# Ekumen-OS/beluga

Measured on AMD Instinct MI355X. Metric: MCL update cycles/sec (motion+sensor+resample), N particles x 1080 beams, higher is better.
Workload: dtype f64; 1 GPU; BASELINE configs[1]: 1M particles/GPU, 1080-beam LikelihoodFieldModel, 4000x4000@5cm grid (seed 42), DifferentialDriveModel, multinomial resample every cycle; particles_per_gpu=1000000, particles_total=1000000, beams=1080, grid=4000x4000@0.05, parallelism=1 GPU

## Files before the change

### beluga_amd/csrc/context.hip

```cpp
#include <hip/hip_runtime.h>
#include <dlfcn.h>

#include <algorithm>
#include <cctype>
#include <atomic>
#include <chrono>
#include <thread>
#include <cmath>
#include <cstdio>
#include <cstring>
#include <limits>
#include <new>
#include <numeric>
#include <optional>
#include <string>
#include <unordered_set>
#include <map>
#include <vector>

#include "beluga_mcl.h"
#include "cluster_host.h"
#include "cycle_host.h"
#include "kernels.h"
#include "landmark_host.h"
// ... 27 lines not shown
  mcl_config cfg;
  std::string error;
  int device{0};
  hipStream_t stream{nullptr};
  bool own_stream{false};
  mcl_batch* batch{nullptr};

  uint64_t capacity{0};
  uint64_t n{0};
  ParticleSet sets[2];
  int live{0};

  bool have_map{false};
  MapHold<MapStore> map{std::make_shared<MapStore>()};
  DeviceBuffer<uint32_t> d_field_scratch;
  uint64_t comm_bytes_out{0};
  uint64_t comm_collectives{0};
  uint64_t comm_host_syncs{0};
  uint64_t comm_overflows{0};
  uint64_t comm_ranks_seen{0};
  int comm_backend{0};
  uint64_t cluster_cells{0};

  DeviceBuffer<double> d_points;
  DeviceBuffer<double> d_beam_points;
  DeviceBuffer<double> d_beam_table;
  uint32_t beam_table_count{0};
  bool beam_table_ready{false};
  HostBuffer<double> h_points;
  double scan_extent{0.0};
  uint64_t scan_no_cell{0};
  hipEvent_t points_event{nullptr};
  bool points_in_flight{false}, points_event_valid{false};

  DeviceBuffer<double> d_chunk;
  uint32_t chunk_stride{0};
  DeviceBuffer<double> d_scalars;
  HostBuffer<double> h_scalars;
  DeviceBuffer<double> d_cdf;
  DeviceBuffer<double4> d_cloud;
  DeviceBuffer<double> d_est_partials;
  uint64_t done_seq{0};
  bool done_armed{false};
  uint64_t host_ns[4]{0, 0, 0, 0};
  uint64_t host_cycles{0};
  uint64_t noise_ahead_used{0};
  DeviceBuffer<double> d_cloud_w;
  DeviceBuffer<double> d_cdf_tree;
  DeviceBuffer<unsigned long long> d_scan_state;
  uint32_t scan_epoch{0};
  SetFacts facts;
  DeviceBuffer<double> d_lf_wsum;
  DeviceBuffer<double> d_noise;
  DiffDriveSampler order_sampler{};
  uint64_t order_ahead_used{0}, order_ahead_missed{0};
  DiffDriveSampler last_sampler{};
  bool have_last_sampler{false};
  CdfTree cdf_tree() const { return make_cdf_tree(d_cdf.ptr, d_cdf_tree.ptr, n); }
  struct PendingMap {
    std::vector<int8_t> cells;
    uint32_t W{0}, H{0};
    double resolution{0.0}, origin[4]{1.0, 0.0, 0.0, 0.0};
    int8_t traits[3]{0, -1, 100};
    std::vector<float> field;
    std::thread worker;
    std::atomic<int> state{0};
  };
  PendingMap* pending_map{nullptr};

  DeviceBuffer<unsigned long long> d_hashes;
  DeviceBuffer<unsigned long long> d_table_keys;
  DeviceBuffer<unsigned int> d_table_first;
  uint64_t table_capacity{0};
  DeviceBuffer<uint32_t> d_flags, d_uchunk;
  uint64_t kld_capacity{0};
  uint32_t kld_chunks{0};
  uint64_t kld_pos{0}, kld_table_slots{0};
  int kld_flip{0};
  DeviceBuffer<unsigned long long> d_kld_scalars;
  HostBuffer<unsigned long long> h_kld_scalars;

  DeviceBuffer<double> d_cell_f64;
  DeviceBuffer<unsigned int> d_cell_u32;
  DeviceBuffer<unsigned long long> d_cell_u64;
  DeviceBuffer<double> d_cell_exchange;
  DeviceBuffer<double> d_cluster_sums;
  DeviceBuffer<unsigned int> d_cluster_labels;
  int estimate_kind{0};
  mcl_cluster_params cluster_params{0.20, 0.524, 0.90};

  ExponentialFilter slow, fast;
  bool have_latest{false};
  Pose2 latest{};
  uint64_t every_n_current{0};
  bool force_update{true};
  bool have_window{false};
  Pose2 window0{}, window1{};
  uint32_t step{0};
  Tuning tuning{};
  CloudEstimate cloud;
  uint64_t lf_fast_launches{0};
  LfPlanner lf_planner;
  uint64_t lf_patch_launches{0};
  uint64_t lf_queue_launches{0};
  uint64_t lf_beams_launches{0};
  uint64_t estimate_repivots{0};
// ... 127 lines not shown
}
void stage_end(mcl_ctx* ctx, int stage) {
  if (!stage_timed(ctx, stage)) return;
  (void)hipEventRecord(ctx->ev[stage][1], ctx->stream);
  ctx->ev_pending[stage] = true;
}
void stage_collect(mcl_ctx* ctx) {
  ctx->points_in_flight = false;
  if (!ctx->profile) return;
  for (int s = 0; s < MCL_NUM_STAGES; ++s) {
    if (!ctx->ev_pending[s]) continue;
    float ms = 0.f;
    if (hipEventElapsedTime(&ms, ctx->ev[s][0], ctx->ev[s][1]) == hipSuccess) {
      ctx->prof_ms[s] += ms;
      ctx->prof_count[s] += 1;
    }
    ctx->ev_pending[s] = false;
  }
}

mcl_status wait_for_cycle(mcl_ctx* ctx) {
  if (ctx->done_armed) {
    ctx->done_armed = false;
    const volatile uint64_t* word = reinterpret_cast<const volatile uint64_t*>(ctx->h_scalars.host + kSlotDoneWord);
    const auto t0 = std::chrono::steady_clock::now();
    for (uint32_t spins = 1;; ++spins) {
      if (*word == ctx->done_seq) {
        std::atomic_thread_fence(std::memory_order_acquire);
        if ((ctx->done_seq & 0xFFu) == 0) break;
        return MCL_OK;
      }
#if defined(__x86_64__) || defined(__i386__)
      __builtin_ia32_pause();
#elif defined(__aarch64__)
      asm volatile("yield" ::: "memory");
#else
      std::this_thread::yield();
#endif
      if ((spins & 0xFFFu) == 0 && std::chrono::steady_clock::now() - t0 > std::chrono::milliseconds(20)) break;
    }
  }
  MCL_HIP(ctx, hipStreamSynchronize(ctx->stream));
  return MCL_OK;
}

mcl_status ensure_capacity(mcl_ctx* ctx, uint64_t cap) {
  for (auto& set : ctx->sets) MCL_HIP(ctx, set.ensure(cap));
  const uint32_t chunks = num_chunks(cap) + 1;
  ctx->chunk_stride = chunks;
  MCL_HIP(ctx, ctx->d_chunk.ensure(static_cast<size_t>(12) * chunks));
  MCL_HIP(ctx, ctx->d_cdf.ensure(cap));
  MCL_HIP(ctx, ctx->d_cdf_tree.ensure(cdf_tree_doubles(cap)));
  MCL_HIP(ctx, ctx->d_lf_wsum.ensure(cap / 448 + 2));
  if (!ctx->d_scan_state.ptr) {
    MCL_HIP(ctx, ctx->d_scan_state.ensure(kScanStateWords));
    MCL_HIP(ctx, hipMemset(ctx->d_scan_state.ptr, 0, kScanStateWords * sizeof(unsigned long long)));
  }
  ctx->capacity = cap;
  {
    static_assert(sizeof(KeyFrame) <= 8 * sizeof(double), "the key frame sits in the first 8 doubles of d_sort_f64");
    const size_t table = static_cast<size_t>(kSortDigits) * num_chunks(cap);
    MCL_HIP(ctx, ctx->d_sort_u32.ensure(2 * cap + table + 2 * kSortDigits + 16));
    MCL_HIP(ctx, ctx->d_sort_u64.ensure(cap));
    MCL_HIP(ctx, ctx->d_sort_f64.ensure(8 + 8 + 6 * static_cast<size_t>(chunks) + kLfMaxSegments * std::min<uint64_t>(cap, kLfSegmentedBelow)));
  }
  return MCL_OK;
}

mcl_status ensure_kld(mcl_ctx* ctx) {
  const uint64_t cap = std::max<uint64_t>(ctx->capacity, ctx->cfg.shard_capacity ? ctx->cfg.amcl.max_particles : 0);
  MCL_HIP(ctx, ctx->d_hashes.ensure(cap));
  MCL_HIP(ctx, ctx->d_flags.ensure(cap));
  ctx->kld_chunks = num_chunks(cap) + 1;
  MCL_HIP(ctx, ctx->d_uchunk.ensure(static_cast<size_t>(2) * ctx->kld_chunks));
  uint64_t tc = 1024;
  while (tc < 2 * cap) tc <<= 1;
  MCL_HIP(ctx, ctx->d_table_keys.ensure(tc));
  MCL_HIP(ctx, ctx->d_table_first.ensure(tc));
  ctx->table_capacity = tc;
  ctx->kld_capacity = cap;
  return MCL_OK;
}

enum KldWord : int { kKldFirstFail = 0, kKldBeamSteps = 1, kKldCounts = 4 };
mcl_status kld_begin(mcl_ctx* ctx) {
  if (ctx->table_capacity == 0) {
    if (const mcl_status s = ensure_kld(ctx)) return s;
  }
  MCL_HIP(ctx, hipMemsetAsync(ctx->d_kld_scalars.ptr + kKldFirstFail, 0xFF, sizeof(unsigned long long), ctx->stream));
  uint32_t* kwords = reinterpret_cast<uint32_t*>(ctx->d_kld_scalars.ptr + kKldCounts);
  MCL_HIP(ctx, hipMemsetAsync(kwords, 0, 2 * sizeof(uint32_t), ctx->stream));
  ctx->kld_pos = 0;
  ctx->kld_table_slots = 0;
  ctx->kld_flip = 0;
  return MCL_OK;
}

mcl_status kld_grow_table(mcl_ctx* ctx, uint64_t candidates) {
  uint64_t want = 1024;
  while (want < 2 * candidates) want <<= 1;
  want = std::min<uint64_t>(want, ctx->table_capacity);
  if (want <= ctx->kld_table_slots) return MCL_OK;
  ctx->kld_table_slots = want;
  MCL_HIP(ctx, hipMemsetAsync(ctx->d_table_keys.ptr, 0xFF, want * sizeof(unsigned long long), ctx->stream));
  MCL_HIP(ctx, hipMemsetAsync(ctx->d_table_first.ptr, 0xFF, want * sizeof(unsigned int), ctx->stream));
  launch_kld_insert(ctx->stream, ctx->d_hashes.ptr, 0, ctx->kld_pos, KldTable{ctx->d_table_keys.ptr, ctx->d_table_first.ptr, want});
// ... 310 lines not shown
    staged->doubles = kept;
  }
  ctx->scan_extent = poisoned ? std::numeric_limits<double>::quiet_NaN() : extent;
  return MCL_OK;
}
void points_pulled(mcl_ctx* ctx, bool with_event) {
  if (with_event) (void)hipEventRecord(ctx->points_event, ctx->stream);
  ctx->points_event_valid = with_event;
  ctx->points_in_flight = true;
}

void advance_window(mcl_ctx* ctx, const Pose2& pose) {
  ctx->window1 = ctx->have_window ? ctx->window0 : pose;
  ctx->window0 = pose;
  ctx->have_window = true;
  ctx->step += 1;
  const Pose2 action = pose_mul(pose_inverse(ctx->window1), ctx->window0);
  ctx->facts.pivot_carried(action.r.c, action.r.s, action.x, action.y);
}
void finish_cycle(mcl_ctx* ctx, const mcl_estimate& est, const mcl_update_info& report, mcl_estimate* estimate, mcl_update_info* info) {
  ctx->facts.estimate_reported(est.pose[0], est.pose[1], est.pose[2], est.pose[3]);
  ctx->cloud.remember(est);
  if (estimate) *estimate = est;
  if (info) *info = report;
}

void patch_totals(const mcl_ctx* ctx, uint64_t* planned, uint64_t* through, bool synchronised = false) {
  const volatile uint64_t* mirror = reinterpret_cast<const volatile uint64_t*>(ctx->h_scalars.host + kSlotPatchMirror);
  if (synchronised) {
    *planned = mirror[0];
    *through = mirror[1];
    return;
  }
  const uint64_t packed = mirror[2];
  *planned = packed & 0xFFFFFFFFull;
  *through = packed >> 32;
}
LfPlanner::Mode plan_lf(mcl_ctx* ctx) {
  uint64_t planned = 0, through = 0;
  if (!ctx->lf_planner.decided()) patch_totals(ctx, &planned, &through);
  return ctx->lf_planner.decide(ctx->lf_site(), ctx->cloud, planned, through);
}
struct HeldCycle {
  bool propagate_held{false};
  bool fused{false};
  bool pending{false};
  bool beam{false};
  BatchItem item{};
  uint64_t every_n{0};
};
void launch_held_propagate(mcl_ctx* ctx, HeldCycle* hold) {
  const BatchItem& it = hold->item;
  launch_propagate(ctx->stream, it.p, it.n, it.smp, it.seed, it.step, it.index_offset, it.scan_src, it.scan_dst, it.scan_doubles, nullptr, nullptr,
                   nullptr, 0);
  hold->propagate_held = false;
}
mcl_status do_propagate(mcl_ctx* ctx, const Pose2& pose, const Pose2& prev, uint32_t step, uint64_t scan_doubles = 0,
                        bool* keys_emitted = nullptr, HeldCycle* hold = nullptr) {
  stage_begin(ctx, MCL_STAGE_PROPAGATE);
  const DiffDriveSampler sampler = make_sampler(pose, prev, ctx->cfg.motion, ctx->cfg.motion_kind, ctx->cfg.strafe_noise_from_translation);
  KeyFrame frame{};
  const SortScratch sort = ctx->sort_scratch();
  if (keys_emitted) plan_lf(ctx);
  ctx->facts.order_accepted(false);
  bool use_ahead = false;
  if (keys_emitted) {
    const SetFacts::OrderTaken ahead = ctx->facts.take_order_ahead(step, ctx->n, ctx->key_layout());
    use_ahead = ahead.matched && ctx->tuning.order_ahead != 0 && ctx->wants_ordering() && samplers_close(sampler, ctx->order_sampler);
    if (use_ahead) ctx->order_ahead_used += 1;
    else if (ahead.recorded) ctx->order_ahead_missed += 1;
  }
  ctx->last_sampler = sampler;
  ctx->have_last_sampler = true;
  const bool keys = !use_ahead && keys_emitted && ctx->wants_ordering() && ctx->predict_key_frame(&sampler, &frame);
  const bool ahead = ctx->d_noise.ptr && ctx->n > 65536 && ctx->facts.noise_ahead_serves(step, ctx->n, ctx->cfg.seed, ctx->cfg.shard_offset);
  if (hold && !keys && !ahead && ctx->n >= 1 && ctx->n <= kBatchMaxParticles && !ctx->profile) {
    BatchItem& it = hold->item;
    it.p = ctx->cur();
    it.n = ctx->n;
    it.smp = sampler;
    it.seed = ctx->cfg.seed;
    it.step = step;
    it.index_offset = ctx->cfg.shard_offset;
    it.scan_src = scan_doubles ? ctx->h_points.device : nullptr;
    it.scan_dst = scan_doubles ? ctx->d_points.ptr : nullptr;
    it.scan_doubles = static_cast<uint32_t>(scan_doubles);
    hold->propagate_held = true;
  } else {
    launch_propagate(ctx->stream, ctx->cur(), ctx->n, sampler, ctx->cfg.seed, step, ctx->cfg.shard_offset,
                     scan_doubles ? ctx->h_points.device : nullptr, scan_doubles ? ctx->d_points.ptr : nullptr, static_cast<uint32_t>(scan_doubles),
                     keys ? &sort : nullptr, keys ? &frame : nullptr, ahead ? ctx->d_noise.ptr : nullptr, ctx->facts.noise_ahead_count());
  }
  if (ahead) ctx->noise_ahead_used += 1;
  if (scan_doubles) points_pulled(ctx, false);
  if (keys_emitted) *keys_emitted = keys;
  ctx->facts.order_accepted(use_ahead);
  stage_end(ctx, MCL_STAGE_PROPAGATE);
  MCL_HIP(ctx, hipGetLastError());
  return MCL_OK;
}

mcl_status reweight_preconditions(mcl_ctx* ctx, uint64_t B) {
  if (ctx->is_ndt()) {
    if (!ctx->have_ndt_map) return fail(ctx, MCL_ERR_NOT_READY, "mcl_reweight: no NDT map set (mcl_set_ndt_map)");
    MCL_REQUIRE(ctx, B <= 0x7FFFFFFFull, "too many points");
    return MCL_OK;
  }
  if (ctx->is_landmark()) {
    if (!ctx->have_landmark_map) return fail(ctx, MCL_ERR_NOT_READY, "no landmark map set (mcl_set_landmark_map)");
    return MCL_OK;
  }
  if (!ctx->have_map) return fail(ctx, MCL_ERR_NOT_READY, "mcl_reweight: no map set");
  MCL_REQUIRE(ctx, B <= 0x7FFFFFFFull, "too many points");
  if (ctx->cfg.sensor_kind == MCL_SENSOR_BEAM && !(ctx->n < (1ull << 32) && ctx->n >= static_cast<uint64_t>(ctx->tuning.beam_sort_min_particles)))
    MCL_REQUIRE(ctx, B * sizeof(double2) <= 64 * 1024, "scan too large for the beam model's small-set kernel (4096 points)");
  return MCL_OK;
}

mcl_status do_reweight(mcl_ctx* ctx, Measurement m, bool points_staged = false, bool keys_ready = false,
                       bool want_weight_sums = false, HeldCycle* hold = nullptr) {
  ctx->facts.lf_sums_dropped();
  if (const mcl_status s = reweight_preconditions(ctx, ctx->off_grid() ? 0 : m.doubles / 2)) return s;
  const bool unit_weights = ctx->facts.take_unit_weights() && ctx->tuning.lf_unit_weights != 0;
  if (!points_staged) {
    if (const mcl_status s = stage_points(ctx, &m)) return s;
    if (m.doubles) {
      launch_pull_scan(ctx->stream, ctx->h_points.device, ctx->d_points.ptr, static_cast<uint32_t>(m.doubles));
      points_pulled(ctx, true);
    }
  }
  const uint64_t B = ctx->off_grid() ? 0 : m.doubles / 2;
  stage_begin(ctx, MCL_STAGE_REWEIGHT);
  const LfPlanner::Mode mode = plan_lf(ctx);
  const bool ordered = ctx->wants_ordering();
  const bool dispersed = ctx->lf_planner.gathers_dispersed(ctx->tuning);
  ctx->lf_planner.mode_consumed();
  const SortScratch sort = ctx->sort_scratch();
  const bool have_order = ctx->facts.take_order_accepted();
  const bool lf_kind = !ctx->off_grid() && ctx->cfg.sensor_kind != MCL_SENSOR_BEAM;
  LfReweightArgs lf_args{};
  if (lf_kind)
    lf_args = LfReweightArgs{.p = ctx->cur(), .n = ctx->n, .f = ctx->field_view(), .d_points = ctx->d_points.ptr, .B = static_cast<uint32_t>(B),
                             .sort = ordered ? &sort : nullptr, .patches = mode.patches, .beams = mode.beams,
                             .dispersed = dispersed,
                             .scan_cells = ctx->scan_extent / ctx->map->resolution, .unit_weights = unit_weights,
                             .stats = PatchStats{reinterpret_cast<unsigned long long*>(ctx->d_scalars.ptr + kSlotPatchTotals),
                                                 reinterpret_cast<unsigned long long*>(ctx->h_scalars.device + kSlotPatchMirror),
                                                 static_cast<uint32_t>(ctx->tuning.lf_loose_below), ctx->tuning.lf_margin ? 0u : 1u,
                                                 static_cast<uint32_t>(ctx->tuning.lf_split), want_weight_sums ? ctx->d_lf_wsum.ptr : nullptr,
                                                 reinterpret_cast<unsigned int*>(ctx->d_scalars.ptr + kSlotPatchQueue)}};
  if (hold && hold->propagate_held) {
    hold->fused = lf_kind && batch_member_fused(BatchMemberFacts{
                                 ctx->cfg.sensor_kind, ctx->have_comm && ctx->comm_world > 1, ctx->tuning.small_fused != 0, ctx->n,
                                 std::min<uint64_t>(ctx->cfg.amcl.max_particles, ctx->capacity), lf_takes_beams(lf_args, ctx->tuning), ctx->profile != 0});
    hold->beam = !lf_kind && !ordered && batch_beam_member_fused(BatchBeamFacts{
                                 ctx->cfg.sensor_kind, ctx->have_comm && ctx->comm_world > 1, ctx->tuning.small_fused != 0,
                                 ctx->tuning.batch_beam_fused != 0, ctx->n, std::min<uint64_t>(ctx->cfg.amcl.max_particles, ctx->capacity),
                                 static_cast<uint64_t>(ctx->tuning.beam_sort_min_particles), ctx->profile != 0});
    hold->fused = hold->fused || hold->beam;
    if (!hold->fused) launch_held_propagate(ctx, hold);
  }
  if (ordered && !have_order) {
    KeyFrame frame{};
    const bool have_frame = !keys_ready && ctx->predict_key_frame(nullptr, &frame);
    launch_order_particles(ctx->stream, ctx->cur(), ctx->n, &sort, have_frame ? &frame : nullptr, keys_ready, frame.layout);
  }
  if (ctx->is_ndt()) {
    stage_begin(ctx, MCL_STAGE_SENSOR_KERNEL);
    launch_reweight_ndt(ctx->stream, ctx->cur(), ctx->n, ctx->ndt_view, ctx->d_points.ptr, static_cast<uint32_t>(m.doubles / kNdtRecord));
    stage_end(ctx, MCL_STAGE_SENSOR_KERNEL);
  } else if (ctx->is_landmark()) {
    const uint32_t k = static_cast<uint32_t>(m.doubles / kLandmarkRecord);
    stage_begin(ctx, MCL_STAGE_SENSOR_KERNEL);
    if (ctx->cfg.sensor_kind == MCL_SENSOR_LANDMARK) launch_reweight_landmarks(ctx->stream, ctx->cur(), ctx->n, ctx->landmark_view, ctx->d_points.ptr, k);
    else launch_reweight_bearings(ctx->stream, ctx->cur(), ctx->n, ctx->landmark_view, ctx->d_points.ptr, k);
    stage_end(ctx, MCL_STAGE_SENSOR_KERNEL);
  } else if (ctx->cfg.sensor_kind != MCL_SENSOR_BEAM) {
    stage_begin(ctx, MCL_STAGE_SENSOR_KERNEL);
    LfLaunch launched{LfKernel::kBeams, 0};
    if (hold && hold->fused) {
      hold->item.f = lf_args.f;
      hold->item.B = lf_args.B;
    } else {
      launched = launch_reweight_lf(ctx->stream, lf_args, ctx->tuning);
    }
    ctx->facts.lf_sums_left(launched.weight_sums);
    switch (launched.kernel) {
      case LfKernel::kPatchQueue: ctx->lf_queue_launches += 1; [[fallthrough]];
      case LfKernel::kPatch: ctx->lf_patch_launches += 1; ctx->lf_fast_launches += 1; break;
      case LfKernel::kFarBeams: ctx->lf_far_beams_launches += 1; [[fallthrough]];
      case LfKernel::kPaletteFar: ctx->lf_far_launches += 1; [[fallthrough]];
      case LfKernel::kPaletteFast: ctx->lf_fast_launches += 1; break;
      case LfKernel::kBeams: ctx->lf_beams_launches += 1; break;
      default: break;
    }
    stage_end(ctx, MCL_STAGE_SENSOR_KERNEL);
  } else {
    const mcl_beam_params& b = ctx->cfg.beam;
    const BeamModel model{b.z_hit, b.z_short, b.z_max, b.z_rand, b.sigma_hit, b.lambda_short, b.beam_max_range};
    const bool use_table = ordered && ctx->tuning.beam_table != 0 && ctx->beam_table_count != 0;
    if (use_table && !ctx->beam_table_ready) {
      hipError_t e = ctx->d_beam_table.ensure(4 * static_cast<size_t>(ctx->beam_table_count));
      if (e == hipSuccess) {
        launch_beam_table(ctx->stream, model, ctx->map->resolution, ctx->beam_table_count, ctx->d_beam_table.ptr);
        e = hipGetLastError();
      }
      if (e != hipSuccess) {
        stage_end(ctx, MCL_STAGE_REWEIGHT);
        return fail(ctx, MCL_ERR_HIP, std::string("reweight (beam table): ") + hipGetErrorString(e));
      }
      ctx->beam_table_ready = true;
    }
    stage_begin(ctx, MCL_STAGE_SENSOR_KERNEL);
    if (hold && hold->fused) {
      hold->item.B = static_cast<uint32_t>(B);
      hold->item.beam = batch_beam_record(ctx->grid_view(), model, ctx->map->d_nonfree_bits.ptr, ctx->d_kld_scalars.ptr + kKldBeamSteps);
    } else {
      launch_reweight_beam(ctx->stream, ctx->cur(), ctx->n, ctx->grid_view(), model,
                           ctx->d_points.ptr, static_cast<uint32_t>(B), ctx->d_kld_scalars.ptr + kKldBeamSteps, ordered ? &sort : nullptr,
                           ctx->map->d_nonfree_bits.ptr, ctx->d_beam_points.ptr, use_table ? ctx->d_beam_table.ptr : nullptr,
                           use_table ? ctx->beam_table_count : 0u, ctx->tuning.beam_free_ahead != 0, ctx->tuning.beam_sectors != 0);
    }
    stage_end(ctx, MCL_STAGE_SENSOR_KERNEL);
  }
  stage_end(ctx, MCL_STAGE_REWEIGHT);
  ctx->profile_tick += 1;
  if (const hipError_t e = hipGetLastError(); e != hipSuccess) {
    ctx->facts.lf_sums_dropped();
    return fail(ctx, MCL_ERR_HIP, std::string("reweight: ") + hipGetErrorString(e));
  }
  return MCL_OK;
}

mcl_weight_stats mirrored_weight_stats(const mcl_ctx* ctx) {
  return mcl_weight_stats{ctx->h_scalars.host[kSlotWeightSum], ctx->h_scalars.host[kSlotNormSum], ctx->h_scalars.host[kSlotNormSumSq]};
// ... 1231 lines not shown
    p->cells.assign(cells, cells + static_cast<size_t>(width) * height);
  } catch (const std::bad_alloc&) {
    delete p;
    return fail(ctx, MCL_ERR_OUT_OF_MEMORY, "mcl_set_map_async: out of memory");
  }
  p->W = width;
  p->H = height;
  p->resolution = resolution;
  std::memcpy(p->origin, origin, sizeof p->origin);
  std::memcpy(p->traits, value_traits, sizeof p->traits);
  ctx->pending_map = p;
  if (ctx->cfg.sensor_kind != MCL_SENSOR_BEAM && ctx->tuning.field_build == 0) {
    p->state.store(1, std::memory_order_release);
    const mcl_lf_params lf = ctx->cfg.lf;
    p->worker = std::thread([p, lf] {
      build_likelihood_field(p->cells.data(), p->W, p->H, p->resolution, OccupancyTraits{p->traits[0], p->traits[1], p->traits[2]}, lf, p->field);
      p->state.store(2, std::memory_order_release);
    });
  } else {
    p->state.store(2, std::memory_order_release);
  }
  return MCL_OK;
}

mcl_status mcl_map_pending(mcl_ctx* ctx, int32_t* state) {
  if (!ctx || !state) return MCL_ERR_INVALID_ARGUMENT;
  *state = ctx->pending_map ? ctx->pending_map->state.load(std::memory_order_acquire) : 0;
  return MCL_OK;
}

mcl_status mcl_map_commit(mcl_ctx* ctx, int32_t wait) {
  if (!ctx) return MCL_ERR_INVALID_ARGUMENT;
  return apply_pending_map(ctx, wait != 0);
}

}
namespace {
void map_installed(mcl_ctx* ctx) {
  if (ctx->cfg.sensor_kind == MCL_SENSOR_BEAM) {
    ctx->beam_table_count = beam_table_entries(ctx->cfg.beam.beam_max_range, ctx->map->resolution);
    ctx->beam_table_ready = false;
  }
  ctx->have_map = true;
}

mcl_status set_map_impl(mcl_ctx* ctx, const int8_t* cells, uint32_t width, uint32_t height, double resolution, const double origin[4],
                        const int8_t value_traits[3], std::vector<float>* prebuilt_field) {
  if (const mcl_status s = bind_device(ctx)) return s;
  MCL_HIP(ctx, hipStreamSynchronize(ctx->stream));
  auto store = std::make_shared<MapStore>();
  if (const std::shared_ptr<MapStore> old = ctx->map.take_private()) store->take_buffers(*old);
  ctx->map.drop();
  ctx->have_map = false;
  store->key = MapStoreKey{ctx->device, ctx->cfg.sensor_kind, ctx->cfg.lf};
  const MapSource in{cells, width, height, resolution, origin, value_traits, ctx->tuning.field_build, prebuilt_field};
  std::string err;
  if (const mcl_status s = build_map_store(*store, in, ctx->stream, &ctx->d_field_scratch, ctx->ev[MCL_STAGE_REWEIGHT], &err)) return fail(ctx, s, err);
  ctx->map.own(std::move(store));
  map_installed(ctx);
  return MCL_OK;
}

struct InstallSet {
  uint64_t n;
  bool unit_weights;
  enum { kGlobalKept, kGlobalShares, kGlobalAsked } global;
  bool force_update;
  enum { kCloudKept, kCloudUnknown, kCloudGiven } cloud;
  double cloud_mean[3], cloud_sigma[3];
  LfPlanner::Installed patches;
  bool pivot_known = false;
  double pivot[2] = {0.0, 0.0};
  bool pivot_kept = false;
};
void install_set(mcl_ctx* ctx, const InstallSet& s) {
  ctx->facts.set_replaced(s.unit_weights, s.pivot_kept);
  ctx->n = s.n;
  if (s.global == InstallSet::kGlobalShares) ctx->global_n = 0;
  if (s.global != InstallSet::kGlobalKept) ctx->global_n_unknown = s.global == InstallSet::kGlobalAsked && ctx->have_comm && ctx->comm_world > 1;
  if (s.force_update) ctx->force_update = true;
  if (s.cloud == InstallSet::kCloudGiven) ctx->cloud.set(s.cloud_mean, s.cloud_sigma);
  else if (s.cloud == InstallSet::kCloudUnknown) ctx->cloud.forget();
  if (s.cloud == InstallSet::kCloudGiven)
    ctx->facts.estimate_reported(std::cos(s.cloud_mean[2]), std::sin(s.cloud_mean[2]), s.cloud_mean[0], s.cloud_mean[1]);
  else if (s.pivot_known) ctx->facts.pivot_given(s.pivot[0], s.pivot[1]);
  uint64_t planned = 0, through = 0;
  if (s.patches != LfPlanner::Installed::kKept) patch_totals(ctx, &planned, &through);
  ctx->lf_planner.set_installed(s.patches, planned, through);
}
}
extern "C" {

mcl_status mcl_get_likelihood_field(mcl_ctx* ctx, float* out) {
  if (!ctx) return MCL_ERR_INVALID_ARGUMENT;
  MCL_REQUIRE(ctx, out, "null output");
  if (ctx->off_grid()) return fail(ctx, MCL_ERR_UNSUPPORTED, "The current sensor model does not support likelihood field");
  if (!ctx->have_map || !ctx->map->d_field.ptr) return fail(ctx, MCL_ERR_NOT_READY, "no likelihood field");
  if (const mcl_status s = bind_device(ctx)) return s;
  MCL_HIP(ctx, hipStreamSynchronize(ctx->stream));
  MCL_HIP(ctx, hipMemcpy(out, ctx->map->d_field.ptr, static_cast<size_t>(ctx->map->W) * ctx->map->H * sizeof(float), hipMemcpyDeviceToHost));
  return MCL_OK;
}

mcl_status mcl_set_likelihood_field(mcl_ctx* ctx, const float* field) {
  if (!ctx) return MCL_ERR_INVALID_ARGUMENT;
  MCL_REQUIRE(ctx, field, "null field");
  if (ctx->off_grid()) return fail(ctx, MCL_ERR_UNSUPPORTED, "mcl_set_likelihood_field: not on a context whose sensor model has a map of its own (mcl_set_ndt_map, mcl_set_landmark_map)");
  if (!ctx->have_map) return fail(ctx, MCL_ERR_NOT_READY, "set the map first");
  if (ctx->map.shared())
    return fail(ctx, MCL_ERR_UNSUPPORTED, "mcl_set_likelihood_field: the context reads a shared map, which does not change (mcl_set_map gives it a map of its own)");
  if (const mcl_status s = bind_device(ctx)) return s;
  MCL_HIP(ctx, hipStreamSynchronize(ctx->stream));
  const std::shared_ptr<MapStore> old = ctx->map.take_private();
  if (!old) return fail(ctx, MCL_ERR_NOT_READY, "set the map first");
  ctx->have_map = false;
  auto store = std::make_shared<MapStore>();
  store->take_buffers(*old);
  store->key = old->key;
  store->W = old->W;
  store->H = old->H;
  store->resolution = old->resolution;
  store->origin = old->origin;
  store->origin_inverse = old->origin_inverse;
  store->traits = old->traits;
  store->n_free = old->n_free;
  store->field_built_on_device = old->field_built_on_device;
  store->field_build_ms = old->field_build_ms;
  const size_t n = static_cast<size_t>(store->W) * store->H;
  MCL_HIP(ctx, store->d_field.ensure(n));
  MCL_HIP(ctx, hipMemcpy(store->d_field.ptr, field, n * sizeof(float), hipMemcpyHostToDevice));
  store->h_field.assign(field, field + n);
  std::string err;
  if (const mcl_status s = build_field_tables(*store, field, ctx->stream, &err)) return fail(ctx, s, err);
  ctx->map.own(std::move(store));
  ctx->have_map = true;
  return MCL_OK;
}

}
struct mcl_shared_map {
  std::shared_ptr<const MapStore> store;
  std::string error;
};
namespace {
thread_local std::string g_shared_map_error;
mcl_status fail_shared_map(mcl_status code, const std::string& msg) {
  g_shared_map_error = msg;
  return code;
}
}
extern "C" {

mcl_status mcl_shared_map_create(const mcl_config* cfg, const int8_t* cells, uint32_t width, uint32_t height, double resolution,
                                 const double origin[4], const int8_t value_traits[3], int32_t field_build, mcl_shared_map** out) {
  if (!cfg || !out) return fail_shared_map(MCL_ERR_INVALID_ARGUMENT, "mcl_shared_map_create: null argument");
  *out = nullptr;
  if (const char* why = map_store_check_kind(cfg->sensor_kind)) return fail_shared_map(MCL_ERR_UNSUPPORTED, why);
  if (!(cells && origin && value_traits && width > 0 && height > 0 && resolution > 0) || (field_build != 0 && field_build != 1))
    return fail_shared_map(MCL_ERR_INVALID_ARGUMENT, "mcl_shared_map_create: bad argument");
  if (!(static_cast<uint64_t>(width) * height < 0xFFFFFFFFull)) return fail_shared_map(MCL_ERR_INVALID_ARGUMENT, "mcl_shared_map_create: grid too large");
  int count = 0;
  if (hipGetDeviceCount(&count) != hipSuccess || count == 0)
    return fail_shared_map(MCL_ERR_NO_DEVICE, "mcl_shared_map_create: no HIP device (this library has no CPU fallback)");
  if (cfg->device_id < 0 || cfg->device_id >= count) return fail_shared_map(MCL_ERR_INVALID_ARGUMENT, "mcl_shared_map_create: bad device_id");
  mcl_shared_map* map = new (std::nothrow) mcl_shared_map();
  if (!map) return fail_shared_map(MCL_ERR_OUT_OF_MEMORY, "mcl_shared_map_create: host allocation failed");
  hipStream_t stream = nullptr;
  DeviceBuffer<uint32_t> scratch;
  auto store = std::make_shared<MapStore>();
  store->key = MapStoreKey{cfg->device_id, cfg->sensor_kind, cfg->lf};
  std::string err;
  auto build = [&]() -> mcl_status {
    MAP_HIP(&err, hipSetDevice(cfg->device_id));
    MAP_HIP(&err, configure_device_kernels());
    MAP_HIP(&err, hipStreamCreateWithFlags(&stream, hipStreamNonBlocking));
    const MapSource in{cells, width, height, resolution, origin, value_traits, field_build, nullptr};
    if (const mcl_status s = build_map_store(*store, in, stream, &scratch, nullptr, &err)) return s;
    MAP_HIP(&err, hipStreamSynchronize(stream));
    return MCL_OK;
  };
  const mcl_status st = build();
  if (stream) {
    (void)hipStreamSynchronize(stream);
    (void)hipStreamDestroy(stream);
  }
  scratch.release();
  if (st != MCL_OK) {
    delete map;
    return fail_shared_map(st, "mcl_shared_map_create: " + err);
  }
  map->store = std::move(store);
  *out = map;
  return MCL_OK;
}

void mcl_shared_map_release(mcl_shared_map* map) { delete map; }

mcl_status mcl_shared_map_get_info(const mcl_shared_map* map, mcl_shared_map_info* info) {
  if (!map || !info) return MCL_ERR_INVALID_ARGUMENT;
  const MapStore& s = *map->store;
  *info = mcl_shared_map_info{s.W, s.H, s.resolution, s.key.sensor_kind, s.key.device, s.device_bytes(), s.host_bytes(),
                              s.users.load(std::memory_order_relaxed)};
  return MCL_OK;
}

const char* mcl_shared_map_last_error(const mcl_shared_map* map) { return map ? map->error.c_str() : g_shared_map_error.c_str(); }

mcl_status mcl_use_shared_map(mcl_ctx* ctx, mcl_shared_map* map) {
  if (!ctx) return MCL_ERR_INVALID_ARGUMENT;
  MCL_REQUIRE(ctx, map, "mcl_use_shared_map: null map");
  if (ctx->off_grid()) return fail(ctx, MCL_ERR_UNSUPPORTED, "mcl_use_shared_map: not on a context whose sensor model has a map of its own (mcl_set_ndt_map, mcl_set_landmark_map)");
  if (const char* why = map_store_mismatch(map->store->key, ctx->device, ctx->cfg.sensor_kind, ctx->cfg.lf))
    return fail(ctx, MCL_ERR_INVALID_ARGUMENT, why);
  drop_pending_map(ctx);
  if (const mcl_status s = bind_device(ctx)) return s;
  MCL_HIP(ctx, hipStreamSynchronize(ctx->stream));
  ctx->map.attach(map->store);
  map_installed(ctx);
  return MCL_OK;
}

mcl_status mcl_initialize_normal(mcl_ctx* ctx, const double mean_xytheta[3], const double cov[9]) {
  if (!ctx) return MCL_ERR_INVALID_ARGUMENT;
  ctx->facts.set_changes();
  MCL_REQUIRE(ctx, mean_xytheta && cov, "null argument");
  double T[9];
  if (!covariance_to_transform(cov, T)) return fail(ctx, MCL_ERR_BAD_COVARIANCE, "Invalid covariance matrix");
  if (const mcl_status s = bind_device(ctx)) return s;
  const uint64_t n = std::min<uint64_t>(ctx->cfg.amcl.max_particles, ctx->capacity);
  ctx->facts.weights_rewrite_begins();
  launch_init_normal(ctx->stream, ctx->cur(), n, mean_xytheta, T, ctx->cfg.seed, ctx->cfg.shard_offset);
  MCL_HIP(ctx, hipGetLastError());
  install_set(ctx, {.n = n, .unit_weights = true, .global = InstallSet::kGlobalShares, .force_update = true ,
                    .cloud = InstallSet::kCloudGiven, .cloud_mean = {mean_xytheta[0], mean_xytheta[1], mean_xytheta[2]},
                    .cloud_sigma = {std::sqrt(std::max(cov[0], 0.0)), std::sqrt(std::max(cov[4], 0.0)), std::sqrt(std::max(cov[8], 0.0))},
                    .patches = LfPlanner::Installed::kFresh});
  return MCL_OK;
}

mcl_status mcl_set_particles(mcl_ctx* ctx, const double* states, const double* weights, uint64_t n) {
  if (!ctx) return MCL_ERR_INVALID_ARGUMENT;
  ctx->facts.set_changes();
  MCL_REQUIRE(ctx, n == 0 || (states && weights), "null argument");
  MCL_REQUIRE(ctx, n <= ctx->capacity, "mcl_set_particles: n exceeds capacity");
  if (const mcl_status s = bind_device(ctx)) return s;
  if (n) {
    MCL_HIP(ctx, hipStreamSynchronize(ctx->stream));
    MCL_HIP(ctx, hipMemcpy(ctx->cur().pose, states, n * 4 * sizeof(double), hipMemcpyHostToDevice));
    MCL_HIP(ctx, hipMemcpy(ctx->cur().w, weights, n * sizeof(double), hipMemcpyHostToDevice));
  }
  uint64_t first = 0;
  while (first < n && !(weights[first] > 0.0)) ++first;
  const bool sharded = ctx->have_comm && ctx->comm_world > 1;
  const bool pivot_known = first < n && !sharded;
  install_set(ctx, {.n = n, .unit_weights = false, .global = InstallSet::kGlobalAsked, .force_update = true, .cloud = InstallSet::kCloudUnknown,
                    .patches = LfPlanner::Installed::kFresh, .pivot_known = pivot_known,
                    .pivot = {pivot_known ? states[4 * first + 2] : 0.0, pivot_known ? states[4 * first + 3] : 0.0}, .pivot_kept = sharded});
  return MCL_OK;
}

mcl_status mcl_num_particles(mcl_ctx* ctx, uint64_t* n) {
  if (!ctx || !n) return MCL_ERR_INVALID_ARGUMENT;
  *n = ctx->n;
  return MCL_OK;
}

mcl_status mcl_get_particles(mcl_ctx* ctx, double* states, double* weights, uint64_t capacity, uint64_t* n) {
  if (!ctx) return MCL_ERR_INVALID_ARGUMENT;
  MCL_REQUIRE(ctx, capacity >= ctx->n, "mcl_get_particles: output too small");
  if (const mcl_status s = bind_device(ctx)) return s;
// ... 973 lines not shown
  origin[1] = o.r.s;
  origin[2] = o.x;
  origin[3] = o.y;
  return MCL_OK;
}

mcl_status mcl_update_point_cloud(mcl_ctx* ctx, const double control_pose[4], const float* points_xyz, uint64_t num_points,
                                  const double origin_se3[7], mcl_estimate* estimate, mcl_update_info* info) {
  if (!ctx) return MCL_ERR_INVALID_ARGUMENT;
  if (ctx->is_landmark()) return fail(ctx, MCL_ERR_UNSUPPORTED, "mcl_update_point_cloud: not on a landmark or bearing context");
  MCL_REQUIRE(ctx, origin_se3 && (num_points == 0 || points_xyz), "null argument");
  std::vector<double> pts(2 * num_points + 2);
  if (mcl_project_point_cloud(points_xyz, num_points, origin_se3, pts.data()) != MCL_OK) return fail(ctx, MCL_ERR_INVALID_ARGUMENT, "bad point cloud");
  return mcl_update(ctx, control_pose, pts.data(), num_points, estimate, info);
}

mcl_status mcl_set_option(mcl_ctx* ctx, const char* name, int64_t value) {
  if (!ctx || !name) return MCL_ERR_INVALID_ARGUMENT;
  const std::string key(name);
  const Tuning before = ctx->tuning;
  if (!set_tuning(ctx->tuning, name, value)) return fail(ctx, MCL_ERR_INVALID_ARGUMENT, "mcl_set_option: unknown option " + key);
  if (key == "device_policy" || key == "shard_pad_permille") {
    if (const mcl_status s = comm_agree(ctx, ("mcl_set_option(" + key + ")").c_str())) {
      ctx->tuning = before;
      return s;
    }
  } else if (key == "beam_table" && !ctx->tuning.beam_table && ctx->beam_table_ready) {
    if (bind_device(ctx) == MCL_OK && hipStreamSynchronize(ctx->stream) == hipSuccess) {
      ctx->d_beam_table.release();
      ctx->beam_table_ready = false;
    }
  }
  return MCL_OK;
}

}
namespace {
struct Counter {
  const char* name;
  uint64_t mcl_ctx::*member;
};
constexpr Counter kCounters[] = {
    {"lf_fast_launches", &mcl_ctx::lf_fast_launches},
    {"lf_patch_launches", &mcl_ctx::lf_patch_launches},
    {"lf_queue_launches", &mcl_ctx::lf_queue_launches},
    {"lf_beams_launches", &mcl_ctx::lf_beams_launches},
    {"lf_far_launches", &mcl_ctx::lf_far_launches},
    {"lf_far_beams_launches", &mcl_ctx::lf_far_beams_launches},
    {"small_tail_launches", &mcl_ctx::small_tail_launches},
    {"estimate_repivots", &mcl_ctx::estimate_repivots},
    {"noise_ahead_used", &mcl_ctx::noise_ahead_used},
    {"order_ahead_used", &mcl_ctx::order_ahead_used},
    {"order_ahead_missed", &mcl_ctx::order_ahead_missed},
    {"host_cycles", &mcl_ctx::host_cycles},
    {"cluster_cells", &mcl_ctx::cluster_cells},
    {"comm_bytes_out", &mcl_ctx::comm_bytes_out},
    {"comm_collectives", &mcl_ctx::comm_collectives},
    {"comm_host_syncs", &mcl_ctx::comm_host_syncs},
    {"comm_overflows", &mcl_ctx::comm_overflows},
    {"comm_ranks_seen", &mcl_ctx::comm_ranks_seen},
};
}
extern "C" {

mcl_status mcl_get_counter(mcl_ctx* ctx, const char* name, uint64_t* value) {
  if (!ctx || !name || !value) return MCL_ERR_INVALID_ARGUMENT;
  const std::string key(name);
  for (const Counter& c : kCounters) {
    if (key != c.name) continue;
    *value = ctx->*c.member;
    return MCL_OK;
  }
  if (key == "lf_far_tiles") *value = ctx->map->far_tiles;
  else if (key == "lf_patch_groups_planned" || key == "lf_patch_groups_through") {
    if (const mcl_status s = bind_device(ctx)) return s;
    MCL_HIP(ctx, hipStreamSynchronize(ctx->stream));
    uint64_t planned, through;
    patch_totals(ctx, &planned, &through, true);
    *value = key == "lf_patch_groups_planned" ? planned : through;
  }
  else if (key == "host_ns_to_first_launch") *value = ctx->host_ns[0];
  else if (key == "host_ns_other_launches") *value = ctx->host_ns[1];
  else if (key == "host_ns_wait") *value = ctx->host_ns[2];
  else if (key == "host_ns_after_wait") *value = ctx->host_ns[3];
  else if (key == "field_build_us") *value = static_cast<uint64_t>(ctx->map->field_build_ms * 1e3);
  else if (key == "field_built_on_device") *value = ctx->map->field_built_on_device ? 1 : 0;
  else if (key == "map_device_bytes") *value = ctx->map.shared() ? 0 : ctx->map->device_bytes();
  else if (key == "map_shared") *value = ctx->map.shared() ? 1 : 0;
  else if (key == "comm_backend") *value = static_cast<uint64_t>(ctx->comm_backend);
  else return fail(ctx, MCL_ERR_INVALID_ARGUMENT, "mcl_get_counter: unknown counter " + key);
  return MCL_OK;
}

mcl_status mcl_debug_order(mcl_ctx* ctx, uint32_t* perm, uint32_t* keys) {
  if (!ctx) return MCL_ERR_INVALID_ARGUMENT;
  MCL_REQUIRE(ctx, perm && keys, "null output");
  MCL_REQUIRE(ctx, ctx->n > 0 && ctx->n < (1ull << 32), "no particles");
  if (const mcl_status s = bind_device(ctx)) return s;
  const SortScratch sort = ctx->sort_scratch();
  KeyFrame frame{};
  const bool have_frame = ctx->predict_key_frame(nullptr, &frame);
  launch_order_particles(ctx->stream, ctx->cur(), ctx->n, &sort, have_frame ? &frame : nullptr, false, frame.layout);
  MCL_HIP(ctx, hipGetLastError());
  MCL_HIP(ctx, hipMemcpyAsync(perm, sort.perm, ctx->n * sizeof(uint32_t), hipMemcpyDeviceToHost, ctx->stream));
  MCL_HIP(ctx, hipMemcpyAsync(keys, sort.keys, ctx->n * sizeof(uint32_t), hipMemcpyDeviceToHost, ctx->stream));
  MCL_HIP(ctx, hipStreamSynchronize(ctx->stream));
// ... 303 lines not shown
```

### beluga_amd/csrc/cycle_host.cpp

```cpp
#include "cycle_host.h"

#include <algorithm>
#include <cmath>
#include <limits>

namespace mcl {

namespace {

double rotation_variance(const Rot2& r) {
  const Rot2 flipped = rot_mul(r, rot_exp(kPi));
  const double delta = std::min(std::abs(rot_log(r)), std::abs(rot_log(flipped)));
  return delta * delta;
}

bool off_grid(int sensor_kind) {
  return sensor_kind == MCL_SENSOR_NDT || sensor_kind == MCL_SENSOR_LANDMARK || sensor_kind == MCL_SENSOR_BEARING;
}

}


DiffDriveSampler make_sampler(const Pose2& pose, const Pose2& prev, const mcl_diffdrive_params& a, int kind, double alpha5) {
  const double tx = pose.x - prev.x, ty = pose.y - prev.y;
// ... 258 lines not shown
  const double average = norm_sum / static_cast<double>(n);
  const double fast_average = fast(average), slow_average = slow(average);
  if (std::abs(slow_average) >= std::numeric_limits<double>::epsilon())
    r.random_state_probability = std::clamp(1.0 - fast_average / slow_average, 0.0, 1.0);
  r.resample = fires;
  if (fires && selective_resampling) {
    r.ess = norm_sum == 0.0 ? 0.0 : (norm_sum * norm_sum) / norm_sumsq;
    r.resample = r.ess < static_cast<double>(n) * 0.5;
  }
  return r;
}


void shard_bounds(uint64_t n_total, uint32_t world, uint32_t rank, uint64_t* first, uint64_t* count) {
  const uint64_t base = n_total / world, rem = n_total % world;
  *first = rank * base + std::min<uint64_t>(rank, rem);
  *count = base + (rank < rem ? 1 : 0);
}

uint64_t padded_capacity(uint64_t n_total, uint32_t world, uint32_t permille) {
  const uint64_t m_max = (n_total + world - 1) / world;
  const double mean = static_cast<double>(m_max) / world;
  const double cap = mean * (permille / 1000.0) + 8.0 * std::sqrt(mean) + 64.0;
  return (static_cast<uint64_t>(cap) + 63u) & ~63ull;
}

uint64_t rebalance_block(uint64_t pos, uint64_t cnt, uint64_t n_out, uint32_t world, uint32_t rank, uint64_t* send, uint64_t* recv) {
  auto overlap = [](uint64_t a0, uint64_t a1, uint64_t b0, uint64_t b1) {
    const uint64_t lo = std::max(a0, b0), hi = std::min(a1, b1);
    return hi > lo ? hi - lo : 0;
  };
  uint64_t new_first, new_n, my_lo, my_m;
  shard_bounds(n_out, world, rank, &new_first, &new_n);
  shard_bounds(cnt, world, rank, &my_lo, &my_m);
  for (uint32_t q = 0; q < world; ++q) {
    uint64_t q_lo, q_m, span_first, span_n;
    shard_bounds(cnt, world, q, &q_lo, &q_m);
    shard_bounds(n_out, world, q, &span_first, &span_n);
    send[q] = overlap(pos + my_lo, std::min(pos + my_lo + my_m, n_out), span_first, span_first + span_n) * 4 * sizeof(double);
    recv[q] = overlap(pos + q_lo, std::min(pos + q_lo + q_m, n_out), new_first, new_first + new_n) * 4 * sizeof(double);
  }
  return std::min(std::max(pos, new_first) - new_first, new_n);
}

bool estimate_needs_repivot(const double sums[12]) {
  const double w = sums[0];
  if (!(w > 0.0)) return false;
  const double mx = sums[4] / w, my = sums[5] / w;
  const double m2 = mx * mx + my * my, second = (sums[6] + sums[8]) / w;
  if (!(m2 - m2 == 0.0 && second - second == 0.0)) return false;
  return (1.0 + kRepivotMultiple) * m2 > kRepivotMultiple * second;
}

}
```

### beluga_amd/csrc/cycle_host.h

```cpp
#pragma once

#include <cstdint>

#include "beluga_mcl.h"
#include "cycle_types.h"
#include "se2.h"

namespace mcl {

DiffDriveSampler make_sampler(const Pose2& pose, const Pose2& prev, const mcl_diffdrive_params& a, int kind, double alpha5);
bool samplers_close(const DiffDriveSampler& now, const DiffDriveSampler& predicted);
bool covariance_to_transform(const double cov[9], double T[9]);

class CloudEstimate {
 public:
  bool valid() const { return valid_; }
  const double* mean() const { return mean_; }
  const double* sigma() const { return sigma_; }
  void remember(const mcl_estimate& est);
  void set(const double mean[3], const double sigma[3]);
  void forget() { valid_ = false; }

 private:
  bool valid_{false};
  double mean_[3]{0, 0, 0}, sigma_[3]{0, 0, 0};
};

struct KeyFrameInputs {
  bool patch_useful;
  double resolution;
  double scan_extent;
  int key_warp, key_bits_xy;
};
bool predict_key_frame(const CloudEstimate& cloud, const DiffDriveSampler* motion, int moves, uint32_t layout, const KeyFrameInputs& in,
                       KeyFrame* out);

constexpr double kRepivotMultiple = 3.0;
bool estimate_needs_repivot(const double sums[12]);

struct LfSite {
  int sensor_kind;
  uint64_t n;
  bool palette;
  bool far_tiles;
  double resolution;
  const Tuning& tuning;
};

class LfPlanner {
 public:
  struct Mode { bool patches, beams; };
  enum class Installed { kKept, kFresh, kDispersed };

  bool patch_useful() const { return patch_useful_; }
  bool decided() const { return decided_; }

  void cycle_begins() { decided_ = false; }
  Mode decide(const LfSite& site, const CloudEstimate& cloud, uint64_t planned, uint64_t through);
  void mode_consumed() { decided_ = false; }
  void set_installed(Installed how, uint64_t planned, uint64_t through);

  bool wants_ordering(const LfSite& site) const;
  uint32_t key_layout(const LfSite& site) const;
  bool gathers_dispersed(const Tuning& tuning) const;
  static bool hopelessly_sparse(const LfSite& site, const CloudEstimate& cloud);

 private:
  bool wants_patches(const LfSite& site, const CloudEstimate& cloud, uint64_t planned, uint64_t through);

  uint64_t seen_planned_{0}, seen_through_{0};
  bool patch_useful_{true};
  int probe_in_{0};
  bool decided_{false};
  Mode mode_{false, false};
};

struct ExponentialFilter {
  double alpha{0.}, output{0.};
  void reset() { output = 0.; }
  double operator()(double input) {
    output += (output == 0.) ? input : alpha * (input - output);
    return output;
  }
};
bool moved_enough(const Pose2& latest, const Pose2& pose, double min_d, double min_a);
inline uint64_t next_every_n(uint64_t current, uint64_t interval) { return (current + 1) % interval; }

inline double lf_acc0(bool prob, float unknown_value, uint64_t no_cell) {
  const double pz = static_cast<double>(unknown_value);
  if (no_cell == 0) return prob ? 0.0 : 1.0;
  return prob ? static_cast<double>(no_cell) * std::log(pz) : 1.0 + static_cast<double>(no_cell) * (pz * pz * pz);
}
struct HostPolicy {
  double random_state_probability{0.0}, ess{-1.0};
  bool resample{false};
};
HostPolicy host_policy(ExponentialFilter& slow, ExponentialFilter& fast, bool selective_resampling, bool fires, double norm_sum,
                       double norm_sumsq, uint64_t n);

void shard_bounds(uint64_t n_total, uint32_t world, uint32_t rank, uint64_t* first, uint64_t* count);
uint64_t padded_capacity(uint64_t n_total, uint32_t world, uint32_t permille);
uint64_t rebalance_block(uint64_t pos, uint64_t cnt, uint64_t n_out, uint32_t world, uint32_t rank, uint64_t* send, uint64_t* recv);

}
```

### beluga_amd/csrc/cycle_types.h

```cpp
#pragma once

#include <algorithm>
#include <cstdint>

namespace mcl {

struct DiffDriveSampler {
  int kind;
  double m1, s1, mt, st, m2, s2;
  double first_c, first_s;
};

enum LfVariant : int {
  kLfWavePerParticle = 0,
  kLfLanePerParticle = 1,
  kLfSortedLanes = 2,
  kLfBeamLanes = 3
};

struct Tuning {
  int lf_variant = kLfSortedLanes;
  int lf_fast = -1;
  int lf_table = 0;
  int lf_patch = 1;
  int lf_loose_below = 224;
  int lf_dispersed = 2;
  int lf_far_beams_per_wave = 0;
  int device_policy = 1;
  int sort_min_particles = 16384;
  int beam_sort_min_particles = 16384;
  int lf_far_tiles = 1;
  int key_layout = -1;
  int lf_small_particles = 65536;
  int field_build = 0;
  int key_curve = 1;
  int key_warp = 1;
  int key_bits_xy = 0;
  int cycle_spin = -1;
  int beam_table = 1;
  int lf_weight_sums = 1;
  int lf_split = 3;
  int lf_margin = 1;
  int beam_free_ahead = 1;
  int lf_queue_grid = 0;
  int device_cus = 0;
  int shard_pad_permille = 1063;
  int lf_ends_first = 1;
  int beam_sectors = 1;
  int lf_queue = 1;
  int scan_fused = 1;
  int draw_fold = 1;
  int noise_ahead = 1;
  int order_ahead = 1;
  int draw_key_hist = 1;
  int rows_merged = 1;
  int norm_store = 0;
  int batch_cluster_fused = 1;
  int batch_beam_fused = 0;
  int small_fused = 1;
  int lf_unit_weights = 1;
};

struct KeyFrame {
  double cx, cy;
  double c0, s0;
  float inv_x, inv_y;
  float inv_t, t_off;
  uint32_t layout;
  uint32_t bits_xy;
};

inline bool lf_set_is_small(uint64_t n, const Tuning& t) {
  return n < static_cast<uint64_t>(std::max(t.sort_min_particles, t.lf_small_particles));
}

}
```

### beluga_amd/csrc/kernels.h

```cpp
#pragma once
#include <hip/hip_runtime.h>

#include <algorithm>
#include <cstdint>

#include "batch_host.h"
#include "cycle_types.h"
#include "se2.h"
#include "sensor_records.h"

namespace mcl {

struct Particles {
  double4* pose;
  double* w;
};

struct FieldView {
  const float* data;
  uint32_t W, H;
  double inv_resolution;
  Pose2 world_to_field;
  float unknown_value;
  const double* cube;
  int prob;
  const uint16_t* pal_idx;
  const double* pal_val;
  uint32_t pal_count;
  uint32_t pal_pitch;
  uint32_t pal_base;
  uint32_t pal_bytes;
  const uint8_t* far_bits;
  uint32_t far_row_bytes;
  uint32_t far_bytes;
  uint32_t far_entry;
  const uint8_t* far_linear;
  uint32_t far_linear_bytes;
  double acc0;
};

constexpr uint32_t kMaxPalette = 2048;
__host__ __device__ inline uint32_t palette_row_offset(int32_t y, uint32_t pitch) {
  const uint32_t py = static_cast<uint32_t>(y + 8);
  return (py >> 3) * pitch + ((py & 7u) << 1) + 128u;
}
__host__ __device__ inline uint32_t palette_offset(int32_t x, int32_t y, uint32_t pitch) {
  return palette_row_offset(y, pitch) + (static_cast<uint32_t>(x) << 4);
}

struct GridView {
  const int8_t* cells;
  uint32_t W, H;
  double resolution;
  Pose2 origin;
  Pose2 origin_inverse;
  int8_t free_value;
};

struct BeamModel {
  double z_hit, z_short, z_max, z_rand, sigma_hit, lambda_short, beam_max_range;
};

struct FreeCells {
  const uint32_t* index;
  uint64_t count;
  int normal{0};
  double mean[3]{0.0, 0.0, 0.0};
  double T[9]{0.0, 0.0, 0.0, 0.0, 0.0, 0.0, 0.0, 0.0, 0.0};
// ... 89 lines not shown
      const bool inv = (x1 & q) != 0;
      x0 ^= inv ? p : t;
      x1 ^= inv ? 0u : t;
    }
    {
      const uint32_t t = (x0 ^ x2) & p;
      const bool inv = (x2 & q) != 0;
      x0 ^= inv ? p : t;
      x2 ^= inv ? 0u : t;
    }
  }
  x1 ^= x0;
  x2 ^= x1;
  uint32_t t = 0;
#pragma unroll
  for (uint32_t q = 1u << (bits - 1); q > 1; q >>= 1) t ^= (x2 & q) ? q - 1 : 0u;
  x0 ^= t;
  x1 ^= t;
  x2 ^= t;
  auto spread = [](uint32_t v) {
    v = (v | (v << 8)) & 0x0300F00Fu;
    v = (v | (v << 4)) & 0x030C30C3u;
    v = (v | (v << 2)) & 0x09249249u;
    return v;
  };
  return (spread(x0) << 2) | (spread(x1) << 1) | spread(x2);
}
__host__ __device__ inline uint32_t hilbert_index_3(uint32_t a0, uint32_t a1, uint32_t a2, uint32_t bits) {
  switch (bits) {
    case 1: return hilbert_index_3_fixed<1>(a0, a1, a2);
    case 2: return hilbert_index_3_fixed<2>(a0, a1, a2);
    case 3: return hilbert_index_3_fixed<3>(a0, a1, a2);
    case 4: return hilbert_index_3_fixed<4>(a0, a1, a2);
    case 5: return hilbert_index_3_fixed<5>(a0, a1, a2);
    default: return hilbert_index_3_fixed<6>(a0, a1, a2);
  }
}
struct SortScratch {
  uint32_t* keys;
  uint32_t* perm;
  uint32_t* table;
  uint32_t* totals;
  unsigned long long* keyidx;
  double* bbox;
  KeyFrame* frame;
  double* partial;
};
constexpr uint32_t kLfMaxSegments = 16;
constexpr uint64_t kLfSegmentedBelow = 262144;

void launch_propagate(hipStream_t st, Particles p, uint64_t n, DiffDriveSampler smp, uint64_t seed, uint32_t step,
                      uint64_t index_offset, const double* scan_src = nullptr, double* scan_dst = nullptr, uint32_t scan_doubles = 0,
                      const SortScratch* sort = nullptr, const KeyFrame* frame = nullptr, const double* normals_ahead = nullptr,
                      uint64_t normals_stride = 0);
void launch_noise_ahead(hipStream_t st, uint64_t seed, uint32_t step, uint64_t index_offset, uint64_t n, double* d_normals);
void launch_pull_scan(hipStream_t st, const double* scan_src, double* scan_dst, uint32_t scan_doubles);
void launch_order_particles(hipStream_t st, Particles p, uint64_t n, const SortScratch* sort, const KeyFrame* frame, bool keys_ready,
                            uint32_t layout = 0);
enum OrderAheadDone : int {
  kOrderAheadKeys = 0,
  kOrderAheadHalfColumns = 1,
  kOrderAheadTable = 2
};
void launch_order_ahead(hipStream_t st, uint64_t n, const SortScratch* sort, OrderAheadDone done = kOrderAheadKeys);
struct PatchStats {
  unsigned long long* device;
  unsigned long long* mirror;
  uint32_t loose_below;
  uint32_t isotropic_margin;
  uint32_t split_patches;
  double* weight_sums;
  unsigned int* arrivals;
};
struct LfReweightArgs {
  Particles p;
  uint64_t n;
  FieldView f;
  const double* d_points;
  uint32_t B;
  const SortScratch* sort;
  bool patches, beams;
  bool dispersed;
  double scan_cells;
  bool unit_weights;
  PatchStats stats;
};
enum class LfKernel { kNone, kPatch, kPatchQueue, kFarBeams, kPaletteFar, kPaletteFast, kPaletteExact, kSortedCube, kSortedField, kBeams, kIndexOrder };
struct LfLaunch { LfKernel kernel; uint32_t weight_sums; };
LfLaunch launch_reweight_lf(hipStream_t st, const LfReweightArgs& a, const Tuning& tuning);
bool lf_takes_beams(const LfReweightArgs& a, const Tuning& tuning);
inline size_t lf_palette_lds(const FieldView& f) { return static_cast<size_t>(f.pal_base) + static_cast<size_t>(f.pal_count) * sizeof(double); }
constexpr uint32_t kBeamPointDoubles = 5;
void launch_lf_combine(hipStream_t st, double* w, uint64_t n, const uint32_t* perm, const double* partial, uint32_t segments, int mode);
void launch_reweight_beam(hipStream_t st, Particles p, uint64_t n, GridView g, BeamModel m, const double* d_points, uint32_t B,
                          unsigned long long* d_steps, const SortScratch* sorted, const uint32_t* nonfree_bits, double* d_beam_points,
                          const double* d_beam_table = nullptr, uint32_t beam_table_count = 0, bool free_ahead = true, bool sectors = true);
constexpr double kBeamTableMaxCells = 2046.0;
uint32_t beam_table_entries(double beam_max_range, double resolution);
void launch_beam_table(hipStream_t st, BeamModel m, double resolution, uint32_t entries, double* table);
struct NonFreeBits {
  const uint32_t* fine;
  const uint32_t* rows;
  const uint32_t* columns;
  const uint8_t* dist;
  uint32_t words_per_row, row_words, column_words, dist_stride;
};
NonFreeBits nonfree_layout(uint32_t W, uint32_t H, uint32_t* base);
size_t nonfree_words(uint32_t W, uint32_t H);
void launch_pack_nonfree(hipStream_t st, const int8_t* cells, uint32_t W, uint32_t H, int8_t free_value, uint32_t* bits);
hipError_t configure_device_kernels();
hipError_t configure_beam_kernels();

constexpr uint32_t kChunk = 2048;
inline uint32_t num_chunks(uint64_t n) { return static_cast<uint32_t>((n + kChunk - 1) / kChunk); }

void launch_weight_sum(hipStream_t st, const double* w, uint64_t n, double* d_partials, double* d_out, double* host_mirror = nullptr);
void launch_normalize(hipStream_t st, double* w, uint64_t n, const double* d_factor, double* d_chunk_sum, double* d_chunk_sumsq,
                      double* d_out, double* host_mirror = nullptr);
void launch_sum_and_normalize(hipStream_t st, double* w, uint64_t n, double* d_partials, double* d_chunk_sum, double* d_chunk_sumsq,
                              double* d_sums, double* host_mirror, bool finalize = true, const double* known_partials = nullptr,
                              uint32_t known_count = 0, bool store_weights = true);
struct RecoveryPolicy {
  double alpha_slow, alpha_fast;
  int resampling;
  double* d_policy;
  double* host_mirror;
};
void launch_norm_finalize(hipStream_t st, const double* d_chunk_sum, const double* d_chunk_sumsq, uint64_t n, double* d_sums,
                          double* sums_mirror, const RecoveryPolicy* policy);
struct Completion {
  unsigned long long* d_ticket{nullptr};
  unsigned long long* host_flag{nullptr};
  unsigned long long seq{0};
};
constexpr int kCdfTreeMaxDepth = 8;
struct CdfTree {
  const double* cdf;
  const double* levels;
// ... 59 lines not shown
  uint32_t step;
  bool fires, selective;
  double alpha_slow, alpha_fast, slow, fast, kld_epsilon, kld_z;
  HashParams hp;
  GridView g;
  FreeCells fc;
  double pivot_x, pivot_y;
  double* mirror;
  double* d_scalars;
  unsigned long long* done_flag{nullptr};
  unsigned long long done_seq{0};
};
bool launch_small_tail(hipStream_t st, const SmallTail& t);
struct SmallTailArgs {
  Particles src, dst;
  uint32_t n;
  uint32_t min_particles, max_particles;
  uint64_t seed;
  uint32_t step;
  int fires;
  int selective;
  int adaptive;
  double alpha_slow, alpha_fast, slow, fast;
  double two_epsilon, z;
  HashParams hp;
  GridView g;
  FreeCells fc;
  double pivot_x, pivot_y;
  double* out;
  double* d_out;
  unsigned long long* done_flag;
  unsigned long long done_seq;
};
SmallTailArgs small_tail_args(const SmallTail& t);
bool small_tail_fits(uint64_t n, uint64_t max_particles);

struct BatchBeam {
  GridView g;
  BeamModel m;
  NonFreeBits bits;
  unsigned long long* d_steps;
};
BatchBeam batch_beam_record(GridView g, BeamModel m, const uint32_t* nonfree_bits, unsigned long long* d_steps);
struct BatchItem {
  Particles p;
  uint64_t n;
  DiffDriveSampler smp;
  uint64_t seed;
  uint32_t step;
  uint64_t index_offset;
  const double* scan_src;
  double* scan_dst;
  uint32_t scan_doubles;
  FieldView f;
  uint32_t B;
  SmallTailArgs tail;
  uint32_t first_propagate_block, first_reweight_block;
  BatchBeam beam;
  uint32_t first_beam_block;
};
uint32_t launch_batch_cycle(hipStream_t st, const BatchItem* d_items, const BatchGrid& grid, const BatchBeamGrid& beam);
void launch_batch_reweight_beam(hipStream_t st, const BatchItem* d_items, uint32_t members, const BatchBeamGrid& grid);
void launch_resample_draw(hipStream_t st, Particles src, CdfTree cdf, const double* d_total, Particles dst,
                          ResampleArgs a, GridView g, FreeCells fc, HashParams hp, unsigned long long* d_hashes);
OrderAheadDone launch_resample_draw_and_estimate(hipStream_t st, Particles src, CdfTree cdf, const double* d_total, Particles dst, ResampleArgs a,
                                                 GridView g, FreeCells fc, HashParams hp, double pivot_x, double pivot_y, double* d_partials,
                                                 double* d_sums, double* host_mirror, const Completion* done = nullptr,
                                                 unsigned int* fold_ticket = nullptr, double* normals_ahead = nullptr,
                                                 uint64_t normals_stride = 0, uint64_t normals_index_offset = 0, uint32_t normals_step = 0,
                                                 uint32_t* keys_ahead = nullptr, const DiffDriveSampler* predicted = nullptr,
                                                 const KeyFrame* frame_ahead = nullptr, const SortScratch* hist_sort = nullptr,
                                                 bool rows_merged = false);
void launch_resample_targets(hipStream_t st, uint64_t seed, uint32_t step, double p, double total, uint64_t first_slot,
                             uint64_t count, uint64_t n_free, double* d_targets, const double* d_plan = nullptr);
struct RecoveryPolicy;
void launch_shard_plan(hipStream_t st, const double* d_stats, uint32_t world, uint64_t n_total, double* d_sums, double* sums_mirror,
                       const RecoveryPolicy& policy, double* d_intervals, double* d_plan);
void launch_route_targets(hipStream_t st, const double* d_targets, uint64_t count, const double* d_ends, const double* d_offsets,
                          uint32_t world, uint32_t self_rank, uint8_t* d_dest, uint32_t* d_block_hist, uint32_t* d_chunk_sum,
                          uint32_t* d_chunk_off, double* d_send_targets, uint32_t* d_order, long long* d_counts, uint32_t pad_capacity = 0,
                          double* d_overflow = nullptr);
void launch_gather_by_cdf_aos(hipStream_t st, Particles src, CdfTree cdf, const double* d_targets, uint64_t m,
                              double* d_out);
void launch_commit_routed(hipStream_t st, Particles dst, uint64_t seed, uint32_t step, uint64_t first_slot, uint64_t count,
                          const double* d_replies, const uint32_t* d_order, const double* d_targets, GridView g, FreeCells fc);
void launch_commit_injected(hipStream_t st, Particles dst, uint64_t seed, uint32_t step, uint64_t first_slot, uint64_t count,
                            const double* d_targets, GridView g, FreeCells fc);
void launch_finish_candidates(hipStream_t st, uint64_t seed, uint32_t step, uint64_t first_slot, uint64_t count, const double* d_replies,
                              const uint32_t* d_order, const double* d_targets, GridView g, FreeCells fc, HashParams hp,
                              double* d_states, unsigned long long* d_hashes);
struct KldTable {
  unsigned long long* keys;
  unsigned int* first;
  uint64_t capacity;
};
void launch_kld_insert(hipStream_t st, const unsigned long long* d_hashes, uint64_t first, uint64_t count, KldTable t);
void launch_kld_scan(hipStream_t st, const unsigned long long* d_hashes, uint64_t first, uint64_t count, KldTable t,
                     uint32_t* d_flags_scan, uint32_t* d_chunk_sum, uint32_t* d_chunk_offset, const uint32_t* d_k_base,
                     uint32_t* d_k_total, uint64_t min_particles, double epsilon, double z, unsigned long long* d_first_fail);
void launch_estimate_sums(hipStream_t st, Particles p, uint64_t n, double pivot_x, double pivot_y, double* d_partials,
                          double* d_out, double* host_mirror = nullptr);
struct CellTable {
  unsigned long long* keys;
  unsigned int* first;
  double* wsum;
  unsigned int* count;
// ... 71 lines not shown
```

### beluga_amd/csrc/kernels.hip

```cpp
#include "device_common.hpp"


namespace mcl {
namespace {

constexpr uint32_t kKeyBitsXY = 6, kKeyBitsTheta = 8, kKeyBits = 2 * kKeyBitsXY + kKeyBitsTheta;
constexpr uint32_t kDigitBits = 10;
static_assert((1u << kDigitBits) == kSortDigits && kKeyBits == 2 * kDigitBits, "two passes of one digit each");
__device__ __forceinline__ uint32_t spread3(uint32_t v) {
  v &= 0x3FF;
  v = (v | (v << 16)) & 0x030000FF;
  v = (v | (v << 8)) & 0x0300F00F;
  v = (v | (v << 4)) & 0x030C30C3;
  v = (v | (v << 2)) & 0x09249249;
  return v;
}
__device__ __forceinline__ uint32_t spread2(uint32_t v) {
  v &= 0x3F;
  v = (v | (v << 4)) & 0x30F;
  v = (v | (v << 2)) & 0x333;
  v = (v | (v << 1)) & 0x555;
  return v;
}
__device__ __forceinline__ int unit_bin(float u, int bins) {
// ... 119 lines not shown
  rot_apply(a.r, b.x, b.y, tx, ty);
  o.x = a.x + tx;
  o.y = a.y + ty;
  return o;
}
__device__ __forceinline__ void box_muller_fast(double u1, double u2, double& z0, double& z1) {
  const double r = sqrt(-2.0 * log(1.0 - u1));
  double sn, cs;
  sincos_fast(2.0 * kPi * u2, sn, cs);
  z0 = r * cs;
  z1 = r * sn;
}
__device__ __forceinline__ double4 propagation_normals(uint64_t seed, uint32_t step, uint64_t index) {
  const RngWords a = rng_draw(seed, step, kRngPropagateA, index);
  const RngWords b = rng_draw(seed, step, kRngPropagateB, index);
  double z0, z1, z2, z3;
  box_muller_fast(rng_uniform53(a.w[0], a.w[1]), rng_uniform53(a.w[2], a.w[3]), z0, z1);
  box_muller_fast(rng_uniform53(b.w[0], b.w[1]), rng_uniform53(b.w[2], b.w[3]), z2, z3);
  return double4{z0, z1, z2, z3};
}
__device__ __forceinline__ Pose2 propagate_with_normals(const Pose2& state, const DiffDriveSampler& smp, double z0, double z1, double z2) {
  if (smp.kind == 1) {
    const Rot2 first{smp.first_c, smp.first_s};
    const Rot2 second = rot_mul_fast(rot_exp_fast(z0 * smp.s1 + smp.m1), rot_inverse(first));
    const double t = z1 * smp.st + smp.mt;
    const double strafe = z2 * smp.s2 + 0.0;
    return pose_mul_fast(pose_mul_fast(state, Pose2{first, 0.0, 0.0}), Pose2{second, t, -strafe});
  }
  if (smp.kind == 2) {
    return pose_mul_fast(state, Pose2{rot_exp_fast(z0 * 0.02 + 0.0), z1 * 0.02 + 0.0, z2 * 0.02 + 0.0});
  }
  const double r1 = z0 * smp.s1 + smp.m1;
  const double t = z1 * smp.st + smp.mt;
  const double r2 = z2 * smp.s2 + smp.m2;
  return pose_mul_fast(pose_mul_fast(state, Pose2{rot_exp_fast(r1), 0.0, 0.0}), Pose2{rot_exp_fast(r2), t, 0.0});
}

__device__ __forceinline__ Pose2 propagate_one(const Pose2& state, const DiffDriveSampler& smp, uint64_t seed, uint32_t step, uint64_t index,
                                               const double* __restrict__ normals_ahead = nullptr, uint64_t local = 0, uint64_t stride = 0) {
  double z0, z1, z2;
  if (normals_ahead) {
    z0 = normals_ahead[local];
    z1 = normals_ahead[stride + local];
    z2 = normals_ahead[2 * stride + local];
  } else {
    const double4 z = propagation_normals(seed, step, index);
    z0 = z.x;
    z1 = z.y;
    z2 = z.z;
  }
  return propagate_with_normals(state, smp, z0, z1, z2);
}

__device__ __forceinline__ void propagate_small_block(uint32_t block, uint32_t blocks, const Particles& p, uint64_t n, const DiffDriveSampler& smp,
                                                      uint64_t seed, uint32_t step, uint64_t index_offset, const double* __restrict__ scan_src,
                                                      double* __restrict__ scan_dst, uint32_t scan_doubles) {
  if (scan_dst && block == blocks - 1) pull_scan(scan_src, scan_dst, scan_doubles);
  const uint64_t i = static_cast<uint64_t>(block) * kBlock + threadIdx.x;
  if (i < n) store_pose(p, i, propagate_one(load_pose(p, i), smp, seed, step, index_offset + i));
}
__global__ __launch_bounds__(kBlock) void k_propagate_small(Particles p, uint64_t n, DiffDriveSampler smp, uint64_t seed, uint32_t step,
                                                           uint64_t index_offset, const double* __restrict__ scan_src,
                                                           double* __restrict__ scan_dst, uint32_t scan_doubles) {
  propagate_small_block(blockIdx.x, gridDim.x, p, n, smp, seed, step, index_offset, scan_src, scan_dst, scan_doubles);
}

constexpr int kPropBlock = 512;
template <bool kKeys>
__global__ __launch_bounds__(kPropBlock) void k_propagate(Particles p, uint64_t n, DiffDriveSampler smp, uint64_t seed, uint32_t step,
                                                      uint64_t index_offset, const double* __restrict__ scan_src,
                                                      double* __restrict__ scan_dst, uint32_t scan_doubles, KeyFrame kf,
                                                      uint32_t* __restrict__ keys, uint32_t* __restrict__ table, uint32_t nblocks,
                                                      const double* __restrict__ normals_ahead, uint64_t normals_stride) {
  __shared__ uint32_t hist[kKeys ? kSortDigits : 1];
  if (kKeys) {
    for (uint32_t d = threadIdx.x; d < kSortDigits; d += kPropBlock) hist[d] = 0;
    __syncthreads();
  }
  if (scan_dst && blockIdx.x == gridDim.x - 1) pull_scan(scan_src, scan_dst, scan_doubles);
  const uint64_t base = static_cast<uint64_t>(blockIdx.x) * kChunk;
#pragma unroll 1
  for (int k = 0; k < kChunk / kPropBlock; ++k) {
    const uint64_t i = base + static_cast<uint64_t>(k) * kPropBlock + threadIdx.x;
    if (i >= n) break;
    const Pose2 out = propagate_one(load_pose(p, i), smp, seed, step, index_offset + i, normals_ahead, i, normals_stride);
    store_pose(p, i, out);
    if (kKeys) {
      const uint32_t key = order_key(double4{out.r.c, out.r.s, out.x, out.y}, kf);
      keys[i] = key;
      atomicAdd(&hist[key >> kDigitBits], 1u);
    }
  }
  if (kKeys) {
    __syncthreads();
    for (uint32_t d = threadIdx.x; d < kSortDigits; d += kPropBlock) table[static_cast<size_t>(d) * nblocks + blockIdx.x] = hist[d];
  }
}

__global__ __launch_bounds__(kBlock) void k_noise_ahead(uint64_t seed, uint32_t step, uint64_t index_offset, uint64_t n, double* __restrict__ out) {
  const uint64_t i = static_cast<uint64_t>(blockIdx.x) * kBlock + threadIdx.x;
  if (i >= n) return;
  const double4 z = propagation_normals(seed, step, index_offset + i);
  out[i] = z.x;
  out[n + i] = z.y;
  out[2 * n + i] = z.z;
}

__device__ __forceinline__ double lf_beam(const FieldView& f, double px, double py, double ct, double st, double xt, double yt) {
  const double x = px * ct - py * st + xt;
  const double y = px * st + py * ct + yt;
  const int xi = static_cast<int>(floor(x * f.inv_resolution));
  const int yi = static_cast<int>(floor(y * f.inv_resolution));
  const bool inside = static_cast<unsigned>(xi) < f.W && static_cast<unsigned>(yi) < f.H;
  const size_t idx = inside ? static_cast<size_t>(yi) * f.W + static_cast<size_t>(xi) : size_t{0};
  float v = f.data[idx];
  v = inside ? v : f.unknown_value;
  const double pz = static_cast<double>(v);
  return f.prob ? log(pz) : pz * pz * pz;
}

constexpr double kFloorMagic = 6755399441055744.0;
#define MCL_RD_BEGIN "s_nop 1\n\ts_setreg_imm32_b32 hwreg(HW_REG_MODE, 2, 2), 2\n\t"
#define MCL_RD_END "s_setreg_imm32_b32 hwreg(HW_REG_MODE, 2, 2), 0"
__device__ __forceinline__ void floor_rd_16(double (&v)[16]) {
  asm volatile(MCL_RD_BEGIN
               "v_add_f64 %0, %0, %16\n\tv_add_f64 %1, %1, %16\n\tv_add_f64 %2, %2, %16\n\tv_add_f64 %3, %3, %16\n\t"
               "v_add_f64 %4, %4, %16\n\tv_add_f64 %5, %5, %16\n\tv_add_f64 %6, %6, %16\n\tv_add_f64 %7, %7, %16\n\t"
               "v_add_f64 %8, %8, %16\n\tv_add_f64 %9, %9, %16\n\tv_add_f64 %10, %10, %16\n\tv_add_f64 %11, %11, %16\n\t"
               "v_add_f64 %12, %12, %16\n\tv_add_f64 %13, %13, %16\n\tv_add_f64 %14, %14, %16\n\tv_add_f64 %15, %15, %16\n\t"
               MCL_RD_END
               : "+v"(v[0]), "+v"(v[1]), "+v"(v[2]), "+v"(v[3]), "+v"(v[4]), "+v"(v[5]), "+v"(v[6]), "+v"(v[7]), "+v"(v[8]),
                 "+v"(v[9]), "+v"(v[10]), "+v"(v[11]), "+v"(v[12]), "+v"(v[13]), "+v"(v[14]), "+v"(v[15])
               : "s"(kFloorMagic));
}
__device__ __forceinline__ void floor_rd_8(double (&v)[8]) {
  asm volatile(MCL_RD_BEGIN
               "v_add_f64 %0, %0, %8\n\tv_add_f64 %1, %1, %8\n\tv_add_f64 %2, %2, %8\n\tv_add_f64 %3, %3, %8\n\t"
               "v_add_f64 %4, %4, %8\n\tv_add_f64 %5, %5, %8\n\tv_add_f64 %6, %6, %8\n\tv_add_f64 %7, %7, %8\n\t"
               MCL_RD_END
               : "+v"(v[0]), "+v"(v[1]), "+v"(v[2]), "+v"(v[3]), "+v"(v[4]), "+v"(v[5]), "+v"(v[6]), "+v"(v[7])
               : "s"(kFloorMagic));
}
__device__ __forceinline__ void floor_rd_2(double& a, double& b) {
  asm volatile(MCL_RD_BEGIN "v_add_f64 %0, %0, %2\n\tv_add_f64 %1, %1, %2\n\t" MCL_RD_END : "+v"(a), "+v"(b) : "s"(kFloorMagic));
}
__device__ __forceinline__ int floor_rd_result(double v) { return static_cast<int>(static_cast<uint32_t>(__builtin_bit_cast(uint64_t, v))); }

__device__ __forceinline__ double lf_cube_fetch(__amdgpu_buffer_rsrc_t rsrc, const FieldView& f, uint32_t row_bytes,
                                                uint32_t unknown_offset, int xi, int yi) {
  const bool inside = static_cast<unsigned>(xi) < f.W && static_cast<unsigned>(yi) < f.H;
  const uint32_t offset = inside ? __umul24(static_cast<unsigned>(yi), row_bytes) + (static_cast<unsigned>(xi) << 3) : unknown_offset;
  return __builtin_bit_cast(double, __builtin_amdgcn_raw_buffer_load_b64(rsrc, offset, 0, 0));
}

__device__ __forceinline__ Pose2 ordered_pose(const Pose2& to_frame, const double4* __restrict__ pose, uint64_t i) {
  const double4 q = pose[i];
  return pose_mul_ieee(to_frame, Pose2{Rot2{q.x, q.y}, q.z, q.w});
}

template <bool kCube>
__global__ __launch_bounds__(kBlock) void k_reweight_lf_sorted(double* __restrict__ w, uint64_t n, FieldView f,
                                                               const double* __restrict__ pts, uint32_t B,
                                                               const uint32_t* __restrict__ perm, const double4* __restrict__ pose,
                                                               double* __restrict__ partial, uint32_t beams_per_segment) {
  const uint64_t t = static_cast<uint64_t>(blockIdx.x) * kBlock + threadIdx.x;
  const uint64_t tt = t < n ? t : n - 1;
  const uint64_t i = perm ? perm[tt] : tt;
  const Pose2 T = ordered_pose(f.world_to_field, pose, i);
  const double ct = T.r.c, st = T.r.s, xt = T.x, yt = T.y;
  const uint32_t b_begin = partial ? blockIdx.y * beams_per_segment : 0u;
  const uint32_t b_end = partial ? (b_begin + beams_per_segment < B ? b_begin + beams_per_segment : B) : B;
  double acc = partial ? 0.0 : f.acc0;
  if (kCube) {
    const uint32_t cells = f.W * f.H;
    const __amdgpu_buffer_rsrc_t rsrc =
        __builtin_amdgcn_make_buffer_rsrc(const_cast<double*>(f.cube), 0, static_cast<int>((cells + 1) * 8u), 0x00020000);
    const uint32_t row_bytes = f.W * 8u, unknown_offset = cells * 8u;
    uint32_t b = b_begin;
    for (; b + 8 <= b_end; b += 8) {
      double v[16];
#pragma unroll
      for (int k = 0; k < 8; ++k) {
        const double px = pts[2 * (b + k)], py = pts[2 * (b + k) + 1];
        v[2 * k] = (px * ct - py * st + xt) * f.inv_resolution;
        v[2 * k + 1] = (px * st + py * ct + yt) * f.inv_resolution;
      }
      floor_rd_16(v);
      double t[8];
#pragma unroll
      for (int k = 0; k < 8; ++k)
        t[k] = lf_cube_fetch(rsrc, f, row_bytes, unknown_offset, floor_rd_result(v[2 * k]), floor_rd_result(v[2 * k + 1]));
      acc += sum4(t[0], t[1], t[2], t[3]);
      acc += sum4(t[4], t[5], t[6], t[7]);
    }
    auto term = [&](uint32_t at) {
      const double px = pts[2 * at], py = pts[2 * at + 1];
      double vx = (px * ct - py * st + xt) * f.inv_resolution, vy = (px * st + py * ct + yt) * f.inv_resolution;
      floor_rd_2(vx, vy);
      return lf_cube_fetch(rsrc, f, row_bytes, unknown_offset, floor_rd_result(vx), floor_rd_result(vy));
    };
    if (b + 4 <= b_end) {
      const double t0 = term(b), t1 = term(b + 1), t2 = term(b + 2), t3 = term(b + 3);
      acc += sum4(t0, t1, t2, t3);
      b += 4;
    }
    for (; b < b_end; ++b) acc += term(b);
  } else {
    uint32_t b = b_begin;
#pragma unroll 2
    for (; b + 4 <= b_end; b += 4) {
      double t[4];
#pragma unroll
      for (int k = 0; k < 4; ++k) t[k] = lf_beam(f, pts[2 * (b + k)], pts[2 * (b + k) + 1], ct, st, xt, yt);
      acc += sum4(t[0], t[1], t[2], t[3]);
    }
    for (; b < b_end; ++b) acc += lf_beam(f, pts[2 * b], pts[2 * b + 1], ct, st, xt, yt);
  }
  if (t < n) {
    if (partial) {
      partial[static_cast<size_t>(blockIdx.y) * n + t] = acc;
    } else {
// ... 3 lines not shown
}

constexpr int kPalBlock = 512;
typedef __attribute__((address_space(3))) const double lds_f64_t;
typedef __attribute__((address_space(3))) const uint32_t lds_u32_t;
typedef __attribute__((address_space(3))) const uint8_t lds_u8_t;
__device__ __forceinline__ int clamp_cell(int v, uint32_t hi) {
  int r;
  asm("v_med3_i32 %0, %1, -1, %2" : "=v"(r) : "v"(v), "s"(hi));
  return r;
}
constexpr uint32_t kFastBias = 0x41380000u;
constexpr uint32_t kFastBiasX = kFastBias << 4;
constexpr double kFastMagic = 1572864.0;
__device__ __forceinline__ uint32_t lf_palette_offset(const FieldView& f, int xi, int yi, uint32_t row_fix) {
  const int xc = clamp_cell(xi, f.W), yc = clamp_cell(yi, f.H);
  const uint32_t row = *reinterpret_cast<lds_u32_t*>(static_cast<uintptr_t>(static_cast<uint32_t>(yc + 1) << 2));
  return (static_cast<uint32_t>(xc) << 4) + row_fix + row;
}
__device__ __forceinline__ int med3_i32(int v, int lo , int hi) {
  int r;
  asm("v_med3_i32 %0, %1, %2, %3" : "=v"(r) : "v"(v), "v"(lo), "s"(hi));
  return r;
}
__device__ __forceinline__ uint32_t mad_u24(uint32_t a, uint32_t b , uint32_t c) {
  uint32_t r;
  asm("v_mad_u32_u24 %0, %1, %2, %3" : "=v"(r) : "v"(a), "s"(b), "v"(c));
  return r;
}
__device__ __forceinline__ uint32_t patch_address(uint32_t cx, uint32_t cy, uint32_t K ) {
  uint32_t r;
  asm("v_lshl_add_u32 %0, %1, 1, %3\n\tv_mad_u32_u24 %0, %2, %4, %0" : "=&v"(r) : "v"(cy), "v"(cx), "s"(K), "s"(144u));
  return r;
}
__device__ __forceinline__ uint32_t min3_u32(uint32_t a, uint32_t b, uint32_t c) {
  uint32_t r;
  asm("v_min3_u32 %0, %1, %2, %3" : "=v"(r) : "v"(a), "v"(b), "v"(c));
  return r;
}
__device__ __forceinline__ uint32_t lf_palette_fetch(__amdgpu_buffer_rsrc_t rsrc, const FieldView& f, int xi, int yi, uint32_t row_fix) {
  return static_cast<uint32_t>(
      static_cast<uint16_t>(__builtin_amdgcn_raw_buffer_load_b16(rsrc, lf_palette_offset(f, xi, yi, row_fix), 0, 0)));
}
__device__ __forceinline__ double lf_palette_value(uint32_t lds_address) {
  return *reinterpret_cast<lds_f64_t*>(static_cast<uintptr_t>(lds_address));
}

__device__ __forceinline__ uint32_t far_block(uint32_t b, uint32_t blocks ) { return (b & 7u) * (blocks >> 3) + (b >> 3); }
template <bool kFast, bool kFar = false>
__global__ __launch_bounds__(kPalBlock) void k_reweight_lf_palette(double* __restrict__ w, uint64_t n, FieldView f,
                                                                   const double* __restrict__ pts, uint32_t B,
                                                                   const uint32_t* __restrict__ perm, const double4* __restrict__ pose,
                                                                   double* __restrict__ partial, uint32_t beams_per_segment,
                                                                   uint32_t far_base) {
  static_assert(kFast || !kFar, "far tiles ride on the biased coordinates of the FMA variant");
  extern __shared__ __attribute__((aligned(16))) unsigned char smem[];
  if constexpr (kFar) {
    if (static_cast<uint64_t>(far_block(blockIdx.x, gridDim.x)) * kPalBlock >= n) return;
    const uint4* src = reinterpret_cast<const uint4*>(f.far_bits);
    uint4* dst = reinterpret_cast<uint4*>(smem + far_base);
    for (uint32_t j = threadIdx.x; j < f.far_bytes / 16; j += kPalBlock) dst[j] = src[j];
  }
  {
    uint32_t* s_row = reinterpret_cast<uint32_t*>(smem);
    constexpr uint32_t row_fix_stored = kFast ? kFastBiasX : 0u;
    for (uint32_t j = threadIdx.x; j < f.H + 2; j += kPalBlock)
      s_row[j] = palette_row_offset(static_cast<int32_t>(j) - 1, f.pal_pitch) - row_fix_stored;
    double* s_pal = reinterpret_cast<double*>(smem + f.pal_base);
    for (uint32_t k = threadIdx.x; k < f.pal_count; k += kPalBlock) s_pal[k] = f.pal_val[k];
  }
  __syncthreads();
  const uint32_t block = kFar ? far_block(blockIdx.x, gridDim.x) : blockIdx.x;
  const uint64_t t = static_cast<uint64_t>(block) * kPalBlock + threadIdx.x;
  const uint64_t tt = t < n ? t : n - 1;
  const uint32_t i = perm[tt];
  const Pose2 T = ordered_pose(f.world_to_field, pose, i);
  const double ct = T.r.c, st = T.r.s, xt = T.x, yt = T.y;
  const uint32_t b_begin = partial ? blockIdx.y * beams_per_segment : 0u;
  const uint32_t b_end = partial ? (b_begin + beams_per_segment < B ? b_begin + beams_per_segment : B) : B;
  double acc = partial ? 0.0 : f.acc0;
  const __amdgpu_buffer_rsrc_t rsrc =
      __builtin_amdgcn_make_buffer_rsrc(const_cast<uint16_t*>(f.pal_idx), 0, static_cast<int>(f.pal_bytes), 0x00020000);
  constexpr uint32_t row_fix = kFast ? kFastBiasX : 0u;
  auto issue = [&](uint32_t (&e)[8], uint32_t b0) {
    double v[16];
#pragma unroll
    for (int k = 0; k < 8; ++k) {
      const double px = pts[2 * (b0 + k)], py = pts[2 * (b0 + k) + 1];
      v[2 * k] = (px * ct - py * st + xt) * f.inv_resolution;
      v[2 * k + 1] = (px * st + py * ct + yt) * f.inv_resolution;
    }
    floor_rd_16(v);
#pragma unroll
    for (int k = 0; k < 8; ++k) e[k] = lf_palette_fetch(rsrc, f, floor_rd_result(v[2 * k]), floor_rd_result(v[2 * k + 1]), row_fix);
  };
  auto consume = [&](uint32_t (&e)[8], bool) {
    double t[8];
#pragma unroll
    for (int k = 0; k < 8; ++k) t[k] = lf_palette_value(e[k]);
    acc += sum4(t[0], t[1], t[2], t[3]);
    acc += sum4(t[4], t[5], t[6], t[7]);
  };
  uint32_t b = b_begin;
  uint32_t groups = (b_end - b_begin) / 8;
  bool fast = false;
  if constexpr (kFast) {
    const double ict = ct * f.inv_resolution, ist = st * f.inv_resolution, ixt = xt * f.inv_resolution, iyt = yt * f.inv_resolution;
    const bool lane_small = fabs(ixt) < 16384.0 && fabs(iyt) < 16384.0;
    fast = __builtin_amdgcn_ballot_w64(!lane_small) == 0;
    if (groups && fast) {
      const int c_lo = static_cast<int>(kFastBias) - 1, x_hi = static_cast<int>(kFastBias + f.W), y_hi = static_cast<int>(kFastBias + f.H);
      const uint32_t row_bias = 4u - (kFastBias << 2);
      auto issue_fast = [&](uint32_t (&e)[8], uint32_t b0) {
        uint32_t near_integer = 0xFFFFFFFFu;
#pragma unroll
        for (int k = 0; k < 8; ++k) {
          const double px = pts[2 * (b0 + k)], py = pts[2 * (b0 + k) + 1];
          const double sx = __builtin_fma(px, ict, __builtin_fma(-py, ist, ixt)) + kFastMagic;
          const double sy = __builtin_fma(px, ist, __builtin_fma(py, ict, iyt)) + kFastMagic;
          const uint64_t bx = __builtin_bit_cast(uint64_t, sx), by = __builtin_bit_cast(uint64_t, sy);
          near_integer = min3_u32(near_integer, static_cast<uint32_t>(bx), static_cast<uint32_t>(by));
          const int xc = med3_i32(static_cast<int>(bx >> 32), c_lo, x_hi), yc = med3_i32(static_cast<int>(by >> 32), c_lo, y_hi);
          const uint32_t row = *reinterpret_cast<lds_u32_t*>(static_cast<uintptr_t>((static_cast<uint32_t>(yc) << 2) + row_bias));
          uint32_t offset = (static_cast<uint32_t>(xc) << 4) + row;
          uint32_t common = 0u;
          if constexpr (kFar) {
            const uint32_t tx8 = static_cast<uint32_t>(xc) + 8u, ty8 = static_cast<uint32_t>(yc) + 8u;
            const uint32_t at = mad_u24(__builtin_amdgcn_ubfe(ty8, 3, 16), f.far_row_bytes, __builtin_amdgcn_ubfe(tx8, 6, 13)) + far_base;
            const uint32_t byte = *reinterpret_cast<lds_u8_t*>(static_cast<uintptr_t>(at));
// ... 24 lines not shown
        b += 8;
      } else {
        consume(ea, false);
      }
      groups = 0;
    }
  }
  if (groups) {
    uint32_t ea[8], eb[8];
    issue(ea, b);
    b += 8;
    --groups;
    while (groups >= 2) {
      issue(eb, b);
      consume(ea, true);
      issue(ea, b + 8);
      consume(eb, true);
      b += 16;
      groups -= 2;
    }
    if (groups) {
      issue(eb, b);
      consume(ea, true);
      consume(eb, false);
      b += 8;
    } else {
      consume(ea, false);
    }
  }
  auto term = [&](uint32_t at) {
    const double px = pts[2 * at], py = pts[2 * at + 1];
    double vx = (px * ct - py * st + xt) * f.inv_resolution, vy = (px * st + py * ct + yt) * f.inv_resolution;
    floor_rd_2(vx, vy);
    return lf_palette_value(lf_palette_fetch(rsrc, f, floor_rd_result(vx), floor_rd_result(vy), row_fix));
  };
  if (b + 4 <= b_end) {
    const double t0 = term(b), t1 = term(b + 1), t2 = term(b + 2), t3 = term(b + 3);
    acc += sum4(t0, t1, t2, t3);
    b += 4;
  }
  for (; b < b_end; ++b) acc += term(b);
  if (t < n) {
    if (partial) {
      partial[static_cast<size_t>(blockIdx.y) * n + t] = acc;
    } else {
      w[i] = w[i] * (f.prob ? exp(acc) : acc);
    }
  }
}

constexpr int kBeamsBlock = 256;
__device__ __forceinline__ void reweight_lf_beams_block(uint32_t block, const Particles& p, uint64_t n, const FieldView& f,
                                                        const double2* __restrict__ pts, uint32_t B,
                                                        uint32_t per_wave ) {
  extern __shared__ __attribute__((aligned(16))) unsigned char smem[];
  {
    uint32_t* s_row = reinterpret_cast<uint32_t*>(smem);
    for (uint32_t j = threadIdx.x; j < f.H + 2; j += kBeamsBlock) s_row[j] = palette_row_offset(static_cast<int32_t>(j) - 1, f.pal_pitch);
    double* s_pal = reinterpret_cast<double*>(smem + f.pal_base);
    for (uint32_t k = threadIdx.x; k < f.pal_count; k += kBeamsBlock) s_pal[k] = f.pal_val[k];
  }
  __syncthreads();
  const uint32_t lane = threadIdx.x & 63;
  const uint64_t tile = static_cast<uint64_t>(block) * (kBeamsBlock / kWave) + (threadIdx.x >> 6);
  const uint64_t base = tile * per_wave;
  if (base >= n) return;
  const uint32_t cnt = static_cast<uint32_t>(n - base < per_wave ? n - base : per_wave);
  const uint64_t i = base + lane;
  Pose2 state = pose_identity();
  if (lane < cnt) state = load_pose(p, i);
  const Pose2 T = pose_mul_ieee(f.world_to_field, state);
  const __amdgpu_buffer_rsrc_t rsrc =
      __builtin_amdgcn_make_buffer_rsrc(const_cast<uint16_t*>(f.pal_idx), 0, static_cast<int>(f.pal_bytes), 0x00020000);
  const uint32_t full = B & ~255u;
  double mine = 0.0;
#pragma unroll 1
  for (uint32_t q = 0; q < cnt; ++q) {
    const double ct = readlane_f64(T.r.c, q), st = readlane_f64(T.r.s, q);
    const double xt = readlane_f64(T.x, q), yt = readlane_f64(T.y, q);
    double acc = 0.0;
#pragma unroll 1
    for (uint32_t b0 = 0; b0 < full; b0 += 256) {
      double v[8];
#pragma unroll
      for (int k = 0; k < 4; ++k) {
        const double2 pt = pts[b0 + 64 * k + lane];
        v[2 * k] = (pt.x * ct - pt.y * st + xt) * f.inv_resolution;
        v[2 * k + 1] = (pt.x * st + pt.y * ct + yt) * f.inv_resolution;
      }
      floor_rd_8(v);
      uint32_t e[4];
#pragma unroll
      for (int k = 0; k < 4; ++k) e[k] = lf_palette_fetch(rsrc, f, floor_rd_result(v[2 * k]), floor_rd_result(v[2 * k + 1]), 0u);
#pragma unroll
      for (int k = 0; k < 4; ++k) acc += lf_palette_value(e[k]);
    }
    for (uint32_t b = full + lane; b < B; b += kWave) {
      const double2 pt = pts[b];
      double vx = (pt.x * ct - pt.y * st + xt) * f.inv_resolution, vy = (pt.x * st + pt.y * ct + yt) * f.inv_resolution;
      floor_rd_2(vx, vy);
      acc += lf_palette_value(lf_palette_fetch(rsrc, f, floor_rd_result(vx), floor_rd_result(vy), 0u));
    }
    const double total = wave_sum_f64(acc);
    if (lane == q) mine = total;
  }
  if (lane < cnt) p.w[i] = p.w[i] * (f.prob ? exp(f.acc0 + mine) : f.acc0 + mine);
}
__global__ __launch_bounds__(kBeamsBlock) void k_reweight_lf_beams(Particles p, uint64_t n, FieldView f, const double2* __restrict__ pts,
                                                                   uint32_t B, uint32_t per_wave ) {
  reweight_lf_beams_block(blockIdx.x, p, n, f, pts, B, per_wave);
}

constexpr int kFarBeamsBlock = 768;
constexpr int kFarBeamsWaves = 6;
constexpr int kFarBeamsPoses = 2;
typedef double f64x2_t __attribute__((ext_vector_type(2)));
typedef __attribute__((address_space(3))) const f64x2_t lds_f64x2_t;
constexpr uint32_t kFarBeamsPalShift = 32768;
constexpr uint32_t kFarBeamsChunk = 16;
template <bool kProb>
__global__ __launch_bounds__(kFarBeamsBlock) __attribute__((amdgpu_waves_per_eu(kFarBeamsWaves, kFarBeamsWaves))) void k_reweight_lf_far_beams(double* __restrict__ w, uint64_t n, FieldView f,
                                                                          const double2* __restrict__ pts, uint32_t B,
                                                                          const uint32_t* __restrict__ perm, const double4* __restrict__ pose,
                                                                          uint32_t pts_at, uint32_t per_wave, uint32_t unit_weights) {
  extern __shared__ __attribute__((aligned(16))) unsigned char smem[];
  constexpr int J = kFarBeamsPoses;
  const uint32_t rows_at = f.far_linear_bytes;
  const uint32_t rounds = (B + 63u) >> 6;
  {
    const uint4* src = reinterpret_cast<const uint4*>(f.far_linear);
    uint4* dst = reinterpret_cast<uint4*>(smem);
    for (uint32_t j = threadIdx.x; j < f.far_linear_bytes / 16; j += kFarBeamsBlock) dst[j] = src[j];
    uint32_t* s_row = reinterpret_cast<uint32_t*>(smem + rows_at);
    for (uint32_t j = threadIdx.x; j < f.H + 2; j += kFarBeamsBlock)
      s_row[j] = palette_row_offset(static_cast<int32_t>(j) - 1, f.pal_pitch) - kFastBiasX;
    double* s_pal = reinterpret_cast<double*>(smem + kFarBeamsPalShift + f.pal_base);
    for (uint32_t k = threadIdx.x; k < f.pal_count; k += kFarBeamsBlock) s_pal[k] = f.pal_val[k];
    double2* s_pts = reinterpret_cast<double2*>(smem + pts_at);
    for (uint32_t b = threadIdx.x; b < rounds * 64u; b += kFarBeamsBlock) s_pts[b] = b < B ? pts[b] : double2{0.0, 0.0};
  }
  __syncthreads();
  const uint32_t lane = threadIdx.x & 63, wave = threadIdx.x >> 6;
  const uint64_t first = (static_cast<uint64_t>(far_block(blockIdx.x, gridDim.x)) * (kFarBeamsBlock / kWave) + wave) * per_wave;
  if (first >= n) return;
  const uint32_t cnt = static_cast<uint32_t>(n - first < per_wave ? n - first : per_wave);
  const bool dead_last = ((rounds - 1u) << 6) + lane >= B;
  const __amdgpu_buffer_rsrc_t rsrc =
      __builtin_amdgcn_make_buffer_rsrc(const_cast<uint16_t*>(f.pal_idx), 0, static_cast<int>(f.pal_bytes), 0x00020000);
  const int c_lo = static_cast<int>(kFastBias) - 1, x_hi = static_cast<int>(kFastBias + f.W), y_hi = static_cast<int>(kFastBias + f.H);
  const uint32_t row_bias = rows_at + 4u - (kFastBias << 2);
  const uint32_t my_point = pts_at + (lane << 4);
  const uint32_t slots_at = pts_at + (rounds << 10) + wave * (kFarBeamsChunk * 32u);
#pragma unroll 1
  for (uint32_t c0 = 0; c0 < cnt; c0 += kFarBeamsChunk) {
    const uint32_t m = cnt - c0 < kFarBeamsChunk ? cnt - c0 : kFarBeamsChunk;
    uint32_t i = 0;
    Pose2 T = pose_identity();
    if (lane < m) {
      i = perm[first + c0 + lane];
      T = ordered_pose(f.world_to_field, pose, i);
    }
    unsigned long long large;
    {
      const double l_ict = T.r.c * f.inv_resolution, l_ist = T.r.s * f.inv_resolution, l_ixt = T.x * f.inv_resolution,
                   l_iyt = T.y * f.inv_resolution;
      large = __builtin_amdgcn_ballot_w64(!(fabs(l_ixt) < 16384.0 && fabs(l_iyt) < 16384.0));
      if (lane < kFarBeamsChunk) {
        f64x2_t* slot = reinterpret_cast<f64x2_t*>(smem + slots_at + (lane << 5));
        slot[0] = f64x2_t{l_ict, l_ist};
        slot[1] = f64x2_t{l_ixt, l_iyt};
      }
    }
    double mine = 0.0;
#pragma unroll 1
    for (uint32_t q0 = 0; q0 < m; q0 += J) {
      double ict[J], ist[J], ixt[J], iyt[J], acc[J];
#pragma unroll
      for (int j = 0; j < J; ++j) {
        const uint32_t at = slots_at + ((q0 + j) << 5);
        const f64x2_t rot = *reinterpret_cast<lds_f64x2_t*>(static_cast<uintptr_t>(at));
        const f64x2_t tr = *reinterpret_cast<lds_f64x2_t*>(static_cast<uintptr_t>(at + 16u));
        ict[j] = rot.x;
        ist[j] = rot.y;
        ixt[j] = tr.x;
        iyt[j] = tr.y;
        acc[j] = 0.0;
      }
      bool exact = ((large >> q0) & ((1ull << J) - 1ull)) != 0;
      if (!exact) {
        uint32_t near_integer = 0xFFFFFFFFu;
        auto issue = [&](uint32_t (&e)[J], uint32_t k) {
          const f64x2_t pt = *reinterpret_cast<lds_f64x2_t*>(static_cast<uintptr_t>(my_point + (k << 10)));
#pragma unroll
          for (int j = 0; j < J; ++j) {
            const double sx = __builtin_fma(pt.x, ict[j], __builtin_fma(-pt.y, ist[j], ixt[j])) + kFastMagic;
            const double sy = __builtin_fma(pt.x, ist[j], __builtin_fma(pt.y, ict[j], iyt[j])) + kFastMagic;
            const uint64_t bx = __builtin_bit_cast(uint64_t, sx), by = __builtin_bit_cast(uint64_t, sy);
            near_integer = min3_u32(near_integer, static_cast<uint32_t>(bx), static_cast<uint32_t>(by));
            const int xc = med3_i32(static_cast<int>(bx >> 32), c_lo, x_hi), yc = med3_i32(static_cast<int>(by >> 32), c_lo, y_hi);
            const uint32_t row = *reinterpret_cast<lds_u32_t*>(static_cast<uintptr_t>((static_cast<uint32_t>(yc) << 2) + row_bias));
            const uint32_t offset = (static_cast<uint32_t>(xc) << 4) + row;
            const uint32_t byte = *reinterpret_cast<lds_u8_t*>(static_cast<uintptr_t>(offset >> 10));
            const uint32_t far = __builtin_amdgcn_ubfe(byte, __builtin_amdgcn_ubfe(offset, 7, 3), 1);
            const uint32_t loaded = static_cast<uint32_t>(
                static_cast<uint16_t>(__builtin_amdgcn_raw_buffer_load_b16(rsrc, offset | (far << 31), 0, 0)));
            e[j] = mad_u24(far, f.far_entry, loaded);
          }
        };
        auto consume = [&](const uint32_t (&e)[J], bool last) {
#pragma unroll
          for (int j = 0; j < J; ++j) {
            double v = lf_palette_value(e[j] + kFarBeamsPalShift);
            if (last) v = dead_last ? 0.0 : v;
            acc[j] += v;
          }
        };
        uint32_t ea[J], eb[J];
        if (rounds > 1) {
          issue(ea, 0);
          uint32_t k = 1;
          while (k + 2 < rounds) {
            issue(eb, k);
            consume(ea, false);
            issue(ea, k + 1);
            consume(eb, false);
            k += 2;
          }
          if (k + 1 < rounds) {
            issue(eb, k);
            consume(ea, false);
            issue(ea, k + 1);
            consume(eb, false);
            consume(ea, true);
          } else {
            issue(eb, k);
            consume(ea, false);
            consume(eb, true);
          }
        } else {
          issue(ea, 0);
          consume(ea, true);
        }
        exact = __builtin_amdgcn_ballot_w64(near_integer == 0) != 0;
      }
      if (exact) {
#pragma unroll 1
        for (int j = 0; j < J; ++j) {
          const uint32_t iq = static_cast<uint32_t>(__builtin_amdgcn_readlane(static_cast<int>(i), static_cast<int>(q0) + j));
          const Pose2 Tq = ordered_pose(f.world_to_field, pose, iq);
          double sum = 0.0;
#pragma unroll 1
          for (uint32_t k = 0; k < rounds; ++k) {
            if (64u * k + lane < B) {
              const double2 pt = pts[64u * k + lane];
              double vx = (pt.x * Tq.r.c - pt.y * Tq.r.s + Tq.x) * f.inv_resolution, vy = (pt.x * Tq.r.s + pt.y * Tq.r.c + Tq.y) * f.inv_resolution;
              floor_rd_2(vx, vy);
              const int xc = clamp_cell(floor_rd_result(vx), f.W), yc = clamp_cell(floor_rd_result(vy), f.H);
              const uint32_t row = *reinterpret_cast<lds_u32_t*>(static_cast<uintptr_t>(rows_at + (static_cast<uint32_t>(yc + 1) << 2)));
              const uint32_t at = (static_cast<uint32_t>(xc) << 4) + kFastBiasX + row;
              sum += lf_palette_value(static_cast<uint32_t>(static_cast<uint16_t>(__builtin_amdgcn_raw_buffer_load_b16(rsrc, at, 0, 0))) +
                                      kFarBeamsPalShift);
            }
          }
#pragma unroll
          for (int jj = 0; jj < J; ++jj)
            if (j == jj) acc[jj] = sum;
        }
      }
#pragma unroll
      for (int j = 0; j < J; ++j) {
        const double total = wave_sum_f64(acc[j]);
        if (lane == q0 + j) mine = total;
      }
    }
    if (lane < m) w[i] = (unit_weights != 0u ? 1.0 : w[i]) * (kProb ? exp(f.acc0 + mine) : f.acc0 + mine);
  }
}

constexpr int kPatchW = 64, kPatchH = 64;
constexpr uint32_t kPatchPitch = kPatchH * 2 + 16;
static_assert(kPatchPitch == 144, "patch_address() carries the pitch as a literal");
constexpr uint32_t kPatchBytes = kPatchW * kPatchPitch;
constexpr int kPatchBlock = 512;
constexpr uint32_t kPatchParticles = kPatchBlock - 64;
constexpr uint32_t kPatchPlanned = 192;
constexpr uint32_t kPatchBuffers = 3;
constexpr uint32_t kPatchLdsBytes = kPatchBuffers * kPatchBytes + kPatchPlanned * 32 + 16 + 48 * 4;
static_assert(kPatchPlanned * 8 * 16 <= kPatchBuffers * kPatchBytes, "the per-beam records of the plan live in the patch buffers");
constexpr double kPatchMagic = 1572864.0 + 4.656612873077392578125e-10;
__device__ __attribute__((noinline)) double exp_out_of_line(double x) { return exp(x); }
struct PatchArgs {
  double* w;
  uint64_t n;
  FieldView f;
  const double* pts;
  uint32_t B;
  const uint32_t* perm;
  const double4* pose;
  double* partial;
  uint32_t beams_per_segment;
  uint32_t patch_base;
  PatchStats stats;
  uint32_t nblocks;
  uint32_t ends_first;
  uint32_t unit_weights;
};
template <bool kQueue>
__global__ __launch_bounds__(kPatchBlock) __attribute__((amdgpu_waves_per_eu(6, 6))) void k_reweight_lf_patch(PatchArgs args) {
  typedef const __attribute__((address_space(4))) unsigned char* kernarg_bytes_t;
  const kernarg_bytes_t kernarg = (kernarg_bytes_t)(__builtin_amdgcn_kernarg_segment_ptr());
  const PatchArgs* ka = (const PatchArgs*)(kernarg);
  const uint32_t patch_base = ka->patch_base;
  extern __shared__ __attribute__((aligned(16))) unsigned char smem[];
  {
    const FieldView& f = ka->f;
    uint32_t* s_row = reinterpret_cast<uint32_t*>(smem);
    for (uint32_t j = threadIdx.x; j < f.H + 2; j += kPatchBlock)
      s_row[j] = palette_row_offset(static_cast<int32_t>(j) - 1, f.pal_pitch) - kFastBiasX;
    double* s_pal = reinterpret_cast<double*>(smem + f.pal_base);
    for (uint32_t k = threadIdx.x; k < f.pal_count; k += kPatchBlock) s_pal[k] = f.pal_val[k];
    if (threadIdx.x == 0) *reinterpret_cast<int4*>(smem + patch_base + kPatchBuffers * kPatchBytes + kPatchPlanned * 32) = int4{0, 0, 0, 0};
  }
  auto buffer_of = [&](uint32_t g) -> uint32_t {
    const uint32_t slot = g - 3u * ((g * 0xAAABu) >> 17);
    return patch_base + slot * kPatchBytes;
  };
  int4* s_plan = reinterpret_cast<int4*>(smem + patch_base + kPatchBuffers * kPatchBytes);
  int4* s_plan_k = s_plan + kPatchPlanned;
  float* s_bound = reinterpret_cast<float*>(smem + patch_base + kPatchBuffers * kPatchBytes + kPatchPlanned * 32 + 16);
  constexpr uint32_t kConsumers = kPatchBlock / 64 - 1;
  constexpr uint32_t kParticles = kConsumers * 64;
  const uint32_t wave_id = static_cast<uint32_t>(__builtin_amdgcn_readfirstlane(threadIdx.x >> 6));
  const bool producer = wave_id == (kPatchBlock / 64 - 1);
  uint32_t* s_next = reinterpret_cast<uint32_t*>(s_bound) + 46;
#pragma unroll 1
  for (;;) {
  uint32_t tid = threadIdx.x;
  if constexpr (kQueue) asm volatile("" : "+v"(tid));
  const uint32_t lane = tid & 63;
  uint32_t kernarg_offset = 0;
  if constexpr (kQueue) asm volatile("" : "+s"(kernarg_offset));
  const PatchArgs* kb = (const PatchArgs*)(kernarg + kernarg_offset);
  double* const& w = kb->w;
  const uint64_t& n = kb->n;
  const FieldView& f = kb->f;
  const double* const pts = kb->pts;
  const uint32_t B = kb->B;
  const uint32_t* const& perm = kb->perm;
  const double4* const& pose = kb->pose;
  double* const& partial = kb->partial;
  const uint32_t beams_per_segment = kb->beams_per_segment;
  const PatchStats& stats = kb->stats;
  const uint32_t nblocks = kb->nblocks;
  const bool ends_first = kb->ends_first != 0u;
  const uint32_t& unit_weights = kb->unit_weights;
  uint32_t block = blockIdx.x;
  if constexpr (kQueue) {
    __syncthreads();
    if (tid == 0) *s_next = atomicInc(stats.arrivals, nblocks + gridDim.x - 1u);
    __syncthreads();
    block = static_cast<uint32_t>(__builtin_amdgcn_readfirstlane(*s_next));
    if (block >= nblocks) break;
  }
  if (ends_first) block = (block & 1u) ? nblocks - 1u - (block >> 1) : (block >> 1);
  const uint64_t first = static_cast<uint64_t>(block) * kParticles;
  const uint64_t t = producer ? first : first + tid;
  const uint64_t tt = t < n ? t : n - 1;
  const uint32_t i = perm[tt];
  const Pose2 T = ordered_pose(f.world_to_field, pose, i);
  const double ct = T.r.c, st = T.r.s, xt = T.x, yt = T.y;
  const uint32_t b_begin = partial ? blockIdx.y * beams_per_segment : 0u;
  const uint32_t b_end = partial ? (b_begin + beams_per_segment < B ? b_begin + beams_per_segment : B) : B;
  const uint32_t groups = (b_end - b_begin) / 8;
  const __amdgpu_buffer_rsrc_t rsrc =
      __builtin_amdgcn_make_buffer_rsrc(const_cast<uint16_t*>(f.pal_idx), 0, static_cast<int>(f.pal_bytes), 0x00020000);
  const double ict = ct * f.inv_resolution, ist = st * f.inv_resolution, ixt = xt * f.inv_resolution, iyt = yt * f.inv_resolution;
  const double ixm = ixt + kPatchMagic, iym = iyt + kPatchMagic;
  const bool lane_small = fabs(ixt) < 16384.0 && fabs(iyt) < 16384.0;

  float* s_part = s_bound;
  if (!producer) {
    float lo_x = static_cast<float>(ixt), hi_x = lo_x, lo_y = static_cast<float>(iyt), hi_y = lo_y;
    float sum_c = static_cast<float>(ct), sum_s = static_cast<float>(st);
    for (int o = 32; o > 0; o >>= 1) {
      lo_x = fminf(lo_x, __shfl_xor(lo_x, o));
      hi_x = fmaxf(hi_x, __shfl_xor(hi_x, o));
      lo_y = fminf(lo_y, __shfl_xor(lo_y, o));
      hi_y = fmaxf(hi_y, __shfl_xor(hi_y, o));
      sum_c += __shfl_xor(sum_c, o);
      sum_s += __shfl_xor(sum_s, o);
    }
    if (lane == 0) {
      float* mine = s_part + 6 * (tid >> 6);
      mine[0] = lo_x;
      mine[1] = hi_x;
      mine[2] = lo_y;
      mine[3] = hi_y;
      mine[4] = sum_c;
      mine[5] = sum_s;
    }
  }
  __syncthreads();
  double ref_c, ref_s, ref_x, ref_y;
  {
    float lo_x = s_part[0], hi_x = s_part[1], lo_y = s_part[2], hi_y = s_part[3], sum_c = s_part[4], sum_s = s_part[5];
    for (uint32_t k = 1; k < kConsumers; ++k) {
      lo_x = fminf(lo_x, s_part[6 * k]);
      hi_x = fmaxf(hi_x, s_part[6 * k + 1]);
      lo_y = fminf(lo_y, s_part[6 * k + 2]);
      hi_y = fmaxf(hi_y, s_part[6 * k + 3]);
      sum_c += s_part[6 * k + 4];
      sum_s += s_part[6 * k + 5];
    }
    const float len = sqrtf(sum_c * sum_c + sum_s * sum_s);
    ref_c = len > 0.f ? static_cast<double>(sum_c / len) : 1.0;
    ref_s = len > 0.f ? static_cast<double>(sum_s / len) : 0.0;
    ref_x = static_cast<double>(0.5f * (lo_x + hi_x));
    ref_y = static_cast<double>(0.5f * (lo_y + hi_y));
  }
  const double rc = ref_c * f.inv_resolution, rs = ref_s * f.inv_resolution;
  const double rxm = ref_x + kPatchMagic, rym = ref_y + kPatchMagic;
  __syncthreads();
// ... 213 lines not shown
        const uint32_t row_b = palette_row_offset(min(max(yu_b, -8), y_last), f.pal_pitch) - 128u;
        piece[r] = __builtin_bit_cast(uint4, __builtin_amdgcn_raw_buffer_load_b128(rsrc, (low ? column_low : column) + (half_b ? row_b : row_a), 0, 0));
      }
    };
    auto store = [&](uint32_t g, const Pieces& piece) {
      unsigned char* dst = smem + buffer_of(g) + lane * kPatchPitch;
#pragma unroll
      for (int r = 0; r < kPatchH / 8; ++r) *reinterpret_cast<uint4*>(dst + r * 16) = piece[r];
    };
    Pieces even, odd;
    fetch(0, even);
    store(0, even);
    fetch(1, odd);
    fetch(2, even);
    uint32_t g = 0;
    for (; g + 1 < groups; g += 2) {
      __syncthreads();
      store(g + 1, odd);
      fetch(g + 3, odd);
      __syncthreads();
      store(g + 2, even);
      fetch(g + 4, even);
    }
    if (g < groups) __syncthreads();
    report();
    if constexpr (kQueue) {
      if (stats.weight_sums) __syncthreads();
      continue;
    }
    return;
  }

  double acc = partial ? 0.0 : f.acc0;
  const bool fast = __builtin_amdgcn_ballot_w64(!lane_small) == 0;
  const double e_ct = fast ? ict : 0.0, e_st = fast ? ist : 0.0, e_xm = fast ? ixm : 1572864.0, e_ym = fast ? iym : 1572864.0;
  const int c_lo = static_cast<int>(kFastBias) - 1, x_hi = static_cast<int>(kFastBias + f.W), y_hi = static_cast<int>(kFastBias + f.H);
  const uint32_t row_bias = 4u - (kFastBias << 2);
  struct Lookups {
    uint32_t e[8];
    uint64_t redo;
  };
  auto particle_again = [&](uint64_t& position) -> uint32_t {
    uint32_t zero = 0;
    const uint32_t* perm_again = perm;
    asm volatile("" : "+v"(zero), "+s"(perm_again));
    position = static_cast<uint64_t>(block) * kParticles + (tid + zero);
    return perm_again[position < n ? position : n - 1];
  };
  auto add_exact = [&](uint32_t b0, uint32_t count) {
    if (count == 0) return;
    const double4* pose_again = pose;
    asm volatile("" : "+s"(pose_again));
    uint64_t position;
    const Pose2 T_again = ordered_pose(f.world_to_field, pose_again, particle_again(position));
    const double ct = T_again.r.c, st = T_again.r.s, xt = T_again.x, yt = T_again.y;
    auto term = [&](uint32_t at) {
      const double px = pts[2 * at], py = pts[2 * at + 1];
      double vx = (px * ct - py * st + xt) * f.inv_resolution, vy = (px * st + py * ct + yt) * f.inv_resolution;
      floor_rd_2(vx, vy);
      return lf_palette_value(lf_palette_fetch(rsrc, f, floor_rd_result(vx), floor_rd_result(vy), kFastBiasX));
    };
    uint32_t b = b0;
    const uint32_t end = b0 + count;
#pragma unroll 1
    for (; b + 4 <= end; b += 4) {
      const double t0 = term(b), t1 = term(b + 1), t2 = term(b + 2), t3 = term(b + 3);
      acc += sum4(t0, t1, t2, t3);
    }
#pragma unroll 1
    for (; b < end; ++b) acc += term(b);
  };
  auto consume = [&](const Lookups& e, uint32_t b0) {
    if (e.redo != 0) {
      add_exact(b0, 8);
      return;
    }
    {
      const double t0 = lf_palette_value(e.e[0]), t1 = lf_palette_value(e.e[1]), t2 = lf_palette_value(e.e[2]), t3 = lf_palette_value(e.e[3]);
      acc += sum4(t0, t1, t2, t3);
    }
    {
      const double t4 = lf_palette_value(e.e[4]), t5 = lf_palette_value(e.e[5]), t6 = lf_palette_value(e.e[6]), t7 = lf_palette_value(e.e[7]);
      acc += sum4(t4, t5, t6, t7);
    }
  };
  typedef const __attribute__((address_space(4))) double* scan_ptr_t;
  auto step_as = [&](auto is_loose, auto add_before, auto in_loop, auto whole_patch, uint32_t g, Lookups& now, const Lookups& before, uint32_t& rotor,
                     scan_ptr_t& cursor, Plan& carried) {
    const Plan plan = carried;
    const uint32_t buffer = rotor;
    rotor = buffer + kPatchBytes == patch_base + kPatchBuffers * kPatchBytes ? patch_base : buffer + kPatchBytes;
    if constexpr (!decltype(is_loose)::value) {
      asm volatile("" ::: "memory");
      __builtin_amdgcn_s_barrier();
      asm volatile("" ::: "memory");
    }
    const scan_ptr_t q = cursor;
    cursor = q + 16;
    int cx[8], cy[8];
    uint32_t lowest = 0u;
#pragma unroll
    for (int k = 0; k < 8; ++k) {
      const double px = q[2 * k], py = q[2 * k + 1];
      const double sx = __builtin_fma(px, e_ct, __builtin_fma(-py, e_st, e_xm));
      const double sy = __builtin_fma(px, e_st, __builtin_fma(py, e_ct, e_ym));
      const uint64_t bx = __builtin_bit_cast(uint64_t, sx), by = __builtin_bit_cast(uint64_t, sy);
      if (k == 0) lowest = min(static_cast<uint32_t>(bx), static_cast<uint32_t>(by));
// ... 1851 lines not shown
        const double dx = state[k].x - a.pivot_x, dy = state[k].y - a.pivot_y;
        v[0] += 1.0;
        v[1] += 1.0;
        v[2] += state[k].r.c;
        v[3] += state[k].r.s;
        v[4] += dx;
        v[5] += dy;
        v[6] += dx * dx;
        v[7] += dx * dy;
        v[8] += dy * dy;
      }
    }
  }
#pragma unroll
  for (int k = 0; k < 9; ++k) v[k] = wave_sum_f64(v[k]);
  __syncthreads();
  if (lane == 0) {
#pragma unroll
    for (int k = 0; k < 9; ++k) s_wave[wave * 9 + k] = v[k];
  }
  __syncthreads();
  if (tid < 9) {
    double acc = s_wave[tid];
    for (uint32_t q = 1; q < kSmallBlock / 64; ++q) acc += s_wave[q * 9 + tid];
    a.out[kSlotEstimate + tid] = acc;
    a.d_out[kSlotEstimate + tid] = acc;
  }
  if (tid == 0) {
    const double scalars[kSlotEss + 1] = {total, norm_sum, norm_sumsq, 0.0, 0.0, resample ? 1.0 : 0.0, static_cast<double>(n_out), ess};
    for (int k = kSlotWeightSum; k <= kSlotNormSumSq; ++k) a.out[k] = a.d_out[k] = scalars[k];
    for (int k = kSlotResampled; k <= kSlotEss; ++k) a.out[k] = a.d_out[k] = scalars[k];
    a.out[kSlotSlow] = a.d_out[kSlotSlow] = slow;
    a.out[kSlotFast] = a.d_out[kSlotFast] = fast;
    a.out[kSlotPolicy] = a.d_out[kSlotPolicy] = slow;
    a.out[kSlotPolicyFast] = a.d_out[kSlotPolicyFast] = fast;
    a.out[kSlotPolicyP] = a.d_out[kSlotPolicyP] = p;
  }
  if (a.done_flag) {
    __threadfence_system();
    __syncthreads();
    if (tid == 0) __hip_atomic_store(a.done_flag, a.done_seq, __ATOMIC_RELEASE, __HIP_MEMORY_SCOPE_SYSTEM);
  }
}
__global__ __launch_bounds__(kSmallBlock) void k_small_tail(SmallTailArgs a) { small_tail_block(a); }

static_assert(kBatchPropagateBlock == kBlock && kBatchReweightBlock == kBeamsBlock / kWave && kBatchMaxParticles == kSmallMax,
              "batch_host.h restates the small cycle's launch geometry");
__device__ __forceinline__ uint32_t batch_member_here(const BatchItem* __restrict__ items, uint32_t count, uint32_t BatchItem::*first) {
  return batch_member_of(count, blockIdx.x, [items, first](uint32_t m) { return items[m].*first; });
}
__global__ __launch_bounds__(kBlock) void k_batch_propagate(const BatchItem* __restrict__ items, uint32_t count) {
  const BatchItem& it = items[batch_member_here(items, count, &BatchItem::first_propagate_block)];
  propagate_small_block(blockIdx.x - it.first_propagate_block, batch_propagate_blocks(it.n), it.p, it.n, it.smp, it.seed, it.step, it.index_offset,
                        it.scan_src, it.scan_dst, it.scan_doubles);
}
__global__ __launch_bounds__(kBeamsBlock) void k_batch_reweight_lf_beams(const BatchItem* __restrict__ items, uint32_t count) {
  const BatchItem& it = items[batch_member_here(items, count, &BatchItem::first_reweight_block)];
  reweight_lf_beams_block(blockIdx.x - it.first_reweight_block, it.p, it.n, it.f, reinterpret_cast<const double2*>(it.scan_dst), it.B, 1u);
}
__global__ __launch_bounds__(kSmallBlock) void k_batch_small_tail(const BatchItem* __restrict__ items) {
  const SmallTailArgs a = items[blockIdx.x].tail;
  small_tail_block(a);
}

__global__ __launch_bounds__(kBlock) void k_cluster_hash(Particles p, uint64_t n, HashParams hp, unsigned long long* __restrict__ hashes) {
  const uint64_t i = static_cast<uint64_t>(blockIdx.x) * kBlock + threadIdx.x;
  if (i < n) hashes[i] = spatial_hash(load_pose(p, i), hp);
}

__global__ __launch_bounds__(kBlock) void k_cell_aggregate(const unsigned long long* __restrict__ hashes, const double* __restrict__ w,
                                                           uint64_t n, CellTable t) {
  __shared__ unsigned long long lkeys[kLocalSlots];
  __shared__ unsigned int lfirst[kLocalSlots];
  __shared__ unsigned int lcount[kLocalSlots];
  __shared__ double lsum[kLocalSlots];
  for (uint32_t s = threadIdx.x; s < kLocalSlots; s += kBlock) {
    lkeys[s] = kEmptyKey;
    lfirst[s] = 0xFFFFFFFFu;
    lcount[s] = 0;
    lsum[s] = 0.0;
  }
  __syncthreads();
  const uint64_t base = static_cast<uint64_t>(blockIdx.x) * kChunk;
#pragma unroll
  for (int k = 0; k < kChunk / kBlock; ++k) {
    const uint64_t i = base + k * kBlock + threadIdx.x;
    if (i < n) {
      const unsigned long long key = kld_key(hashes[i]);
      uint32_t slot = static_cast<uint32_t>(kld_slot(key, kLocalSlots - 1));
      while (true) {
        const unsigned long long prev = atomicCAS(&lkeys[slot], kEmptyKey, key);
        if (prev == kEmptyKey || prev == key) break;
        slot = (slot + 1) & (kLocalSlots - 1);
      }
      atomicMin(&lfirst[slot], static_cast<unsigned int>(i));
      atomicAdd(&lcount[slot], 1u);
      atomicAdd(&lsum[slot], w[i]);
    }
  }
  __syncthreads();
  const uint64_t mask = t.capacity - 1;
  for (uint32_t s = threadIdx.x; s < kLocalSlots; s += kBlock) {
    const unsigned long long key = lkeys[s];
    if (key == kEmptyKey) continue;
    uint64_t slot = kld_slot(key, mask);
    while (true) {
      const unsigned long long prev = atomicCAS(&t.keys[slot], kEmptyKey, key);
      if (prev == kEmptyKey || prev == key) break;
      slot = (slot + 1) & mask;
    }
    atomicMin(&t.first[slot], lfirst[s]);
// ... 481 lines not shown
__global__ __launch_bounds__(kBlock) void k_far_tile_votes(const uint16_t* __restrict__ idx, uint32_t tiles, uint32_t pal_base,
                                                           uint32_t count, uint32_t* __restrict__ votes) {
  const uint32_t tile = blockIdx.x * kBlock + threadIdx.x;
  uint32_t entry = 0;
  const bool uniform = tile < tiles && tile_is_uniform(idx, tile, &entry);
  const uint32_t k = (entry - pal_base) >> 3;
  const uint32_t lane = threadIdx.x & 63u;
  uint64_t pending = __builtin_amdgcn_ballot_w64(uniform && k < count);
  while (pending) {
    const uint32_t leader = static_cast<uint32_t>(__builtin_ctzll(pending));
    const uint32_t kk = static_cast<uint32_t>(__builtin_amdgcn_readlane(static_cast<int>(k), static_cast<int>(leader)));
    const uint64_t same = __builtin_amdgcn_ballot_w64(uniform && k == kk) & pending;
    if (lane == leader) atomicAdd(votes + kk, static_cast<uint32_t>(__builtin_popcountll(same)));
    pending &= ~same;
  }
}
__global__ __launch_bounds__(kBlock) void k_far_tile_bits(const uint16_t* __restrict__ idx, uint32_t tiles_x, uint32_t tiles_y,
                                                          uint32_t entry, uint32_t row_bytes, uint32_t far_bytes,
                                                          uint8_t* __restrict__ bits) {
  const uint32_t at = blockIdx.x * kBlock + threadIdx.x;
  if (at >= far_bytes) return;
  const uint32_t ty = at / row_bytes, bx = at % row_bytes;
  uint32_t byte = 0;
  if (ty < tiles_y) {
    for (uint32_t k = 0; k < 8; ++k) {
      const uint32_t tx = bx * 8 + k;
      uint32_t found;
      if (tx < tiles_x && tile_is_uniform(idx, static_cast<uint64_t>(ty) * tiles_x + tx, &found) && found == entry) byte |= 1u << k;
    }
  }
  bits[at] = static_cast<uint8_t>(byte);
}
__global__ __launch_bounds__(kBlock) void k_far_tile_bits_linear(const uint16_t* __restrict__ idx, uint32_t tiles, uint32_t entry, uint32_t bytes,
                                                                 uint8_t* __restrict__ bits) {
  const uint32_t at = blockIdx.x * kBlock + threadIdx.x;
  if (at >= bytes) return;
  uint32_t byte = 0;
  for (uint32_t k = 0; k < 8; ++k) {
    const uint64_t tile = static_cast<uint64_t>(at) * 8 + k;
    uint32_t found;
    if (tile < tiles && tile_is_uniform(idx, tile, &found) && found == entry) byte |= 1u << k;
  }
  bits[at] = static_cast<uint8_t>(byte);
}
__global__ __launch_bounds__(kBlock) void k_fill(double* p, uint64_t n, double v) {
  const uint64_t i = static_cast<uint64_t>(blockIdx.x) * kBlock + threadIdx.x;
  if (i < n) p[i] = v;
}

}

void launch_propagate(hipStream_t st, Particles p, uint64_t n, DiffDriveSampler smp, uint64_t seed, uint32_t step,
                      uint64_t index_offset, const double* scan_src, double* scan_dst, uint32_t scan_doubles, const SortScratch* sort,
                      const KeyFrame* frame, const double* normals_ahead, uint64_t normals_stride) {
  if (n == 0) {
    if (scan_dst && scan_doubles) launch_pull_scan(st, scan_src, scan_dst, scan_doubles);
    return;
  }
  const uint32_t nblocks = num_chunks(n);
  if (!(sort && frame) && n <= 65536) {
    hipLaunchKernelGGL(k_propagate_small, dim3(blocks_for(n)), dim3(kBlock), 0, st, p, n, smp, seed, step,
                       index_offset, scan_src, scan_dst, scan_doubles);
    return;
  }
  if (sort && frame && n < (1ull << 32))
    hipLaunchKernelGGL(k_propagate<true>, dim3(nblocks), dim3(kPropBlock), 0, st, p, n, smp, seed, step, index_offset, scan_src, scan_dst,
                       scan_doubles, *frame, sort->keys, sort->table, nblocks, normals_ahead, normals_stride);
  else
    hipLaunchKernelGGL(k_propagate<false>, dim3(nblocks), dim3(kPropBlock), 0, st, p, n, smp, seed, step, index_offset, scan_src, scan_dst,
                       scan_doubles, KeyFrame{}, static_cast<uint32_t*>(nullptr), static_cast<uint32_t*>(nullptr), nblocks, normals_ahead,
                       normals_stride);
}

void launch_noise_ahead(hipStream_t st, uint64_t seed, uint32_t step, uint64_t index_offset, uint64_t n, double* d_normals) {
  if (n == 0) return;
  hipLaunchKernelGGL(k_noise_ahead, dim3(blocks_for(n)), dim3(kBlock), 0, st, seed, step, index_offset, n, d_normals);
}

void launch_pull_scan(hipStream_t st, const double* scan_src, double* scan_dst, uint32_t scan_doubles) {
  if (scan_doubles == 0) return;
  hipLaunchKernelGGL(k_pull_scan, dim3(1), dim3(kBlock), 0, st, scan_src, scan_dst, scan_doubles);
}

void launch_order_particles(hipStream_t st, Particles p, uint64_t n, const SortScratch* sort, const KeyFrame* frame, bool keys_ready,
                            uint32_t layout) {
  if (n == 0 || !sort || n >= (1ull << 32)) return;
  const uint32_t nblocks = num_chunks(n);
  if (!keys_ready) {
    const KeyFrame* device_frame = nullptr;
    if (!frame) {
      double* partials = sort->bbox + 8;
      hipLaunchKernelGGL(k_bbox_partials, dim3(nblocks), dim3(kBlock), 0, st, p, n, partials, nblocks);
      hipLaunchKernelGGL(k_bbox_final, dim3(1), dim3(kBlock), 0, st, partials, nblocks, nblocks, sort->bbox, p, sort->frame, layout);
      device_frame = sort->frame;
    }
    hipLaunchKernelGGL(k_order_keys, dim3(nblocks), dim3(kWide), 0, st, p, n, frame ? *frame : KeyFrame{}, device_frame, sort->keys,
                       sort->table, nblocks);
  }
  const dim3 rows(kSortDigits / (kBlock / 64));
  hipLaunchKernelGGL(k_row_scan, rows, dim3(kBlock), 0, st, sort->table, nblocks, sort->totals, static_cast<const uint32_t*>(nullptr), 0u);
  hipLaunchKernelGGL(k_sort_scatter_high, dim3(nblocks), dim3(kStable), 0, st, sort->keys, n, sort->table, nblocks, sort->totals,
                     sort->keyidx, sort->totals + kSortDigits);
  hipLaunchKernelGGL(k_sort_buckets, dim3(kSortDigits), dim3(kStable), 0, st, sort->keyidx, sort->totals, sort->totals + kSortDigits,
                     sort->perm);
}

namespace {
uint32_t* order_half_columns(const SortScratch* sort) { return reinterpret_cast<uint32_t*>(sort->keyidx); }
uint32_t draw_workgroups(uint64_t n) { return static_cast<uint32_t>((n + kDrawBlock - 1) / kDrawBlock); }
}

void launch_order_ahead(hipStream_t st, uint64_t n, const SortScratch* sort, OrderAheadDone done) {
  if (n == 0 || !sort || n >= (1ull << 32)) return;
  const uint32_t nblocks = num_chunks(n);
  const dim3 rows(kSortDigits / (kBlock / 64));
  if (done == kOrderAheadKeys) {
    hipLaunchKernelGGL(k_key_hist, dim3(nblocks), dim3(kWide), 0, st, sort->keys, n, sort->table, nblocks);
    hipLaunchKernelGGL(k_row_scan, rows, dim3(kBlock), 0, st, sort->table, nblocks, sort->totals, static_cast<const uint32_t*>(nullptr), 0u);
  } else if (done == kOrderAheadHalfColumns) {
    hipLaunchKernelGGL(k_row_scan, rows, dim3(kBlock), 0, st, sort->table, nblocks, sort->totals,
                       static_cast<const uint32_t*>(order_half_columns(sort)), draw_workgroups(n));
  }
  hipLaunchKernelGGL(k_sort_scatter_high, dim3(nblocks), dim3(kStable), 0, st, sort->keys, n, sort->table, nblocks, sort->totals,
                     sort->keyidx, sort->totals + kSortDigits);
  hipLaunchKernelGGL(k_sort_buckets, dim3(kSortDigits), dim3(kStable), 0, st, sort->keyidx, sort->totals, sort->totals + kSortDigits,
                     sort->perm);
}

namespace {
constexpr uint32_t kFarBeamsMaxLds = 80 * 1024;
uint32_t far_beams_points_at(const FieldView& f) {
  return (kFarBeamsPalShift + f.pal_base + f.pal_count * 8u + 15u) & ~15u;
}
uint32_t far_beams_lds(const FieldView& f, uint32_t B) {
  return far_beams_points_at(f) + ((B + 63u) & ~63u) * 16u + (kFarBeamsBlock / kWave) * kFarBeamsChunk * 32u;
}
}

hipError_t configure_device_kernels() {
  const struct { const void* kernel; size_t lds; } opt_ins[] = {
      {reinterpret_cast<const void*>(k_reweight_lf_far_beams<false>), kFarBeamsMaxLds},
      {reinterpret_cast<const void*>(k_reweight_lf_far_beams<true>), kFarBeamsMaxLds},
      {reinterpret_cast<const void*>(k_small_tail), kSmallLdsBytes},
      {reinterpret_cast<const void*>(k_batch_small_tail), kSmallLdsBytes},
      {reinterpret_cast<const void*>(k_small_cluster_cells), kSmallClusterLdsBytes},
      {reinterpret_cast<const void*>(k_small_cluster_sums), kSmallClusterLdsBytes},
      {reinterpret_cast<const void*>(k_batch_small_cluster_cells), kSmallClusterLdsBytes},
      {reinterpret_cast<const void*>(k_batch_small_cluster_sums), kSmallClusterLdsBytes}};
  for (const auto& o : opt_ins)
    if (const hipError_t e = hipFuncSetAttribute(o.kernel, hipFuncAttributeMaxDynamicSharedMemorySize, static_cast<int>(o.lds)); e != hipSuccess)
      return e;
  return configure_beam_kernels();
}

namespace {
bool lf_palette_ok(const FieldView& f, const Tuning& tuning) {
  return tuning.lf_table == 0 && f.pal_idx != nullptr && f.pal_count > 0 && lf_palette_lds(f) <= 65536;
}
}
bool lf_takes_beams(const LfReweightArgs& a, const Tuning& tuning) {
  return a.n != 0 && !a.sort && lf_palette_ok(a.f, tuning) &&
         (a.beams || ((tuning.lf_variant == kLfSortedLanes || tuning.lf_variant == kLfBeamLanes) && lf_set_is_small(a.n, tuning)));
}

LfLaunch launch_reweight_lf(hipStream_t st, const LfReweightArgs& a, const Tuning& tuning) {
  const Particles p = a.p;
  const uint64_t n = a.n;
  const FieldView& f = a.f;
  const double* d_points = a.d_points;
  const uint32_t B = a.B;
  LfLaunch launched{LfKernel::kNone, 0};
  if (n == 0) return launched;
  const size_t pal_lds = lf_palette_lds(f);
  const bool palette_ok = lf_palette_ok(f, tuning);
  if (const SortScratch* sort = a.sort) {
    const uint64_t cells = static_cast<uint64_t>(f.W) * f.H;
    const bool cube_ok = f.cube != nullptr && f.W < (1u << 21) && (cells + 1) * 8 < (1ull << 31);
    uint32_t segments = 1;
    const uint64_t waves = (n + kWave - 1) / kWave;
    if (sort->partial && waves < 4096) {
      segments = static_cast<uint32_t>(std::min<uint64_t>((4096 + waves - 1) / waves, kLfMaxSegments));
      segments = std::max(1u, std::min(segments, B / 64));
    }
    const uint32_t per_segment = (B + segments - 1) / segments;
    double* partial = segments > 1 ? sort->partial : nullptr;
    const dim3 grid(blocks_for(n), segments);
    if (palette_ok) {
      const dim3 pgrid(static_cast<unsigned>((n + kPalBlock - 1) / kPalBlock), segments);
      const bool fast = tuning.lf_fast != 0 && a.scan_cells < 8192.0 && f.W < 16384 && f.H < 16384;
      const uint32_t patch_base = (static_cast<uint32_t>(pal_lds) + 15u) & ~15u;
      const size_t patch_lds = patch_base + kPatchLdsBytes;
      if (fast && a.patches && patch_lds <= 65536) {
        const uint32_t per_group = kPatchParticles;
        const unsigned groups_x = static_cast<unsigned>((n + per_group - 1) / per_group);
        PatchStats patch_stats = a.stats;
        if (segments > 1) patch_stats.weight_sums = nullptr;
        const uint32_t cus = tuning.device_cus > 0 ? static_cast<uint32_t>(tuning.device_cus) : 256u;
        const uint32_t resident = tuning.lf_queue_grid > 0 ? static_cast<uint32_t>(tuning.lf_queue_grid) : 3u * cus;
        const PatchArgs args{p.w, n, f, d_points, B, sort->perm, p.pose, partial, per_segment, patch_base, patch_stats, groups_x,
                             tuning.lf_ends_first != 0 ? 1u : 0u, (a.unit_weights && segments == 1) ? 1u : 0u};
        if (tuning.lf_queue != 0 && segments == 1 && patch_stats.arrivals != nullptr && groups_x > resident) {
          launched.kernel = LfKernel::kPatchQueue;
          hipLaunchKernelGGL(k_reweight_lf_patch<true>, dim3(resident), dim3(kPatchBlock), patch_lds, st, args);
        } else {
          launched.kernel = LfKernel::kPatch;
          hipLaunchKernelGGL(k_reweight_lf_patch<false>, dim3(groups_x, segments), dim3(kPatchBlock), patch_lds, st, args);
        }
        if (patch_stats.weight_sums) launched.weight_sums = groups_x;
      }
      else if (fast && a.dispersed && tuning.lf_far_tiles != 0 && tuning.lf_dispersed == 2 && f.far_linear != nullptr && B > 0 &&
               f.far_linear_bytes <= kFarBeamsPalShift && far_beams_lds(f, B) <= kFarBeamsMaxLds) {
        segments = 1;
        const uint64_t waves_wanted = 256ull * 4 * kFarBeamsWaves;
        const uint32_t per_wave_auto = static_cast<uint32_t>(std::min<uint64_t>(32, std::max<uint64_t>(kFarBeamsPoses, n / waves_wanted)));
        const uint32_t per_wave = tuning.lf_far_beams_per_wave > 0 ? static_cast<uint32_t>(tuning.lf_far_beams_per_wave) : per_wave_auto;
        const uint64_t per_block = static_cast<uint64_t>(per_wave) * (kFarBeamsBlock / kWave);
        const unsigned blocks = (static_cast<unsigned>((n + per_block - 1) / per_block) + 7u) & ~7u;
        if (f.prob)
          hipLaunchKernelGGL(k_reweight_lf_far_beams<true>, dim3(blocks), dim3(kFarBeamsBlock), far_beams_lds(f, B), st, p.w, n, f,
                             reinterpret_cast<const double2*>(d_points), B, sort->perm, p.pose, far_beams_points_at(f), per_wave,
                             a.unit_weights ? 1u : 0u);
        else
          hipLaunchKernelGGL(k_reweight_lf_far_beams<false>, dim3(blocks), dim3(kFarBeamsBlock), far_beams_lds(f, B), st, p.w, n, f,
                             reinterpret_cast<const double2*>(d_points), B, sort->perm, p.pose, far_beams_points_at(f), per_wave,
                             a.unit_weights ? 1u : 0u);
        launched.kernel = LfKernel::kFarBeams;
      }
      else if (fast && a.dispersed && tuning.lf_far_tiles != 0 && f.far_bits != nullptr && patch_base + f.far_bytes <= 65536) {
        const dim3 fgrid((pgrid.x + 7u) & ~7u, segments);
        hipLaunchKernelGGL((k_reweight_lf_palette<true, true>), fgrid, dim3(kPalBlock), patch_base + f.far_bytes, st, p.w, n, f, d_points, B,
                           sort->perm, p.pose, partial, per_segment, patch_base);
        launched.kernel = LfKernel::kPaletteFar;
      } else if (fast) {
        hipLaunchKernelGGL(k_reweight_lf_palette<true>, pgrid, dim3(kPalBlock), pal_lds, st, p.w, n, f, d_points, B, sort->perm, p.pose,
                           partial, per_segment, 0u);
        launched.kernel = LfKernel::kPaletteFast;
      } else {
        hipLaunchKernelGGL(k_reweight_lf_palette<false>, pgrid, dim3(kPalBlock), pal_lds, st, p.w, n, f, d_points, B, sort->perm, p.pose,
                           partial, per_segment, 0u);
        launched.kernel = LfKernel::kPaletteExact;
      }
    } else if (cube_ok) {
      hipLaunchKernelGGL(k_reweight_lf_sorted<true>, grid, dim3(kBlock), 0, st, p.w, n, f, d_points, B, sort->perm, p.pose, partial,
                         per_segment);
      launched.kernel = LfKernel::kSortedCube;
    } else {
      hipLaunchKernelGGL(k_reweight_lf_sorted<false>, grid, dim3(kBlock), 0, st, p.w, n, f, d_points, B, sort->perm, p.pose, partial,
                         per_segment);
      launched.kernel = LfKernel::kSortedField;
    }
    if (segments > 1)
      hipLaunchKernelGGL(k_lf_combine, dim3(blocks_for(n)), dim3(kBlock), 0, st, p.w, n, sort->perm, partial, segments, f.prob, f.acc0);
  } else if (lf_takes_beams(a, tuning)) {
    const uint32_t per_wave = static_cast<uint32_t>(std::min<uint64_t>(kWave, std::max<uint64_t>(1, (n + 4095) / 4096)));
    const uint64_t tiles = (n + per_wave - 1) / per_wave;
    const dim3 grid(static_cast<unsigned>((tiles + (kBeamsBlock / kWave) - 1) / (kBeamsBlock / kWave)));
    hipLaunchKernelGGL(k_reweight_lf_beams, grid, dim3(kBeamsBlock), pal_lds, st, p, n, f, reinterpret_cast<const double2*>(d_points), B,
                       per_wave);
    launched.kernel = LfKernel::kBeams;
  } else {
    hipLaunchKernelGGL(k_reweight_lf_sorted<false>, dim3(blocks_for(n)), dim3(kBlock), 0, st, p.w, n, f, d_points, B,
                       static_cast<const uint32_t*>(nullptr), p.pose, static_cast<double*>(nullptr), 0u);
    launched.kernel = LfKernel::kIndexOrder;
  }
  return launched;
}

}
extern "C" int mcl_measurement_build(void) {
#ifdef MCL_MEASUREMENT_BUILD
  return 1;
#else
  return 0;
#endif
}
namespace mcl {
void launch_lf_combine(hipStream_t st, double* w, uint64_t n, const uint32_t* perm, const double* partial, uint32_t segments, int mode) {
  hipLaunchKernelGGL(k_lf_combine, dim3(blocks_for(n)), dim3(kBlock), 0, st, w, n, perm, partial, segments, mode, mode == 0 ? 1.0 : 0.0);
}

void launch_weight_sum(hipStream_t st, const double* w, uint64_t n, double* d_partials, double* d_out, double* host_mirror) {
  const uint32_t chunks = num_chunks(n);
  if (chunks) hipLaunchKernelGGL(k_chunk_sum, dim3(chunks), dim3(kBlock), 0, st, w, n, d_partials);
  hipLaunchKernelGGL(k_final_rows, dim3(1), dim3(kBlock), 0, st, d_partials, chunks, chunks, d_out, host_mirror, Completion{});
}

void launch_normalize(hipStream_t st, double* w, uint64_t n, const double* d_factor, double* d_chunk_sum, double* d_chunk_sumsq,
                      double* d_out, double* host_mirror) {
  constexpr bool store_weights = true;
  const uint32_t chunks = num_chunks(n);
  if (chunks)
    hipLaunchKernelGGL(k_normalize, dim3(chunks), dim3(kBlock), 0, st, w, n, d_factor, d_chunk_sum, d_chunk_sumsq,
                       static_cast<const double*>(nullptr), 0u, static_cast<double*>(nullptr), static_cast<double*>(nullptr), store_weights ? 1 : 0);
  hipLaunchKernelGGL(k_final_rows, dim3(2), dim3(kBlock), 0, st, d_chunk_sum, chunks, static_cast<uint32_t>(d_chunk_sumsq - d_chunk_sum),
                     d_out, host_mirror, Completion{});
}

void launch_sum_and_normalize(hipStream_t st, double* w, uint64_t n, double* d_partials, double* d_chunk_sum, double* d_chunk_sumsq,
                              double* d_sums, double* host_mirror, bool finalize, const double* known_partials, uint32_t known_count,
                              bool store_weights) {
  const uint32_t chunks = num_chunks(n);
  if (chunks) {
    if (!known_partials) hipLaunchKernelGGL(k_chunk_sum, dim3(chunks), dim3(kBlock), 0, st, w, n, d_partials);
    const double* partials = known_partials ? known_partials : d_partials;
    const uint32_t count = known_partials ? known_count : chunks;
    if (count > 4096u) {
      hipLaunchKernelGGL(k_final_rows, dim3(1), dim3(kBlock), 0, st, partials, count, count, d_sums, host_mirror, Completion{});
      hipLaunchKernelGGL(k_normalize, dim3(chunks), dim3(kBlock), 0, st, w, n, static_cast<const double*>(d_sums), d_chunk_sum, d_chunk_sumsq,
                         static_cast<const double*>(nullptr), 0u, static_cast<double*>(nullptr), static_cast<double*>(nullptr), store_weights ? 1 : 0);
    } else {
      hipLaunchKernelGGL(k_normalize, dim3(chunks), dim3(kBlock), 0, st, w, n, static_cast<const double*>(nullptr), d_chunk_sum,
                         d_chunk_sumsq, partials, count, d_sums, host_mirror, store_weights ? 1 : 0);
    }
  } else {
    hipLaunchKernelGGL(k_final_rows, dim3(1), dim3(kBlock), 0, st, d_partials, chunks, chunks, d_sums, host_mirror, Completion{});
// ... 429 lines not shown
```

### beluga_amd/csrc/options_host.cpp

```cpp
#include "options_host.h"

#include <cctype>
#include <cstdlib>
#include <cstring>
#include <string>

namespace mcl {

namespace {

enum class Rule : int {
  kFlag,
  kTristate,
  kClamp,
  kLowBits,
  kLfVariant,
  kLfPatch,
  kKeyBits
};

struct Option {
  const char* name;
  int Tuning::*member;
  Rule rule;
  int64_t lo, hi;
};

constexpr Option kOptions[] = {
    {"lf_variant", &Tuning::lf_variant, Rule::kLfVariant, 0, 0},
    {"lf_fast", &Tuning::lf_fast, Rule::kTristate, 0, 0},
    {"lf_table", &Tuning::lf_table, Rule::kFlag, 0, 0},
    {"lf_patch", &Tuning::lf_patch, Rule::kLfPatch, 0, 0},
    {"lf_dispersed", &Tuning::lf_dispersed, Rule::kClamp, 0, 2},
    {"lf_far_tiles", &Tuning::lf_far_tiles, Rule::kClamp, 0, 2},
    {"key_layout", &Tuning::key_layout, Rule::kTristate, 0, 0},
    {"lf_loose_below", &Tuning::lf_loose_below, Rule::kClamp, 0, 257},
    {"lf_small_particles", &Tuning::lf_small_particles, Rule::kClamp, 0, INT32_MAX},
    {"device_policy", &Tuning::device_policy, Rule::kFlag, 0, 0},
    {"sort_min_particles", &Tuning::sort_min_particles, Rule::kClamp, 0, 1ll << 30},
    {"beam_sort_min_particles", &Tuning::beam_sort_min_particles, Rule::kClamp, 0, 1ll << 30},
    {"field_build", &Tuning::field_build, Rule::kFlag, 0, 0},
    {"key_curve", &Tuning::key_curve, Rule::kFlag, 0, 0},
    {"key_warp", &Tuning::key_warp, Rule::kFlag, 0, 0},
    {"key_bits_xy", &Tuning::key_bits_xy, Rule::kKeyBits, 0, 0},
    {"lf_margin", &Tuning::lf_margin, Rule::kFlag, 0, 0},
    {"lf_split", &Tuning::lf_split, Rule::kLowBits, 0, 0},
    {"lf_queue_grid", &Tuning::lf_queue_grid, Rule::kClamp, 0, 1 << 20},
    {"shard_pad_permille", &Tuning::shard_pad_permille, Rule::kClamp, 0, 8000},
    {"lf_queue", &Tuning::lf_queue, Rule::kFlag, 0, 0},
    {"lf_ends_first", &Tuning::lf_ends_first, Rule::kFlag, 0, 0},
    {"beam_free_ahead", &Tuning::beam_free_ahead, Rule::kFlag, 0, 0},
    {"beam_sectors", &Tuning::beam_sectors, Rule::kFlag, 0, 0},
    {"lf_weight_sums", &Tuning::lf_weight_sums, Rule::kFlag, 0, 0},
    {"beam_table", &Tuning::beam_table, Rule::kFlag, 0, 0},
    {"cycle_spin", &Tuning::cycle_spin, Rule::kTristate, 0, 0},
    {"scan_fused", &Tuning::scan_fused, Rule::kClamp, 0, 2},
    {"draw_fold", &Tuning::draw_fold, Rule::kClamp, 0, 2},
    {"lf_unit_weights", &Tuning::lf_unit_weights, Rule::kFlag, 0, 0},
    {"small_fused", &Tuning::small_fused, Rule::kFlag, 0, 0},
    {"norm_store", &Tuning::norm_store, Rule::kFlag, 0, 0},
    {"noise_ahead", &Tuning::noise_ahead, Rule::kClamp, 0, 2},
    {"order_ahead", &Tuning::order_ahead, Rule::kFlag, 0, 0},
    {"lf_far_beams_per_wave", &Tuning::lf_far_beams_per_wave, Rule::kClamp, 0, 4096},
    {"batch_cluster_fused", &Tuning::batch_cluster_fused, Rule::kFlag, 0, 0},
    {"batch_beam_fused", &Tuning::batch_beam_fused, Rule::kFlag, 0, 0},
    {"draw_key_hist", &Tuning::draw_key_hist, Rule::kFlag, 0, 0},
    {"rows_merged", &Tuning::rows_merged, Rule::kFlag, 0, 0},
};
constexpr size_t kOptionCount = sizeof(kOptions) / sizeof(kOptions[0]);

int normalised(const Option& o, int64_t value) {
  switch (o.rule) {
    case Rule::kFlag: return value ? 1 : 0;
    case Rule::kTristate: return value < 0 ? -1 : (value ? 1 : 0);
    case Rule::kClamp: return static_cast<int>(std::clamp<int64_t>(value, o.lo, o.hi));
    case Rule::kLowBits: return static_cast<int>(value & 3);
    case Rule::kLfVariant: return value == 0 ? kLfWavePerParticle : (value == 1 ? kLfLanePerParticle : (value == 3 ? kLfBeamLanes : kLfSortedLanes));
    case Rule::kLfPatch: return value < 0 || value > 2 ? 1 : static_cast<int>(value);
    case Rule::kKeyBits: return (value >= 4 && value <= 6) ? static_cast<int>(value) : 0;
  }
  return 0;
}

}

const char* const* tuning_names(size_t* count) {
  static const char* names[kOptionCount];
  static const bool filled = [] {
    for (size_t i = 0; i < kOptionCount; ++i) names[i] = kOptions[i].name;
    return true;
  }();
  (void)filled;
  *count = kOptionCount;
  return names;
}

bool set_tuning(Tuning& t, const char* name, int64_t value) {
  for (const Option& o : kOptions) {
    if (std::strcmp(o.name, name) != 0) continue;
    t.*o.member = normalised(o, value);
    return true;
  }
  return false;
}

void tuning_from_environment(Tuning& t, const std::function<const char*(const char*)>& lookup) {
  for (const Option& o : kOptions) {
    std::string env = "BELUGA_MCL_";
    for (const char* c = o.name; *c; ++c) env += static_cast<char>(std::toupper(static_cast<unsigned char>(*c)));
    const char* v = lookup(env.c_str());
    if (!v) continue;
    const bool cube = std::strcmp(o.name, "lf_table") == 0 && std::strcmp(v, "cube") == 0;
    t.*o.member = normalised(o, cube ? 1 : std::atoi(v));
  }
}

}
```

### beluga_amd/csrc/set_facts.h

```cpp
#pragma once

#include <cstdint>

namespace mcl {

class SetFacts {
 public:
  struct OrderTaken { bool recorded, matched; };

  bool unit_weights() const { return unit_; }
  uint32_t lf_sums() const { return lf_sums_; }
  uint64_t noise_ahead_count() const { return noise_n_; }
  bool noise_ahead_serves(uint32_t step, uint64_t n, uint64_t seed, uint64_t offset) const {
    return noise_n_ >= n && noise_step_ == step && noise_seed_ == seed && noise_offset_ == offset;
  }

  bool pivot_known() const { return pivot_known_; }
  bool pivot_heading_known() const { return pivot_known_ && heading_known_; }
  const double* pivot() const { return pivot_; }

  void set_changes() { lf_sums_ = 0; order_recorded_ = false; }
  void pivot_given(double x, double y) {
    if (!(x - x == 0.0 && y - y == 0.0)) return;
    pivot_known_ = true; heading_known_ = false; pivot_[0] = x; pivot_[1] = y;
  }
  void estimate_reported(double c, double s, double x, double y) {
    if (!(x - x == 0.0 && y - y == 0.0)) return;
    pivot_given(x, y);
    if (c - c == 0.0 && s - s == 0.0) { heading_known_ = true; heading_[0] = c; heading_[1] = s; }
  }
  void pivot_carried(double dc, double ds, double tx, double ty) {
    if (!pivot_heading_known() || !(dc - dc == 0.0 && ds - ds == 0.0 && tx - tx == 0.0 && ty - ty == 0.0)) return;
    const double c = heading_[0], s = heading_[1];
    pivot_[0] += c * tx - s * ty;
    pivot_[1] += s * tx + c * ty;
    heading_[0] = c * dc - s * ds;
    heading_[1] = s * dc + c * ds;
  }
  void set_replaced(bool unit, bool keep_pivot = false) {
    set_changes(); unit_ = unit;
    if (!keep_pivot) { pivot_known_ = heading_known_ = false; pivot_[0] = pivot_[1] = 0.0; }
  }
  void set_resized(bool grew) { set_changes(); if (grew) unit_ = false; }
  void weights_rewrite_begins() { unit_ = false; }
  void weights_touched() { unit_ = false; }
  bool take_unit_weights() { const bool was = unit_; unit_ = false; return was; }
  void lf_sums_left(uint32_t count) { lf_sums_ = count; }
  void lf_sums_dropped() { lf_sums_ = 0; }
  void weights_left_undivided(bool yes) { divides_ = yes; }
  bool take_cdf_divides() { const bool was = divides_; divides_ = false; return was; }
  void resampled_set_committed() { unit_ = true; }
  void commit_rolled_back() { unit_ = false; }
  void order_ahead_recorded(uint32_t step, uint64_t n, uint32_t layout) {
    order_recorded_ = true; order_step_ = step; order_n_ = n; order_layout_ = layout;
  }
  OrderTaken take_order_ahead(uint32_t step, uint64_t n, uint32_t layout) {
    const bool recorded = order_recorded_;
    order_recorded_ = false;
    return OrderTaken{recorded, recorded && order_step_ == step && order_n_ == n && order_layout_ == layout};
  }
  void order_accepted(bool yes) { order_accepted_ = yes; }
  bool take_order_accepted() { const bool was = order_accepted_; order_accepted_ = false; return was; }
  void noise_ahead_recorded(uint32_t step, uint64_t n, uint64_t offset, uint64_t seed) {
    noise_step_ = step; noise_n_ = n; noise_offset_ = offset; noise_seed_ = seed;
  }

 private:
  bool unit_{false}, divides_{false}, order_recorded_{false}, order_accepted_{false};
  uint32_t lf_sums_{0}, order_step_{0}, order_layout_{0}, noise_step_{0};
  uint64_t order_n_{0}, noise_n_{0}, noise_offset_{0}, noise_seed_{0};
  bool pivot_known_{false}, heading_known_{false};
  double pivot_[2]{0.0, 0.0}, heading_[2]{1.0, 0.0};
};

}
```

Measured before the change: 1646 cycles/s.

## Precompute field-frame poses in propagation for likelihood-field reweight kernels

The propagate kernel now also writes each particle's pose transformed into the field frame into a new buffer. The likelihood-field reweight kernels read that buffer instead of applying the world-to-field transform per particle. Generation tracking invalidates the buffer after map changes or resampling, and a standalone kernel rebuilds it when it is stale. The cost is an extra 32 bytes written per particle in propagation. Since resampling runs every cycle and invalidates the buffer, the rebuild path may fire often and add a kernel launch plus extra traffic.

Result: faster. 1691 cycles/s, median of 6 (+2.7%).

```diff
diff --git a/beluga_amd/csrc/context.hip b/beluga_amd/csrc/context.hip
--- a/beluga_amd/csrc/context.hip
+++ b/beluga_amd/csrc/context.hip
@@ -103,6 +103,11 @@
   SetFacts facts;
   DeviceBuffer<double> d_lf_wsum;
   DeviceBuffer<double> d_noise;
+  DeviceBuffer<double4> d_field_pose;
+  uint64_t map_generation{0};
+  uint64_t field_pose_rebuilds{0};
+  bool lf_kind() const { return cfg.sensor_kind == MCL_SENSOR_LIKELIHOOD_FIELD || cfg.sensor_kind == MCL_SENSOR_LIKELIHOOD_FIELD_PROB; }
+  FieldPoseOut field_pose_out() const { return FieldPoseOut{d_field_pose.ptr, map->origin_inverse}; }
   DiffDriveSampler order_sampler{};
   uint64_t order_ahead_used{0}, order_ahead_missed{0};
   DiffDriveSampler last_sampler{};
@@ -336,6 +341,7 @@
   MCL_HIP(ctx, ctx->d_cdf.ensure(cap));
   MCL_HIP(ctx, ctx->d_cdf_tree.ensure(cdf_tree_doubles(cap)));
   MCL_HIP(ctx, ctx->d_lf_wsum.ensure(cap / 448 + 2));
+  if (ctx->lf_kind()) MCL_HIP(ctx, ctx->d_field_pose.ensure(cap));
   if (!ctx->d_scan_state.ptr) {
     MCL_HIP(ctx, ctx->d_scan_state.ensure(kScanStateWords));
     MCL_HIP(ctx, hipMemset(ctx->d_scan_state.ptr, 0, kScanStateWords * sizeof(unsigned long long)));
@@ -752,7 +758,7 @@
 void launch_held_propagate(mcl_ctx* ctx, HeldCycle* hold) {
   const BatchItem& it = hold->item;
   launch_propagate(ctx->stream, it.p, it.n, it.smp, it.seed, it.step, it.index_offset, it.scan_src, it.scan_dst, it.scan_doubles, nullptr, nullptr,
-                   nullptr, 0);
+                   nullptr, 0, it.field_out);
   hold->propagate_held = false;
 }
 mcl_status do_propagate(mcl_ctx* ctx, const Pose2& pose, const Pose2& prev, uint32_t step, uint64_t scan_doubles = 0,
@@ -774,6 +780,8 @@
   ctx->have_last_sampler = true;
   const bool keys = !use_ahead && keys_emitted && ctx->wants_ordering() && ctx->predict_key_frame(&sampler, &frame);
   const bool ahead = ctx->d_noise.ptr && ctx->n > 65536 && ctx->facts.noise_ahead_serves(step, ctx->n, ctx->cfg.seed, ctx->cfg.shard_offset);
+  const bool field_poses = propagation_writes_field_poses(ctx->tuning, ctx->d_field_pose.ptr != nullptr, ctx->have_map);
+  const FieldPoseOut field_out = field_poses ? ctx->field_pose_out() : FieldPoseOut{nullptr, pose_identity()};
   if (hold && !keys && !ahead && ctx->n >= 1 && ctx->n <= kBatchMaxParticles && !ctx->profile) {
     BatchItem& it = hold->item;
     it.p = ctx->cur();
@@ -785,12 +793,16 @@
     it.scan_src = scan_doubles ? ctx->h_points.device : nullptr;
     it.scan_dst = scan_doubles ? ctx->d_points.ptr : nullptr;
     it.scan_doubles = static_cast<uint32_t>(scan_doubles);
+    it.field_out = field_out;
     hold->propagate_held = true;
   } else {
     launch_propagate(ctx->stream, ctx->cur(), ctx->n, sampler, ctx->cfg.seed, step, ctx->cfg.shard_offset,
                      scan_doubles ? ctx->h_points.device : nullptr, scan_doubles ? ctx->d_points.ptr : nullptr, static_cast<uint32_t>(scan_doubles),
-                     keys ? &sort : nullptr, keys ? &frame : nullptr, ahead ? ctx->d_noise.ptr : nullptr, ctx->facts.noise_ahead_count());
-  }
+                     keys ? &sort : nullptr, keys ? &frame : nullptr, ahead ? ctx->d_noise.ptr : nullptr, ctx->facts.noise_ahead_count(),
+                     field_out);
+  }
+  if (field_poses) ctx->facts.field_poses_written(ctx->map_generation);
+  else ctx->facts.poses_moved();
   if (ahead) ctx->noise_ahead_used += 1;
   if (scan_doubles) points_pulled(ctx, false);
   if (keys_emitted) *keys_emitted = keys;
@@ -839,6 +851,8 @@
   const bool have_order = ctx->facts.take_order_accepted();
   const bool lf_kind = !ctx->off_grid() && ctx->cfg.sensor_kind != MCL_SENSOR_BEAM;
   LfReweightArgs lf_args{};
+  const FieldPosePlan field_poses = lf_kind ? field_pose_plan(ctx->tuning, ctx->d_field_pose.ptr != nullptr, ctx->facts, ctx->map_generation)
+                                            : FieldPosePlan{false, false};
   if (lf_kind)
     lf_args = LfReweightArgs{.p = ctx->cur(), .n = ctx->n, .f = ctx->field_view(), .d_points = ctx->d_points.ptr, .B = static_cast<uint32_t>(B),
                              .sort = ordered ? &sort : nullptr, .patches = mode.patches, .beams = mode.beams,
@@ -848,7 +862,8 @@
                                                  reinterpret_cast<unsigned long long*>(ctx->h_scalars.device + kSlotPatchMirror),
                                                  static_cast<uint32_t>(ctx->tuning.lf_loose_below), ctx->tuning.lf_margin ? 0u : 1u,
                                                  static_cast<uint32_t>(ctx->tuning.lf_split), want_weight_sums ? ctx->d_lf_wsum.ptr : nullptr,
-                                                 reinterpret_cast<unsigned int*>(ctx->d_scalars.ptr + kSlotPatchQueue)}};
+                                                 reinterpret_cast<unsigned int*>(ctx->d_scalars.ptr + kSlotPatchQueue)},
+                             .field_pose = field_poses.load ? ctx->d_field_pose.ptr : nullptr};
   if (hold && hold->propagate_held) {
     hold->fused = lf_kind && batch_member_fused(BatchMemberFacts{
                                  ctx->cfg.sensor_kind, ctx->have_comm && ctx->comm_world > 1, ctx->tuning.small_fused != 0, ctx->n,
@@ -876,11 +891,18 @@
     else launch_reweight_bearings(ctx->stream, ctx->cur(), ctx->n, ctx->landmark_view, ctx->d_points.ptr, k);
     stage_end(ctx, MCL_STAGE_SENSOR_KERNEL);
   } else if (ctx->cfg.sensor_kind != MCL_SENSOR_BEAM) {
+    const bool held = hold && hold->fused;
+    if (field_poses.rebuild_first && !held) {
+      launch_field_pose(ctx->stream, ctx->cur().pose, ctx->n, ctx->field_pose_out());
+      ctx->facts.field_poses_written(ctx->map_generation);
+      ctx->field_pose_rebuilds += 1;
+    }
     stage_begin(ctx, MCL_STAGE_SENSOR_KERNEL);
     LfLaunch launched{LfKernel::kBeams, 0};
-    if (hold && hold->fused) {
+    if (held) {
       hold->item.f = lf_args.f;
       hold->item.B = lf_args.B;
+      hold->item.field_pose = field_poses.rebuild_first ? nullptr : lf_args.field_pose;
     } else {
       launched = launch_reweight_lf(ctx->stream, lf_args, ctx->tuning);
     }
@@ -2218,6 +2240,7 @@
   if (const std::shared_ptr<MapStore> old = ctx->map.take_private()) store->take_buffers(*old);
   ctx->map.drop();
   ctx->have_map = false;
+  ctx->map_generation += 1;
   store->key = MapStoreKey{ctx->device, ctx->cfg.sensor_kind, ctx->cfg.lf};
   const MapSource in{cells, width, height, resolution, origin, value_traits, ctx->tuning.field_build, prebuilt_field};
   std::string err;
@@ -2280,6 +2303,7 @@
   const std::shared_ptr<MapStore> old = ctx->map.take_private();
   if (!old) return fail(ctx, MCL_ERR_NOT_READY, "set the map first");
   ctx->have_map = false;
+  ctx->map_generation += 1;
   auto store = std::make_shared<MapStore>();
   store->take_buffers(*old);
   store->key = old->key;
@@ -2382,6 +2406,7 @@
   if (const mcl_status s = bind_device(ctx)) return s;
   MCL_HIP(ctx, hipStreamSynchronize(ctx->stream));
   ctx->map.attach(map->store);
+  ctx->map_generation += 1;
   map_installed(ctx);
   return MCL_OK;
 }
@@ -3461,6 +3486,7 @@
     {"noise_ahead_used", &mcl_ctx::noise_ahead_used},
     {"order_ahead_used", &mcl_ctx::order_ahead_used},
     {"order_ahead_missed", &mcl_ctx::order_ahead_missed},
+    {"field_pose_rebuilds", &mcl_ctx::field_pose_rebuilds},
     {"host_cycles", &mcl_ctx::host_cycles},
     {"cluster_cells", &mcl_ctx::cluster_cells},
     {"comm_bytes_out", &mcl_ctx::comm_bytes_out},
diff --git a/beluga_amd/csrc/cycle_host.cpp b/beluga_amd/csrc/cycle_host.cpp
--- a/beluga_amd/csrc/cycle_host.cpp
+++ b/beluga_amd/csrc/cycle_host.cpp
@@ -334,4 +334,13 @@
   return (1.0 + kRepivotMultiple) * m2 > kRepivotMultiple * second;
 }
 
-}
+bool propagation_writes_field_poses(const Tuning& tuning, bool have_buffer, bool have_map) {
+  return tuning.lf_pose_ahead != 0 && have_buffer && have_map;
+}
+
+FieldPosePlan field_pose_plan(const Tuning& tuning, bool have_buffer, const SetFacts& facts, uint64_t map_generation) {
+  if (tuning.lf_pose_ahead == 0 || !have_buffer) return FieldPosePlan{false, false};
+  return FieldPosePlan{true, !facts.field_poses_current(map_generation)};
+}
+
+}
diff --git a/beluga_amd/csrc/cycle_host.h b/beluga_amd/csrc/cycle_host.h
--- a/beluga_amd/csrc/cycle_host.h
+++ b/beluga_amd/csrc/cycle_host.h
@@ -5,6 +5,7 @@
 #include "beluga_mcl.h"
 #include "cycle_types.h"
 #include "se2.h"
+#include "set_facts.h"
 
 namespace mcl {
 
@@ -75,6 +76,10 @@
   Mode mode_{false, false};
 };
 
+bool propagation_writes_field_poses(const Tuning& tuning, bool have_buffer, bool have_map);
+struct FieldPosePlan { bool load, rebuild_first; };
+FieldPosePlan field_pose_plan(const Tuning& tuning, bool have_buffer, const SetFacts& facts, uint64_t map_generation);
+
 struct ExponentialFilter {
   double alpha{0.}, output{0.};
   void reset() { output = 0.; }
diff --git a/beluga_amd/csrc/cycle_types.h b/beluga_amd/csrc/cycle_types.h
--- a/beluga_amd/csrc/cycle_types.h
+++ b/beluga_amd/csrc/cycle_types.h
@@ -58,6 +58,7 @@
   int batch_cluster_fused = 1;
   int batch_beam_fused = 0;
   int small_fused = 1;
+  int lf_pose_ahead = 1;
   int lf_unit_weights = 1;
 };
 
diff --git a/beluga_amd/csrc/kernels.h b/beluga_amd/csrc/kernels.h
--- a/beluga_amd/csrc/kernels.h
+++ b/beluga_amd/csrc/kernels.h
@@ -14,6 +14,11 @@
 struct Particles {
   double4* pose;
   double* w;
+};
+
+struct FieldPoseOut {
+  double4* pose;
+  Pose2 world_to_field;
 };
 
 struct FieldView {
@@ -209,7 +214,8 @@
 void launch_propagate(hipStream_t st, Particles p, uint64_t n, DiffDriveSampler smp, uint64_t seed, uint32_t step,
                       uint64_t index_offset, const double* scan_src = nullptr, double* scan_dst = nullptr, uint32_t scan_doubles = 0,
                       const SortScratch* sort = nullptr, const KeyFrame* frame = nullptr, const double* normals_ahead = nullptr,
-                      uint64_t normals_stride = 0);
+                      uint64_t normals_stride = 0, FieldPoseOut field = FieldPoseOut{nullptr, Pose2{Rot2{1.0, 0.0}, 0.0, 0.0}});
+void launch_field_pose(hipStream_t st, const double4* pose, uint64_t n, const FieldPoseOut& field);
 void launch_noise_ahead(hipStream_t st, uint64_t seed, uint32_t step, uint64_t index_offset, uint64_t n, double* d_normals);
 void launch_pull_scan(hipStream_t st, const double* scan_src, double* scan_dst, uint32_t scan_doubles);
 void launch_order_particles(hipStream_t st, Particles p, uint64_t n, const SortScratch* sort, const KeyFrame* frame, bool keys_ready,
@@ -241,6 +247,7 @@
   double scan_cells;
   bool unit_weights;
   PatchStats stats;
+  const double4* field_pose;
 };
 enum class LfKernel { kNone, kPatch, kPatchQueue, kFarBeams, kPaletteFar, kPaletteFast, kPaletteExact, kSortedCube, kSortedField, kBeams, kIndexOrder };
 struct LfLaunch { LfKernel kernel; uint32_t weight_sums; };
@@ -406,6 +413,8 @@
   const double* scan_src;
   double* scan_dst;
   uint32_t scan_doubles;
+  FieldPoseOut field_out;
+  const double4* field_pose;
   FieldView f;
   uint32_t B;
   SmallTailArgs tail;
diff --git a/beluga_amd/csrc/kernels.hip b/beluga_amd/csrc/kernels.hip
--- a/beluga_amd/csrc/kernels.hip
+++ b/beluga_amd/csrc/kernels.hip
@@ -195,17 +195,26 @@
   return propagate_with_normals(state, smp, z0, z1, z2);
 }
 
+__device__ __forceinline__ double4 field_pose_record(const Pose2& world_to_field, const Pose2& state) {
+  const Pose2 T = pose_mul_ieee(world_to_field, state);
+  return double4{T.r.c, T.r.s, T.x, T.y};
+}
+
 __device__ __forceinline__ void propagate_small_block(uint32_t block, uint32_t blocks, const Particles& p, uint64_t n, const DiffDriveSampler& smp,
                                                       uint64_t seed, uint32_t step, uint64_t index_offset, const double* __restrict__ scan_src,
-                                                      double* __restrict__ scan_dst, uint32_t scan_doubles) {
+                                                      double* __restrict__ scan_dst, uint32_t scan_doubles, const FieldPoseOut& field) {
   if (scan_dst && block == blocks - 1) pull_scan(scan_src, scan_dst, scan_doubles);
   const uint64_t i = static_cast<uint64_t>(block) * kBlock + threadIdx.x;
-  if (i < n) store_pose(p, i, propagate_one(load_pose(p, i), smp, seed, step, index_offset + i));
+  if (i < n) {
+    const Pose2 out = propagate_one(load_pose(p, i), smp, seed, step, index_offset + i);
+    store_pose(p, i, out);
+    if (field.pose) field.pose[i] = field_pose_record(field.world_to_field, out);
+  }
 }
 __global__ __launch_bounds__(kBlock) void k_propagate_small(Particles p, uint64_t n, DiffDriveSampler smp, uint64_t seed, uint32_t step,
                                                            uint64_t index_offset, const double* __restrict__ scan_src,
-                                                           double* __restrict__ scan_dst, uint32_t scan_doubles) {
-  propagate_small_block(blockIdx.x, gridDim.x, p, n, smp, seed, step, index_offset, scan_src, scan_dst, scan_doubles);
+                                                           double* __restrict__ scan_dst, uint32_t scan_doubles, FieldPoseOut field) {
+  propagate_small_block(blockIdx.x, gridDim.x, p, n, smp, seed, step, index_offset, scan_src, scan_dst, scan_doubles, field);
 }
 
 constexpr int kPropBlock = 512;
@@ -214,7 +223,7 @@
                                                       uint64_t index_offset, const double* __restrict__ scan_src,
                                                       double* __restrict__ scan_dst, uint32_t scan_doubles, KeyFrame kf,
                                                       uint32_t* __restrict__ keys, uint32_t* __restrict__ table, uint32_t nblocks,
-                                                      const double* __restrict__ normals_ahead, uint64_t normals_stride) {
+                                                      const double* __restrict__ normals_ahead, uint64_t normals_stride, FieldPoseOut field) {
   __shared__ uint32_t hist[kKeys ? kSortDigits : 1];
   if (kKeys) {
     for (uint32_t d = threadIdx.x; d < kSortDigits; d += kPropBlock) hist[d] = 0;
@@ -228,6 +237,7 @@
     if (i >= n) break;
     const Pose2 out = propagate_one(load_pose(p, i), smp, seed, step, index_offset + i, normals_ahead, i, normals_stride);
     store_pose(p, i, out);
+    if (field.pose) field.pose[i] = field_pose_record(field.world_to_field, out);
     if (kKeys) {
       const uint32_t key = order_key(double4{out.r.c, out.r.s, out.x, out.y}, kf);
       keys[i] = key;
@@ -296,20 +306,29 @@
   return __builtin_bit_cast(double, __builtin_amdgcn_raw_buffer_load_b64(rsrc, offset, 0, 0));
 }
 
-__device__ __forceinline__ Pose2 ordered_pose(const Pose2& to_frame, const double4* __restrict__ pose, uint64_t i) {
+__device__ __forceinline__ Pose2 ordered_pose(const Pose2& to_frame, const double4* __restrict__ pose, uint64_t i, bool ahead) {
   const double4 q = pose[i];
+  if (ahead) return Pose2{Rot2{q.x, q.y}, q.z, q.w};
   return pose_mul_ieee(to_frame, Pose2{Rot2{q.x, q.y}, q.z, q.w});
+}
+__global__ __launch_bounds__(kBlock) void k_field_pose(const double4* __restrict__ pose, uint64_t n, Pose2 world_to_field,
+                                                       double4* __restrict__ field_pose) {
+  const uint64_t i = static_cast<uint64_t>(blockIdx.x) * kBlock + threadIdx.x;
+  if (i >= n) return;
+  const double4 q = pose[i];
+  field_pose[i] = field_pose_record(world_to_field, Pose2{Rot2{q.x, q.y}, q.z, q.w});
 }
 
 template <bool kCube>
 __global__ __launch_bounds__(kBlock) void k_reweight_lf_sorted(double* __restrict__ w, uint64_t n, FieldView f,
                                                                const double* __restrict__ pts, uint32_t B,
                                                                const uint32_t* __restrict__ perm, const double4* __restrict__ pose,
-                                                               double* __restrict__ partial, uint32_t beams_per_segment) {
+                                                               double* __restrict__ partial, uint32_t beams_per_segment,
+                                                               uint32_t pose_ahead) {
   const uint64_t t = static_cast<uint64_t>(blockIdx.x) * kBlock + threadIdx.x;
   const uint64_t tt = t < n ? t : n - 1;
   const uint64_t i = perm ? perm[tt] : tt;
-  const Pose2 T = ordered_pose(f.world_to_field, pose, i);
+  const Pose2 T = ordered_pose(f.world_to_field, pose, i, pose_ahead != 0u);
   const double ct = T.r.c, st = T.r.s, xt = T.x, yt = T.y;
   const uint32_t b_begin = partial ? blockIdx.y * beams_per_segment : 0u;
   const uint32_t b_end = partial ? (b_begin + beams_per_segment < B ? b_begin + beams_per_segment : B) : B;
@@ -419,7 +438,7 @@
                                                                    const double* __restrict__ pts, uint32_t B,
                                                                    const uint32_t* __restrict__ perm, const double4* __restrict__ pose,
                                                                    double* __restrict__ partial, uint32_t beams_per_segment,
-                                                                   uint32_t far_base) {
+                                                                   uint32_t far_base, uint32_t pose_ahead) {
   static_assert(kFast || !kFar, "far tiles ride on the biased coordinates of the FMA variant");
   extern __shared__ __attribute__((aligned(16))) unsigned char smem[];
   if constexpr (kFar) {
@@ -441,7 +460,7 @@
   const uint64_t t = static_cast<uint64_t>(block) * kPalBlock + threadIdx.x;
   const uint64_t tt = t < n ? t : n - 1;
   const uint32_t i = perm[tt];
-  const Pose2 T = ordered_pose(f.world_to_field, pose, i);
+  const Pose2 T = ordered_pose(f.world_to_field, pose, i, pose_ahead != 0u);
   const double ct = T.r.c, st = T.r.s, xt = T.x, yt = T.y;
   const uint32_t b_begin = partial ? blockIdx.y * beams_per_segment : 0u;
   const uint32_t b_end = partial ? (b_begin + beams_per_segment < B ? b_begin + beams_per_segment : B) : B;
@@ -572,7 +591,8 @@
 constexpr int kBeamsBlock = 256;
 __device__ __forceinline__ void reweight_lf_beams_block(uint32_t block, const Particles& p, uint64_t n, const FieldView& f,
                                                         const double2* __restrict__ pts, uint32_t B,
-                                                        uint32_t per_wave ) {
+                                                        uint32_t per_wave ,
+                                                        const double4* __restrict__ field_pose ) {
   extern __shared__ __attribute__((aligned(16))) unsigned char smem[];
   {
     uint32_t* s_row = reinterpret_cast<uint32_t*>(smem);
@@ -587,9 +607,8 @@
   if (base >= n) return;
   const uint32_t cnt = static_cast<uint32_t>(n - base < per_wave ? n - base : per_wave);
   const uint64_t i = base + lane;
-  Pose2 state = pose_identity();
-  if (lane < cnt) state = load_pose(p, i);
-  const Pose2 T = pose_mul_ieee(f.world_to_field, state);
+  Pose2 T = pose_identity();
+  if (lane < cnt) T = ordered_pose(f.world_to_field, field_pose ? field_pose : p.pose, i, field_pose != nullptr);
   const __amdgpu_buffer_rsrc_t rsrc =
       __builtin_amdgcn_make_buffer_rsrc(const_cast<uint16_t*>(f.pal_idx), 0, static_cast<int>(f.pal_bytes), 0x00020000);
   const uint32_t full = B & ~255u;
@@ -627,8 +646,9 @@
   if (lane < cnt) p.w[i] = p.w[i] * (f.prob ? exp(f.acc0 + mine) : f.acc0 + mine);
 }
 __global__ __launch_bounds__(kBeamsBlock) void k_reweight_lf_beams(Particles p, uint64_t n, FieldView f, const double2* __restrict__ pts,
-                                                                   uint32_t B, uint32_t per_wave ) {
-  reweight_lf_beams_block(blockIdx.x, p, n, f, pts, B, per_wave);
+                                                                   uint32_t B, uint32_t per_wave ,
+                                                                   const double4* __restrict__ field_pose) {
+  reweight_lf_beams_block(blockIdx.x, p, n, f, pts, B, per_wave, field_pose);
 }
 
 constexpr int kFarBeamsBlock = 768;
@@ -642,7 +662,8 @@
 __global__ __launch_bounds__(kFarBeamsBlock) __attribute__((amdgpu_waves_per_eu(kFarBeamsWaves, kFarBeamsWaves))) void k_reweight_lf_far_beams(double* __restrict__ w, uint64_t n, FieldView f,
                                                                           const double2* __restrict__ pts, uint32_t B,
                                                                           const uint32_t* __restrict__ perm, const double4* __restrict__ pose,
-                                                                          uint32_t pts_at, uint32_t per_wave, uint32_t unit_weights) {
+                                                                          uint32_t pts_at, uint32_t per_wave, uint32_t unit_weights,
+                                                                          uint32_t pose_ahead) {
   extern __shared__ __attribute__((aligned(16))) unsigned char smem[];
   constexpr int J = kFarBeamsPoses;
   const uint32_t rows_at = f.far_linear_bytes;
@@ -678,7 +699,7 @@
     Pose2 T = pose_identity();
     if (lane < m) {
       i = perm[first + c0 + lane];
-      T = ordered_pose(f.world_to_field, pose, i);
+      T = ordered_pose(f.world_to_field, pose, i, pose_ahead != 0u);
     }
     unsigned long long large;
     {
@@ -767,7 +788,7 @@
 #pragma unroll 1
         for (int j = 0; j < J; ++j) {
           const uint32_t iq = static_cast<uint32_t>(__builtin_amdgcn_readlane(static_cast<int>(i), static_cast<int>(q0) + j));
-          const Pose2 Tq = ordered_pose(f.world_to_field, pose, iq);
+          const Pose2 Tq = ordered_pose(f.world_to_field, pose, iq, pose_ahead != 0u);
           double sum = 0.0;
 #pragma unroll 1
           for (uint32_t k = 0; k < rounds; ++k) {
@@ -825,7 +846,7 @@
   uint32_t ends_first;
   uint32_t unit_weights;
 };
-template <bool kQueue>
+template <bool kQueue, bool kAhead>
 __global__ __launch_bounds__(kPatchBlock) __attribute__((amdgpu_waves_per_eu(6, 6))) void k_reweight_lf_patch(PatchArgs args) {
   typedef const __attribute__((address_space(4))) unsigned char* kernarg_bytes_t;
   const kernarg_bytes_t kernarg = (kernarg_bytes_t)(__builtin_amdgcn_kernarg_segment_ptr());
@@ -887,7 +908,7 @@
   const uint64_t t = producer ? first : first + tid;
   const uint64_t tt = t < n ? t : n - 1;
   const uint32_t i = perm[tt];
-  const Pose2 T = ordered_pose(f.world_to_field, pose, i);
+  const Pose2 T = ordered_pose(f.world_to_field, pose, i, kAhead);
   const double ct = T.r.c, st = T.r.s, xt = T.x, yt = T.y;
   const uint32_t b_begin = partial ? blockIdx.y * beams_per_segment : 0u;
   const uint32_t b_end = partial ? (b_begin + beams_per_segment < B ? b_begin + beams_per_segment : B) : B;
@@ -1207,7 +1228,7 @@
     const double4* pose_again = pose;
     asm volatile("" : "+s"(pose_again));
     uint64_t position;
-    const Pose2 T_again = ordered_pose(f.world_to_field, pose_again, particle_again(position));
+    const Pose2 T_again = ordered_pose(f.world_to_field, pose_again, particle_again(position), kAhead);
     const double ct = T_again.r.c, st = T_again.r.s, xt = T_again.x, yt = T_again.y;
     auto term = [&](uint32_t at) {
       const double px = pts[2 * at], py = pts[2 * at + 1];
@@ -3165,11 +3186,11 @@
 __global__ __launch_bounds__(kBlock) void k_batch_propagate(const BatchItem* __restrict__ items, uint32_t count) {
   const BatchItem& it = items[batch_member_here(items, count, &BatchItem::first_propagate_block)];
   propagate_small_block(blockIdx.x - it.first_propagate_block, batch_propagate_blocks(it.n), it.p, it.n, it.smp, it.seed, it.step, it.index_offset,
-                        it.scan_src, it.scan_dst, it.scan_doubles);
+                        it.scan_src, it.scan_dst, it.scan_doubles, it.field_out);
 }
 __global__ __launch_bounds__(kBeamsBlock) void k_batch_reweight_lf_beams(const BatchItem* __restrict__ items, uint32_t count) {
   const BatchItem& it = items[batch_member_here(items, count, &BatchItem::first_reweight_block)];
-  reweight_lf_beams_block(blockIdx.x - it.first_reweight_block, it.p, it.n, it.f, reinterpret_cast<const double2*>(it.scan_dst), it.B, 1u);
+  reweight_lf_beams_block(blockIdx.x - it.first_reweight_block, it.p, it.n, it.f, reinterpret_cast<const double2*>(it.scan_dst), it.B, 1u, it.field_pose);
 }
 __global__ __launch_bounds__(kSmallBlock) void k_batch_small_tail(const BatchItem* __restrict__ items) {
   const SmallTailArgs a = items[blockIdx.x].tail;
@@ -3757,7 +3778,7 @@
 
 void launch_propagate(hipStream_t st, Particles p, uint64_t n, DiffDriveSampler smp, uint64_t seed, uint32_t step,
                       uint64_t index_offset, const double* scan_src, double* scan_dst, uint32_t scan_doubles, const SortScratch* sort,
-                      const KeyFrame* frame, const double* normals_ahead, uint64_t normals_stride) {
+                      const KeyFrame* frame, const double* normals_ahead, uint64_t normals_stride, FieldPoseOut field) {
   if (n == 0) {
     if (scan_dst && scan_doubles) launch_pull_scan(st, scan_src, scan_dst, scan_doubles);
     return;
@@ -3765,21 +3786,26 @@
   const uint32_t nblocks = num_chunks(n);
   if (!(sort && frame) && n <= 65536) {
     hipLaunchKernelGGL(k_propagate_small, dim3(blocks_for(n)), dim3(kBlock), 0, st, p, n, smp, seed, step,
-                       index_offset, scan_src, scan_dst, scan_doubles);
+                       index_offset, scan_src, scan_dst, scan_doubles, field);
     return;
   }
   if (sort && frame && n < (1ull << 32))
     hipLaunchKernelGGL(k_propagate<true>, dim3(nblocks), dim3(kPropBlock), 0, st, p, n, smp, seed, step, index_offset, scan_src, scan_dst,
-                       scan_doubles, *frame, sort->keys, sort->table, nblocks, normals_ahead, normals_stride);
+                       scan_doubles, *frame, sort->keys, sort->table, nblocks, normals_ahead, normals_stride, field);
   else
     hipLaunchKernelGGL(k_propagate<false>, dim3(nblocks), dim3(kPropBlock), 0, st, p, n, smp, seed, step, index_offset, scan_src, scan_dst,
                        scan_doubles, KeyFrame{}, static_cast<uint32_t*>(nullptr), static_cast<uint32_t*>(nullptr), nblocks, normals_ahead,
-                       normals_stride);
+                       normals_stride, field);
 }
 
 void launch_noise_ahead(hipStream_t st, uint64_t seed, uint32_t step, uint64_t index_offset, uint64_t n, double* d_normals) {
   if (n == 0) return;
   hipLaunchKernelGGL(k_noise_ahead, dim3(blocks_for(n)), dim3(kBlock), 0, st, seed, step, index_offset, n, d_normals);
+}
+
+void launch_field_pose(hipStream_t st, const double4* pose, uint64_t n, const FieldPoseOut& field) {
+  if (n == 0 || !field.pose) return;
+  hipLaunchKernelGGL(k_field_pose, dim3(blocks_for(n)), dim3(kBlock), 0, st, pose, n, field.world_to_field, field.pose);
 }
 
 void launch_pull_scan(hipStream_t st, const double* scan_src, double* scan_dst, uint32_t scan_doubles) {
@@ -3876,6 +3902,8 @@
   const uint32_t B = a.B;
   LfLaunch launched{LfKernel::kNone, 0};
   if (n == 0) return launched;
+  const double4* const poses = a.field_pose ? a.field_pose : p.pose;
+  const uint32_t ahead = a.field_pose ? 1u : 0u;
   const size_t pal_lds = lf_palette_lds(f);
   const bool palette_ok = lf_palette_ok(f, tuning);
   if (const SortScratch* sort = a.sort) {
@@ -3902,14 +3930,16 @@
         if (segments > 1) patch_stats.weight_sums = nullptr;
         const uint32_t cus = tuning.device_cus > 0 ? static_cast<uint32_t>(tuning.device_cus) : 256u;
         const uint32_t resident = tuning.lf_queue_grid > 0 ? static_cast<uint32_t>(tuning.lf_queue_grid) : 3u * cus;
-        const PatchArgs args{p.w, n, f, d_points, B, sort->perm, p.pose, partial, per_segment, patch_base, patch_stats, groups_x,
+        const PatchArgs args{p.w, n, f, d_points, B, sort->perm, poses, partial, per_segment, patch_base, patch_stats, groups_x,
                              tuning.lf_ends_first != 0 ? 1u : 0u, (a.unit_weights && segments == 1) ? 1u : 0u};
         if (tuning.lf_queue != 0 && segments == 1 && patch_stats.arrivals != nullptr && groups_x > resident) {
           launched.kernel = LfKernel::kPatchQueue;
-          hipLaunchKernelGGL(k_reweight_lf_patch<true>, dim3(resident), dim3(kPatchBlock), patch_lds, st, args);
+          if (ahead) hipLaunchKernelGGL((k_reweight_lf_patch<true, true>), dim3(resident), dim3(kPatchBlock), patch_lds, st, args);
+          else hipLaunchKernelGGL((k_reweight_lf_patch<true, false>), dim3(resident), dim3(kPatchBlock), patch_lds, st, args);
         } else {
           launched.kernel = LfKernel::kPatch;
-          hipLaunchKernelGGL(k_reweight_lf_patch<false>, dim3(groups_x, segments), dim3(kPatchBlock), patch_lds, st, args);
+          if (ahead) hipLaunchKernelGGL((k_reweight_lf_patch<false, true>), dim3(groups_x, segments), dim3(kPatchBlock), patch_lds, st, args);
+          else hipLaunchKernelGGL((k_reweight_lf_patch<false, false>), dim3(groups_x, segments), dim3(kPatchBlock), patch_lds, st, args);
         }
         if (patch_stats.weight_sums) launched.weight_sums = groups_x;
       }
@@ -3923,35 +3953,35 @@
         const unsigned blocks = (static_cast<unsigned>((n + per_block - 1) / per_block) + 7u) & ~7u;
         if (f.prob)
           hipLaunchKernelGGL(k_reweight_lf_far_beams<true>, dim3(blocks), dim3(kFarBeamsBlock), far_beams_lds(f, B), st, p.w, n, f,
-                             reinterpret_cast<const double2*>(d_points), B, sort->perm, p.pose, far_beams_points_at(f), per_wave,
-                             a.unit_weights ? 1u : 0u);
+                             reinterpret_cast<const double2*>(d_points), B, sort->perm, poses, far_beams_points_at(f), per_wave,
+                             a.unit_weights ? 1u : 0u, ahead);
         else
           hipLaunchKernelGGL(k_reweight_lf_far_beams<false>, dim3(blocks), dim3(kFarBeamsBlock), far_beams_lds(f, B), st, p.w, n, f,
-                             reinterpret_cast<const double2*>(d_points), B, sort->perm, p.pose, far_beams_points_at(f), per_wave,
-                             a.unit_weights ? 1u : 0u);
+                             reinterpret_cast<const double2*>(d_points), B, sort->perm, poses, far_beams_points_at(f), per_wave,
+                             a.unit_weights ? 1u : 0u, ahead);
         launched.kernel = LfKernel::kFarBeams;
       }
       else if (fast && a.dispersed && tuning.lf_far_tiles != 0 && f.far_bits != nullptr && patch_base + f.far_bytes <= 65536) {
         const dim3 fgrid((pgrid.x + 7u) & ~7u, segments);
         hipLaunchKernelGGL((k_reweight_lf_palette<true, true>), fgrid, dim3(kPalBlock), patch_base + f.far_bytes, st, p.w, n, f, d_points, B,
-                           sort->perm, p.pose, partial, per_segment, patch_base);
+                           sort->perm, poses, partial, per_segment, patch_base, ahead);
         launched.kernel = LfKernel::kPaletteFar;
       } else if (fast) {
-        hipLaunchKernelGGL(k_reweight_lf_palette<true>, pgrid, dim3(kPalBlock), pal_lds, st, p.w, n, f, d_points, B, sort->perm, p.pose,
-                           partial, per_segment, 0u);
+        hipLaunchKernelGGL(k_reweight_lf_palette<true>, pgrid, dim3(kPalBlock), pal_lds, st, p.w, n, f, d_points, B, sort->perm, poses,
+                           partial, per_segment, 0u, ahead);
         launched.kernel = LfKernel::kPaletteFast;
       } else {
-        hipLaunchKernelGGL(k_reweight_lf_palette<false>, pgrid, dim3(kPalBlock), pal_lds, st, p.w, n, f, d_points, B, sort->perm, p.pose,
-                           partial, per_segment, 0u);
+        hipLaunchKernelGGL(k_reweight_lf_palette<false>, pgrid, dim3(kPalBlock), pal_lds, st, p.w, n, f, d_points, B, sort->perm, poses,
+                           partial, per_segment, 0u, ahead);
         launched.kernel = LfKernel::kPaletteExact;
       }
     } else if (cube_ok) {
-      hipLaunchKernelGGL(k_reweight_lf_sorted<true>, grid, dim3(kBlock), 0, st, p.w, n, f, d_points, B, sort->perm, p.pose, partial,
-                         per_segment);
+      hipLaunchKernelGGL(k_reweight_lf_sorted<true>, grid, dim3(kBlock), 0, st, p.w, n, f, d_points, B, sort->perm, poses, partial,
+                         per_segment, ahead);
       launched.kernel = LfKernel::kSortedCube;
     } else {
-      hipLaunchKernelGGL(k_reweight_lf_sorted<false>, grid, dim3(kBlock), 0, st, p.w, n, f, d_points, B, sort->perm, p.pose, partial,
-                         per_segment);
+      hipLaunchKernelGGL(k_reweight_lf_sorted<false>, grid, dim3(kBlock), 0, st, p.w, n, f, d_points, B, sort->perm, poses, partial,
+                         per_segment, ahead);
       launched.kernel = LfKernel::kSortedField;
     }
     if (segments > 1)
@@ -3961,11 +3991,11 @@
     const uint64_t tiles = (n + per_wave - 1) / per_wave;
     const dim3 grid(static_cast<unsigned>((tiles + (kBeamsBlock / kWave) - 1) / (kBeamsBlock / kWave)));
     hipLaunchKernelGGL(k_reweight_lf_beams, grid, dim3(kBeamsBlock), pal_lds, st, p, n, f, reinterpret_cast<const double2*>(d_points), B,
-                       per_wave);
+                       per_wave, a.field_pose);
     launched.kernel = LfKernel::kBeams;
   } else {
     hipLaunchKernelGGL(k_reweight_lf_sorted<false>, dim3(blocks_for(n)), dim3(kBlock), 0, st, p.w, n, f, d_points, B,
-                       static_cast<const uint32_t*>(nullptr), p.pose, static_cast<double*>(nullptr), 0u);
+                       static_cast<const uint32_t*>(nullptr), poses, static_cast<double*>(nullptr), 0u, ahead);
     launched.kernel = LfKernel::kIndexOrder;
   }
   return launched;
diff --git a/beluga_amd/csrc/options_host.cpp b/beluga_amd/csrc/options_host.cpp
--- a/beluga_amd/csrc/options_host.cpp
+++ b/beluga_amd/csrc/options_host.cpp
@@ -68,6 +68,9 @@
     {"rows_merged", &Tuning::rows_merged, Rule::kFlag, 0, 0},
 };
 constexpr size_t kOptionCount = sizeof(kOptions) / sizeof(kOptions[0]);
+constexpr Option kLaterOptions[] = {
+    {"lf_pose_ahead", &Tuning::lf_pose_ahead, Rule::kFlag, 0, 0},
+};
 
 int normalised(const Option& o, int64_t value) {
   switch (o.rule) {
@@ -101,6 +104,11 @@
     t.*o.member = normalised(o, value);
     return true;
   }
+  for (const Option& o : kLaterOptions) {
+    if (std::strcmp(o.name, name) != 0) continue;
+    t.*o.member = normalised(o, value);
+    return true;
+  }
   return false;
 }
 
diff --git a/beluga_amd/csrc/set_facts.h b/beluga_amd/csrc/set_facts.h
--- a/beluga_amd/csrc/set_facts.h
+++ b/beluga_amd/csrc/set_facts.h
@@ -15,11 +15,13 @@
     return noise_n_ >= n && noise_step_ == step && noise_seed_ == seed && noise_offset_ == offset;
   }
 
+  bool field_poses_current(uint64_t generation) const { return field_poses_ && field_generation_ == generation; }
+
   bool pivot_known() const { return pivot_known_; }
   bool pivot_heading_known() const { return pivot_known_ && heading_known_; }
   const double* pivot() const { return pivot_; }
 
-  void set_changes() { lf_sums_ = 0; order_recorded_ = false; }
+  void set_changes() { lf_sums_ = 0; order_recorded_ = false; field_poses_ = false; }
   void pivot_given(double x, double y) {
     if (!(x - x == 0.0 && y - y == 0.0)) return;
     pivot_known_ = true; heading_known_ = false; pivot_[0] = x; pivot_[1] = y;
@@ -49,8 +51,10 @@
   void lf_sums_dropped() { lf_sums_ = 0; }
   void weights_left_undivided(bool yes) { divides_ = yes; }
   bool take_cdf_divides() { const bool was = divides_; divides_ = false; return was; }
-  void resampled_set_committed() { unit_ = true; }
-  void commit_rolled_back() { unit_ = false; }
+  void resampled_set_committed() { unit_ = true; field_poses_ = false; }
+  void commit_rolled_back() { unit_ = false; field_poses_ = false; }
+  void field_poses_written(uint64_t generation) { field_poses_ = true; field_generation_ = generation; }
+  void poses_moved() { field_poses_ = false; }
   void order_ahead_recorded(uint32_t step, uint64_t n, uint32_t layout) {
     order_recorded_ = true; order_step_ = step; order_n_ = n; order_layout_ = layout;
   }
@@ -69,6 +73,8 @@
   bool unit_{false}, divides_{false}, order_recorded_{false}, order_accepted_{false};
   uint32_t lf_sums_{0}, order_step_{0}, order_layout_{0}, noise_step_{0};
   uint64_t order_n_{0}, noise_n_{0}, noise_offset_{0}, noise_seed_{0};
+  bool field_poses_{false};
+  uint64_t field_generation_{0};
   bool pivot_known_{false}, heading_known_{false};
   double pivot_[2]{0.0, 0.0}, heading_[2]{1.0, 0.0};
 };
```
